# EnricoMiccoli/nodal

Measured on AMD Instinct MI355X. Metric: circuits_per_sec, higher is better.
Workload: dtype f64; 1 GPU; cfg3: grid(1000) 1e6 nodes, sparse CSR path; n=999999, nnz=4995995, parallelism=one GPU

## Files before the change

### nodal_amd/csrc/knobs.h

```cpp
#pragma once
#include <stdint.h>
#include <stdlib.h>

#include <optional>

namespace knob {

struct Present {
    const char *name;
    bool now() const { return getenv(name) != nullptr; }
};
struct OnUnless0 {
    const char *name;
    bool now() const { const char *e = getenv(name); return !(e && atoi(e) == 0); }
};
struct OffUnlessNon0 {
    const char *name;
    bool now() const { const char *e = getenv(name); return e && atoi(e) != 0; }
};
struct OnIfSet0 {
    const char *name;
    bool now() const { const char *e = getenv(name); return e != nullptr && atoi(e) == 0; }
};
struct Level {
    const char *name;
    int now() const {
        const char *e = getenv(name);
        if (!e) return 0;
        const int v = atoi(e);
        return v > 1 ? v : 1;
    }
};
struct Int {
    const char *name;
    int dflt;
    int now() const { const char *e = getenv(name); return e ? atoi(e) : dflt; }
};
struct Int64 {
    const char *name;
    int64_t dflt;
    int64_t now() const { const char *e = getenv(name); return e ? atoll(e) : dflt; }
};
struct Double {
    const char *name;
    double dflt;
    double now() const { const char *e = getenv(name); return e ? atof(e) : dflt; }
};
struct IntIfSet {
    const char *name;
    std::optional<int> now() const { const char *e = getenv(name); return e ? std::optional<int>(atoi(e)) : std::nullopt; }
};
struct Int64IfSet {
    const char *name;
    std::optional<int64_t> now() const { const char *e = getenv(name); return e ? std::optional<int64_t>(atoll(e)) : std::nullopt; }
};
struct DoubleIfSet {
    const char *name;
    std::optional<double> now() const { const char *e = getenv(name); return e ? std::optional<double>(atof(e)) : std::nullopt; }
};
struct Text {
    const char *name;
    const char *now() const { return getenv(name); }
};

inline constexpr Present TRACE{"NODAL_TRACE"};
inline constexpr Level POISON{"NODAL_POISON"};
inline constexpr Present NOFILL{"NODAL_NOFILL"};
inline constexpr Present NANCHECK{"NODAL_NANCHECK"};
inline constexpr Double WAIT_TIMEOUT_S{"NODAL_WAIT_TIMEOUT_S", 60.0};
inline constexpr Text STREAM_PRIORITY{"NODAL_STREAM_PRIORITY"};
inline constexpr IntIfSet EXTRA_STREAMS{"NODAL_EXTRA_STREAMS"};
inline constexpr IntIfSet HOST_THREADS{"NODAL_HOST_THREADS"};
inline constexpr IntIfSet CSV_CHUNKS{"NODAL_CSV_CHUNKS"};
inline constexpr OnUnless0 FOLD_STREAM{"NODAL_FOLD_STREAM"};
inline constexpr OffUnlessNon0 COUNT_LDS{"NODAL_COUNT_LDS"};
inline constexpr IntIfSet DENSE_BLOCKINV{"NODAL_DENSE_BLOCKINV"};
inline constexpr IntIfSet GJ_SCALAR{"NODAL_GJ_SCALAR"};
inline constexpr OnUnless0 GJ_DPP{"NODAL_GJ_DPP"};
inline constexpr OnUnless0 BI_SYM{"NODAL_BI_SYM"};
inline constexpr OnIfSet0 BI_MASKED{"NODAL_BI_MASKED"};
inline constexpr Int PANEL_CUS{"NODAL_PANEL_CUS", 32};
inline constexpr Int64 BI_UNMASK_ROWS{"NODAL_BI_UNMASK_ROWS", 0};
inline constexpr OnUnless0 BI_EARLY_COPY{"NODAL_BI_EARLY_COPY"};
inline constexpr Int BI_FIRST_BLOCKS{"NODAL_BI_FIRST_BLOCKS", 2};
inline constexpr Text BI_SWITCH{"NODAL_BI_SWITCH"};
inline constexpr Text BI_SWITCH2{"NODAL_BI_SWITCH2"};
inline constexpr Text BI_WIDTH{"NODAL_BI_WIDTH"};
inline constexpr IntIfSet GEPP_PANEL{"NODAL_GEPP_PANEL"};
inline constexpr Int GEPP_MAX{"NODAL_GEPP_MAX", 1280};
inline constexpr Present GEPP_PROBE{"NODAL_GEPP_PROBE"};
inline constexpr Int64IfSet FCG_MAXIT{"NODAL_FCG_MAXIT"};
inline constexpr OnUnless0 FCG_HOST_SUM{"NODAL_FCG_HOST_SUM"};
inline constexpr Double FCG_LOOK{"NODAL_FCG_LOOK", 0.75};
inline constexpr OnUnless0 LOWDEG{"NODAL_LOWDEG"};
inline constexpr IntIfSet LOWDEG_SHARE{"NODAL_LOWDEG_SHARE"};
inline constexpr Int64 LOWDEG_MIN{"NODAL_LOWDEG_MIN", 32};
inline constexpr Present SPARSE_FORCE_DIRECT{"NODAL_SPARSE_FORCE_DIRECT"};
inline constexpr Present SPARSE_CHILD_DIRECT{"NODAL_SPARSE_CHILD_DIRECT"};
inline constexpr OnUnless0 SAGG{"NODAL_SAGG"};
inline constexpr OnUnless0 SA_REUSE{"NODAL_SA_REUSE"};
inline constexpr OnUnless0 SA_FORK{"NODAL_SA_FORK"};
inline constexpr Double SA_SPREAD{"NODAL_SA_SPREAD", 16.0};
inline constexpr Double SA_SHARE{"NODAL_SA_SHARE", 0.9};
inline constexpr IntIfSet SA_MIS{"NODAL_SA_MIS"};
inline constexpr Text SA_OMEGA_P{"NODAL_SA_OMEGA_P"};
inline constexpr Double SA_PADSLACK{"NODAL_SA_PADSLACK", 1.3};
inline constexpr OnUnless0 SA_D16{"NODAL_SA_D16"};
inline constexpr Int SA_GG{"NODAL_SA_GG", 40};
inline constexpr Int64 SA_GCAP{"NODAL_SA_GCAP", 16384};
inline constexpr Int SA_GSEG{"NODAL_SA_GSEG", 4};
inline constexpr Text SA_NU{"NODAL_SA_NU"};
inline constexpr Int SA_KCYCLE{"NODAL_SA_KCYCLE", 1};
inline constexpr Int SA_KLEVELS{"NODAL_SA_KLEVELS", 1};
inline constexpr OnUnless0 SA_KFREEZE{"NODAL_SA_KFREEZE"};
inline constexpr OnUnless0 SA_FUSE_DIR{"NODAL_SA_FUSE_DIR"};
inline constexpr OffUnlessNon0 SA_GRAPH{"NODAL_SA_GRAPH"};
inline constexpr Text SA_FOLD_POST{"NODAL_SA_FOLD_POST"};
inline constexpr OffUnlessNon0 SA_FOLD_CHECK{"NODAL_SA_FOLD_CHECK"};
inline constexpr OnUnless0 SA_TAIL_DENSE{"NODAL_SA_TAIL_DENSE"};
inline constexpr OffUnlessNon0 SA_TAIL_CHECK{"NODAL_SA_TAIL_CHECK"};
inline constexpr Int SA_TAIL_NU{"NODAL_SA_TAIL_NU", 3};
inline constexpr Present TAIL_PROBE{"NODAL_TAIL_PROBE"};
inline constexpr IntIfSet AMG_PASSES0{"NODAL_AMG_PASSES0"};
inline constexpr IntIfSet AMG_PASSES1{"NODAL_AMG_PASSES1"};
inline constexpr IntIfSet AMG_SWEEPS0{"NODAL_AMG_SWEEPS0"};
inline constexpr IntIfSet AMG_BLOCK{"NODAL_AMG_BLOCK"};
inline constexpr DoubleIfSet AMG_THETA{"NODAL_AMG_THETA"};
inline constexpr Present AMG_KEEP_DENSE{"NODAL_AMG_KEEP_DENSE"};
inline constexpr Present AMG_NOTAIL{"NODAL_AMG_NOTAIL"};
inline constexpr IntIfSet AMG_KMAX{"NODAL_AMG_KMAX"};
inline constexpr OnUnless0 PAIRS_BLOCK{"NODAL_PAIRS_BLOCK"};
inline constexpr OnUnless0 PAIRS_FUNCTIONAL{"NODAL_PAIRS_FUNCTIONAL"};
inline constexpr Int PAIRS_DIRECT{"NODAL_PAIRS_DIRECT", -1};
inline constexpr Int64 PAIRS_DIRECT_MIN{"NODAL_PAIRS_DIRECT_MIN", 256};
inline constexpr Double MULTI_BAR{"NODAL_MULTI_BAR", 1e-14};
inline constexpr IntIfSet PRESOLVE{"NODAL_PRESOLVE"};
inline constexpr OnUnless0 PRESOLVE_KEEP{"NODAL_PRESOLVE_KEEP"};
inline constexpr IntIfSet FGMRES_WINDOW{"NODAL_FGMRES_WINDOW"};
inline constexpr Text DIRECT_NB{"NODAL_DIRECT_NB"};
inline constexpr Int DIRECT_LANES{"NODAL_DIRECT_LANES", 4};
inline constexpr DoubleIfSet DIRECT_MAX_GB{"NODAL_DIRECT_MAX_GB"};
inline constexpr IntIfSet DIRECT_BIG_DIM{"NODAL_DIRECT_BIG_DIM"};
inline constexpr OnUnless0 DIRECT_FRONT_LDS{"NODAL_DIRECT_FRONT_LDS"};
inline constexpr Int DIRECT_LDS_BS{"NODAL_DIRECT_LDS_BS", 64};
inline constexpr OnUnless0 DIRECT_PANEL_REGS{"NODAL_DIRECT_PANEL_REGS"};
inline constexpr OnUnless0 DIRECT_BATCHED{"NODAL_DIRECT_BATCHED"};
inline constexpr OnUnless0 DIRECT_WAVE{"NODAL_DIRECT_WAVE"};
inline constexpr Present DIRECT_LEVELS{"NODAL_DIRECT_LEVELS"};
inline constexpr OnUnless0 DIRECT_SUPER{"NODAL_DIRECT_SUPER"};
inline constexpr OnUnless0 DIRECT_APPLY_STEPPED{"NODAL_DIRECT_APPLY_STEPPED"};
inline constexpr OnUnless0 DIRECT_PEEL{"NODAL_DIRECT_PEEL"};
inline constexpr Int ND_DEPTH{"NODAL_ND_DEPTH", 4};
inline constexpr Int64 ND_PAR{"NODAL_ND_PAR", 20000};
inline constexpr Present SLU_DEBUG{"SLU_DEBUG"};

}
```

### nodal_amd/csrc/sagg.hip

```cpp
#include <hip/hip_ext.h>

#include <atomic>
#include <type_traits>

#include "group.h"

int grounded_flags(nodal_ctx *h, uint8_t *flags_dev);

namespace {

using grp::TB;
constexpr int PW = 4;
constexpr int ACAP = 64;
constexpr int RCAP = 96;
constexpr int RCAP_SMALL = 512;
constexpr int RCAP_SMALL_ROWS = 16384;
inline int rcap_for(int64_t nc) { return nc <= RCAP_SMALL_ROWS ? RCAP_SMALL : RCAP; }
constexpr int W0_MAX = 32;
constexpr int COARSEST = 64;
constexpr int MAX_LEVELS = 12;
constexpr int MIS_ROUNDS = 6;
constexpr int TAIL_MAX_N = 1024;
constexpr int TAIL_LEVELS = 6;
constexpr int TAIL_LDS_BUDGET = 150 * 1024;
constexpr int APAD = 32;
constexpr int DOT_BLOCKS = 1024;
#ifndef NODAL_SA_OMEGA
#define NODAL_SA_OMEGA 0.85
#endif
constexpr double OMEGA = NODAL_SA_OMEGA;
constexpr double OMEGA_P = 0.70;
constexpr double OMEGA_P_COARSE = 0.85;
using cyc_t = nodal_cyc_t;

inline unsigned grid_for(int64_t n, unsigned cap = 8192) {
    int64_t g = (n + TB - 1) / TB;
    if (g < 1) g = 1;
    if (g >= 64) g = (g + 7) & ~(int64_t)7;
    return (unsigned)(g > cap ? cap : g);
}
inline int64_t pad64(int64_t n) { return (n + 63) & ~(int64_t)63; }
inline size_t align256(size_t x) { return (x + 255) & ~(size_t)255; }

__device__ __forceinline__ unsigned xcd_block() {
    const unsigned g = gridDim.x, b = blockIdx.x;
    return (g & 7u) ? b : (b & 7u) * (g >> 3) + (b >> 3);
}


struct Ell {
    int64_t n = 0, ld = 0;
    int32_t width = 0;
    const int32_t *col = nullptr;
    const int16_t *dcol = nullptr;
    const double *val = nullptr;
    const float *valf = nullptr;
    const int32_t *len = nullptr;
};

enum { ST_MAXLEN = 0, ST_GRADED = 1, ST_BADDIAG = 2, ST_OVERFLOW = 3, ST_NNZ = 4, ST_UNASSIGNED = 5,
       ST_MAXR = 6, ST_NC = 7 ,
       ST_FARCOL = 8 ,
       ST_FOLDMISS = 9 ,
       ST_COUNT = 10 };

struct SLevel {
    int64_t n = 0, ld = 0, nc = 0;
    int32_t width = 0;
    int32_t maxlen = 0;
    int32_t wfix = 0;
    int64_t nnz = 0;
    DevBuf acol, aval, alen, dinv;
    DevBuf adcol;
    bool d16 = false;
    DevBuf agg, pcol, pval;
    DevBuf rcol, rval, rlen;
    int64_t rld = 0;
    DevBuf vec, part, gflag;
    DevBuf avalf, pvalf, rvalf;
    DevBuf wcol, wval, wlen;
    int32_t wslots = 0;
    bool fold_want = false, fold = false;
    Ell A() const {
        Ell e;
        e.n = n; e.ld = ld; e.width = width;
        e.col = acol.as<int32_t>(); e.val = aval.as<double>(); e.len = alen.as<int32_t>();
        e.valf = avalf.as<float>();
        e.dcol = d16 ? adcol.as<int16_t>() : nullptr;
        return e;
    }
    template <typename T = double> T *v(int which) const { return reinterpret_cast<T *>(vec.as<double>() + (int64_t)which * ld); }
};
enum { V_X = 0, V_R = 1, V_XP = 2, V_RC = 3, V_C1 = 4, V_C2 = 5, V_V1 = 6, V_V2 = 7, V_R2 = 8, V_X1 = 9, V_T = 10,
       V_COUNT = 11 };

struct TailLevelDesc {
    int n, nc, ld, rld, width, nq, lpr;
    const int32_t *acol, *pcol, *rcol, *rlen, *alen;
    const double *aval, *dinv, *pval, *rval;
    int o_aval, o_acol, o_dinv, o_pval, o_pcol, o_rval, o_rcol, o_B, o_X, o_Y, o_R;
};
struct TailDesc {
    int nlev;
    TailLevelDesc lv[TAIL_LEVELS];
    const double *inv;
    int nu;
    int image_bytes;
    int lds_bytes;
    int skip;
    int slots;
    long long *stamps;
};

struct SHierarchy {
    std::vector<SLevel *> pool;
    int nlev = 0;
    int tail = -1;
    bool ready = false;
    bool kcycle = true;
    bool kfrozen = false;
    int kslot = -1, kcount = 0, ksamples = 0;
    int klevels = 1;
    int nu[3] = {2, 1, 2};
    bool dense_coarsest = true;
    DevBuf tail_stamps, tail_image, apcol, apval, aplen, bstat;
    DevBuf tail_op;
    bool tail_dense = false;
    DevBuf mvec;
    hipEvent_t ev_copy = nullptr;
    hipStream_t aux = nullptr;
    hipEvent_t ev_fork = nullptr, ev_join = nullptr, ev_flags = nullptr;
    bool aux_pending = false;
    bool aux_tried = false;
    bool want_flags = false;
    int flags_levels = 0;
    DevBuf stats, coarse_inv, mis_t, mis_m, mis_flag, mis_id, agg1, keys, rstart, cursor, lists;
    TailDesc td;
    uint64_t *host_stats = nullptr;
    bool sym_valid = false;
    uint64_t sym_epoch = 0;
    int64_t sym_n = 0, sym_nnz = 0;
    bool sym_general = false, sym_check = false;
    int32_t sym_floating = 0;
    hipGraph_t it_graph = nullptr;
    hipGraphExec_t it_exec = nullptr;
    uint64_t it_key = 0;
    bool refreshed = false;
    int last_iters = 0;
    int hint_iters = 0;
    int64_t hint_n = 0, hint_nnz = 0;
    int mblock_iters = 0;
    int64_t mblock_n = 0;
    unsigned long long sym_stats[MAX_LEVELS * ST_COUNT] = {0};
    SLevel *level(int l) {
        while ((int)pool.size() <= l) pool.push_back(new SLevel());
        return pool[l];
    }
    void drop_graph() {
        if (it_exec) (void)hipGraphExecDestroy(it_exec);
        if (it_graph) (void)hipGraphDestroy(it_graph);
        it_exec = nullptr;
        it_graph = nullptr;
        it_key = 0;
    }
    ~SHierarchy() {
        drop_graph();
        if (ev_copy) (void)hipEventDestroy(ev_copy);
        if (ev_fork) (void)hipEventDestroy(ev_fork);
        if (ev_join) (void)hipEventDestroy(ev_join);
        if (ev_flags) (void)hipEventDestroy(ev_flags);
        if (aux) (void)hipStreamDestroy(aux);
        for (SLevel *l : pool) {
            DevBuf *b[] = {&l->acol, &l->aval, &l->alen, &l->dinv, &l->agg, &l->pcol, &l->pval, &l->rcol,
                           &l->rval, &l->rlen, &l->vec, &l->part, &l->gflag, &l->avalf, &l->pvalf, &l->rvalf, &l->adcol,
                           &l->wcol, &l->wval, &l->wlen};
            for (DevBuf *x : b) x->release();
            delete l;
        }
        tail_image.release();
        tail_op.release();
        mvec.release();
        tail_stamps.release();
        bstat.release();
        apcol.release();
        apval.release();
        aplen.release();
        DevBuf *b[] = {&stats, &coarse_inv, &mis_t, &mis_m, &mis_flag, &mis_id, &agg1, &keys, &rstart, &cursor, &lists};
        for (DevBuf *x : b) x->release();
        if (host_stats) (void)hipHostFree(host_stats);
    }
};


constexpr int BSTAT_MAX = 65536;
__global__ __launch_bounds__(1024) void reduce_bstat(int nblocks, const uint32_t *__restrict__ bstat,
                                                     unsigned long long *__restrict__ stats, int slot_max,
                                                     int slot_sum) {
    __shared__ unsigned int s_max;
    __shared__ unsigned long long s_sum;
    if (threadIdx.x == 0) { s_max = 0; s_sum = 0; }
    __syncthreads();
    unsigned int m = 0;
    unsigned long long t = 0;
    for (int i = threadIdx.x; i < nblocks; i += 1024) {
        m = max(m, bstat[i]);
        t += bstat[BSTAT_MAX + i];
    }
    atomicMax(&s_max, m);
    atomicAdd(&s_sum, t);
    __syncthreads();
    if (threadIdx.x == 0) {
        if (slot_max >= 0) stats[slot_max] = s_max;
        if (slot_sum >= 0) stats[slot_sum] = s_sum;
    }
}

__global__ __launch_bounds__(TB) void row_stats(int64_t n, const int32_t *__restrict__ indptr,
                                                const int32_t *__restrict__ indices,
                                                const double *__restrict__ data, double share, double spread,
                                                bool general, unsigned long long *__restrict__ stats,
                                                uint32_t *__restrict__ bstat) {
    int32_t mlen = 0;
    uint32_t graded = 0, bad = 0, far = 0;
    for (int64_t i = (int64_t)xcd_block() * TB + threadIdx.x; i < n; i += (int64_t)gridDim.x * TB) {
        const int32_t e0 = indptr[i], e1 = indptr[i + 1];
        mlen = max(mlen, e1 - e0);
        double d = 0.0, mx = 0.0, mn = 1e300;
        for (int32_t e = e0; e < e1; ++e) {
            const double v = data[e];
            const int64_t dc = (int64_t)indices[e] - i;
            if (dc > 32767 || dc < -32767) far = 1;
            if (indices[e] == (int32_t)i) d = v;
            else if (v != 0.0) {
                mx = fmax(mx, fabs(v));
                mn = fmin(mn, fabs(v));
                if (v > 0.0 && !general) bad = 1;
            }
        }
        if (!(d > 0.0)) bad = 1;
        graded += (d > 0.0 && (mx > share * d || mx > spread * mn)) ? 1u : 0u;
    }
    __shared__ unsigned int s_len, s_graded, s_bad;
    if (threadIdx.x == 0) s_len = s_graded = s_bad = 0;
    __syncthreads();
    atomicMax(&s_len, (unsigned)mlen);
    if (graded) atomicAdd(&s_graded, graded);
    if (bad) atomicOr(&s_bad, 1u);
    if (far) atomicOr(&s_bad, 2u);
    __syncthreads();
    if (threadIdx.x == 0) {
        bstat[blockIdx.x] = s_len;
        bstat[BSTAT_MAX + blockIdx.x] = s_graded;
        if (s_bad & 1u) atomicOr(&stats[ST_BADDIAG], 1ull);
        if (s_bad & 2u) stats[ST_FARCOL] = 1ull;
    }
}

__global__ __launch_bounds__(TB) void csr_to_ell(int64_t n, int64_t ld, const int32_t *__restrict__ indptr,
                                                 const int32_t *__restrict__ indices,
                                                 const double *__restrict__ data, int32_t *__restrict__ col,
                                                 double *__restrict__ val, float *__restrict__ valf,
                                                 int32_t *__restrict__ len, double *__restrict__ dinv, int32_t wpad,
                                                 int16_t *__restrict__ dcol) {
    for (int64_t i = (int64_t)xcd_block() * TB + threadIdx.x; i < n; i += (int64_t)gridDim.x * TB) {
        const int32_t e0 = indptr[i], e1 = indptr[i + 1];
        double d = 1.0;
        for (int32_t e = e0; e < e1; ++e) {
            const int32_t c = indices[e];
            const double v = data[e];
            col[(int64_t)(e - e0) * ld + i] = c;
            if (dcol) dcol[(int64_t)(e - e0) * ld + i] = (int16_t)(c - (int32_t)i);
            val[(int64_t)(e - e0) * ld + i] = v;
            valf[(int64_t)(e - e0) * ld + i] = (float)v;
            if (c == (int32_t)i) d = v;
        }
        for (int32_t s = e1 - e0; s < wpad; ++s) {
            col[(int64_t)s * ld + i] = (int32_t)i;
            if (dcol) dcol[(int64_t)s * ld + i] = 0;
            val[(int64_t)s * ld + i] = 0.0;
            valf[(int64_t)s * ld + i] = 0.0f;
        }
        len[i] = e1 - e0;
        dinv[i] = 1.0 / d;
    }
}


__device__ __forceinline__ uint32_t hash30(uint32_t x) {
    x ^= x >> 16;
    x *= 0x7feb352du;
    x ^= x >> 15;
    x *= 0x846ca68bu;
    x ^= x >> 16;
    return x & 0x3fffffffu;
}

__global__ __launch_bounds__(TB) void mis_init(int64_t n, uint32_t *__restrict__ T) {
    for (int64_t i = (int64_t)xcd_block() * TB + threadIdx.x; i < n; i += (int64_t)gridDim.x * TB)
        T[i] = (1u << 30) | hash30((uint32_t)i);
}

template <int NB>
__device__ __forceinline__ uint32_t nbr_max_batch(const Ell &A, const uint32_t *__restrict__ v, int64_t i, int32_t l, int32_t s0,
                                                  uint32_t best) {
    int32_t c[NB];
#pragma unroll
    for (int u = 0; u < NB; ++u) c[u] = A.col[(int64_t)(s0 + u < l ? s0 + u : 0) * A.ld + i];
    uint32_t t[NB];
#pragma unroll
    for (int u = 0; u < NB; ++u) t[u] = v[c[u]];
#pragma unroll
    for (int u = 0; u < NB; ++u) best = t[u] > best ? t[u] : best;
    return best;
}
__device__ __forceinline__ uint32_t nbr_max(const Ell &A, const uint32_t *__restrict__ v, int64_t i, int32_t l, uint32_t best) {
    if (l <= 5) return nbr_max_batch<5>(A, v, i, l, 0, best);
    for (int32_t s0 = 0; s0 < l; s0 += 8) best = nbr_max_batch<8>(A, v, i, l, s0, best);
    return best;
}

__global__ __launch_bounds__(TB) void mis_max(Ell A, const uint32_t *__restrict__ v, uint32_t *__restrict__ m) {
    for (int64_t i = (int64_t)xcd_block() * TB + threadIdx.x; i < A.n; i += (int64_t)gridDim.x * TB)
        m[i] = nbr_max(A, v, i, A.len[i], v[i]);
}

__global__ __launch_bounds__(TB) void mis_update(Ell A, uint32_t *__restrict__ T, const uint32_t *__restrict__ m1) {
    for (int64_t i = (int64_t)xcd_block() * TB + threadIdx.x; i < A.n; i += (int64_t)gridDim.x * TB) {
        const uint32_t own = T[i];
        if ((own >> 30) != 1) continue;
        const uint32_t best = nbr_max(A, m1, i, A.len[i], m1[i]);
        if (best == own) T[i] = own | (2u << 30);
        else if ((best >> 30) == 3) T[i] = 0;
    }
}

__global__ __launch_bounds__(TB) void mis_count(int64_t n, const uint32_t *__restrict__ T,
                                                unsigned long long *__restrict__ out) {
    uint32_t left = 0;
    for (int64_t i = (int64_t)xcd_block() * TB + threadIdx.x; i < n; i += (int64_t)gridDim.x * TB)
        left += (T[i] >> 30) == 1 ? 1u : 0u;
#pragma unroll
    for (int off = 32; off > 0; off >>= 1) left += __shfl_down(left, off, 64);
    if ((threadIdx.x & 63) == 0 && left) atomicAdd(out, (unsigned long long)left);
}

__global__ __launch_bounds__(TB) void mis_flag_roots(Ell A, const uint32_t *__restrict__ T,
                                                     uint32_t *__restrict__ flag) {
    for (int64_t i = (int64_t)xcd_block() * TB + threadIdx.x; i <= A.n; i += (int64_t)gridDim.x * TB) {
        uint32_t f = 0;
        if (i < A.n) {
            const uint32_t own = T[i];
            if ((own >> 30) == 3) f = 1;
            else if ((own >> 30) == 1) {
                bool near = false;
                const int32_t l = A.len[i];
                for (int32_t s = 0; s < l; ++s) near = near || (T[A.col[(int64_t)s * A.ld + i]] >> 30) == 3;
                f = near ? 0u : 1u;
            }
        }
        flag[i] = f;
    }
}

constexpr int64_t MIS_SMALL_MAX = 1024;
__global__ __launch_bounds__(1024) void mis_small(Ell A, uint32_t *__restrict__ T, uint32_t *__restrict__ M,
                                                  uint32_t *__restrict__ flag, int rounds) {
    const int64_t n = A.n;
    for (int64_t i = threadIdx.x; i < n; i += 1024) T[i] = (1u << 30) | hash30((uint32_t)i);
    __syncthreads();
    for (int r = 0; r < rounds; ++r) {
        for (int64_t i = threadIdx.x; i < n; i += 1024) {
            uint32_t best = T[i];
            const int32_t l = A.len[i];
            for (int32_t s = 0; s < l; ++s) {
                const uint32_t t = T[A.col[(int64_t)s * A.ld + i]];
                best = t > best ? t : best;
            }
            M[i] = best;
        }
        __syncthreads();
        for (int64_t i = threadIdx.x; i < n; i += 1024) {
            const uint32_t own = T[i];
            if ((own >> 30) != 1) continue;
            uint32_t best = M[i];
            const int32_t l = A.len[i];
            for (int32_t s = 0; s < l; ++s) {
                const uint32_t t = M[A.col[(int64_t)s * A.ld + i]];
                best = t > best ? t : best;
            }
            if (best == own) T[i] = own | (2u << 30);
            else if ((best >> 30) == 3) T[i] = 0;
        }
        __syncthreads();
    }
    for (int64_t i = threadIdx.x; i <= n; i += 1024) {
        uint32_t f = 0;
        if (i < n) {
            const uint32_t own = T[i];
            if ((own >> 30) == 3) f = 1;
            else if ((own >> 30) == 1) {
                bool near = false;
                const int32_t l = A.len[i];
                for (int32_t s = 0; s < l; ++s) near = near || (T[A.col[(int64_t)s * A.ld + i]] >> 30) == 3;
                f = near ? 0u : 1u;
            }
        }
        flag[i] = f;
    }
}

__global__ __launch_bounds__(TB) void assign_near(Ell A, const uint32_t *__restrict__ T,
                                                  const uint32_t *__restrict__ flag,
                                                  const uint32_t *__restrict__ id, int32_t *__restrict__ agg1) {
    for (int64_t i = (int64_t)xcd_block() * TB + threadIdx.x; i < A.n; i += (int64_t)gridDim.x * TB) {
        int32_t a = -1;
        if (flag[i]) a = (int32_t)id[i];
        else {
            uint32_t best = 0;
            const int32_t l = A.len[i];
            auto batch = [&](auto NBc, int32_t s0) {
                constexpr int NB = decltype(NBc)::value;
                int32_t c[NB];
#pragma unroll
                for (int u = 0; u < NB; ++u) c[u] = A.col[(int64_t)(s0 + u < l ? s0 + u : 0) * A.ld + i];
                uint32_t fl[NB], tt[NB], idd[NB];
#pragma unroll
                for (int u = 0; u < NB; ++u) {
                    fl[u] = flag[c[u]];
                    tt[u] = T[c[u]];
                    idd[u] = id[c[u]];
                }
#pragma unroll
                for (int u = 0; u < NB; ++u) {
                    if (s0 + u >= l || c[u] == (int32_t)i || !fl[u]) continue;
                    const uint32_t t = tt[u] | (3u << 30);
                    if (t > best) { best = t; a = (int32_t)idd[u]; }
                }
            };
            if (l <= 5) batch(std::integral_constant<int, 5>{}, 0);
            else for (int32_t s0 = 0; s0 < l; s0 += 8) batch(std::integral_constant<int, 8>{}, s0);
        }
        agg1[i] = a;
    }
}

__global__ __launch_bounds__(TB) void assign_far(Ell A, const int32_t *__restrict__ agg1, int32_t *__restrict__ agg,
                                                 unsigned long long *__restrict__ stats) {
    for (int64_t i = (int64_t)xcd_block() * TB + threadIdx.x; i < A.n; i += (int64_t)gridDim.x * TB) {
        int32_t a = agg1[i];
        if (a < 0) {
            double bw = -1.0;
            const int32_t l = A.len[i];
            auto batch = [&](auto NBc, int32_t s0) {
                constexpr int NB = decltype(NBc)::value;
                int32_t c[NB];
                double w[NB];
#pragma unroll
                for (int u = 0; u < NB; ++u) {
                    const int64_t at = (int64_t)(s0 + u < l ? s0 + u : 0) * A.ld + i;
                    c[u] = A.col[at];
                    w[u] = fabs(A.val[at]);
                }
                int32_t aj[NB];
#pragma unroll
                for (int u = 0; u < NB; ++u) aj[u] = agg1[c[u]];
#pragma unroll
                for (int u = 0; u < NB; ++u) {
                    if (s0 + u >= l || c[u] == (int32_t)i || aj[u] < 0) continue;
                    if (w[u] > bw) { bw = w[u]; a = aj[u]; }
                }
            };
            if (l <= 5) batch(std::integral_constant<int, 5>{}, 0);
            else for (int32_t s0 = 0; s0 < l; s0 += 8) batch(std::integral_constant<int, 8>{}, s0);
            if (a < 0) stats[ST_UNASSIGNED] = 1;
        }
        agg[i] = a;
    }
}

__global__ __launch_bounds__(TB) void build_P(Ell A, const double *__restrict__ dinv,
                                              const int32_t *__restrict__ agg, int32_t *__restrict__ pcol,
                                              double *__restrict__ pval, float *__restrict__ pvalf, double omega_p) {
    for (int64_t i = (int64_t)xcd_block() * TB + threadIdx.x; i < A.n; i += (int64_t)gridDim.x * TB) {
        int32_t c[PW];
        double v[PW];
#pragma unroll
        for (int k = 0; k < PW; ++k) { c[k] = -1; v[k] = 0.0; }
        const int32_t own = agg[i];
        c[0] = own;
        v[0] = 1.0;
        const double wd = omega_p * dinv[i];
        const int32_t l = A.len[i];
        for (int32_t s = 0; s < l; ++s) {
            const int32_t J = agg[A.col[(int64_t)s * A.ld + i]];
            const double t = -wd * A.val[(int64_t)s * A.ld + i];
            bool placed = false;
#pragma unroll
            for (int k = 0; k < PW; ++k) {
                if (!placed && c[k] == J) { v[k] += t; placed = true; }
            }
#pragma unroll
            for (int k = 1; k < PW; ++k) {
                if (!placed && c[k] < 0) { c[k] = J; v[k] = t; placed = true; }
            }
            if (!placed) v[0] += t;
        }
#pragma unroll
        for (int k = 0; k < PW; ++k) {
            pcol[(int64_t)k * A.ld + i] = c[k];
            pval[(int64_t)k * A.ld + i] = v[k];
            pvalf[(int64_t)k * A.ld + i] = (float)v[k];
        }
    }
}

__global__ __launch_bounds__(TB) void r_count(int64_t n, int64_t ld, const int32_t *__restrict__ pcol,
                                              uint32_t *__restrict__ cnt, uint32_t *__restrict__ place) {
    for (int64_t i = (int64_t)xcd_block() * TB + threadIdx.x; i < n; i += (int64_t)gridDim.x * TB) {
#pragma unroll
        for (int k = 0; k < PW; ++k) {
            const int32_t J = pcol[(int64_t)k * ld + i];
            if (J >= 0) place[(int64_t)k * ld + i] = atomicAdd(&cnt[J], 1u);
        }
    }
}
__global__ __launch_bounds__(TB) void r_fill(int64_t n, int64_t ld, const int32_t *__restrict__ pcol,
                                             const uint32_t *__restrict__ rstart, const uint32_t *__restrict__ place,
                                             uint64_t *__restrict__ keys) {
    for (int64_t i = (int64_t)xcd_block() * TB + threadIdx.x; i < n; i += (int64_t)gridDim.x * TB) {
#pragma unroll
        for (int k = 0; k < PW; ++k) {
            const int32_t J = pcol[(int64_t)k * ld + i];
            if (J >= 0) keys[rstart[J] + place[(int64_t)k * ld + i]] = ((uint64_t)i << 2) | (uint64_t)k;
        }
    }
}
__global__ __launch_bounds__(TB) void r_to_ell(int64_t nc, int64_t rld, const uint32_t *__restrict__ rstart,
                                               const uint64_t *__restrict__ keys, int64_t ld,
                                               const double *__restrict__ pval, int32_t *__restrict__ rcol,
                                               double *__restrict__ rval, float *__restrict__ rvalf,
                                               int32_t *__restrict__ rlen,
                                               unsigned long long *__restrict__ stats, uint32_t *__restrict__ bstat,
                                               uint32_t rcap) {
    uint32_t mlen = 0;
    const int sub = threadIdx.x & 7;
    const int64_t rows_per_pass = (int64_t)gridDim.x * (TB / 8);
    for (int64_t I = (int64_t)xcd_block() * (TB / 8) + threadIdx.x / 8; I < nc; I += rows_per_pass) {
        const uint32_t s0 = rstart[I];
        uint32_t l = rstart[I + 1] - s0;
        mlen = l > mlen ? l : mlen;
        if (l > rcap) l = rcap;
        const uint32_t upto = nc <= 4096 ? rcap : ((l + 7u) & ~7u);
        for (uint32_t t = sub; t < upto; t += 8) {
            const int64_t at = ((int64_t)(t >> 3) * rld + I) * 8 + (t & 7);
            if (t < l) {
                const uint64_t key = keys[s0 + t];
                const int64_t i = (int64_t)(key >> 2);
                const double v = pval[(int64_t)(key & 3) * ld + i];
                rcol[at] = (int32_t)i;
                rval[at] = v;
                rvalf[at] = (float)v;
            } else {
                rcol[at] = 0;
                rval[at] = 0.0;
                rvalf[at] = 0.0f;
            }
        }
        if (sub == 0) rlen[I] = (int32_t)l;
    }
    if (mlen > rcap) atomicOr(&stats[ST_OVERFLOW], 2ull);
    __shared__ unsigned int s_max;
    if (threadIdx.x == 0) s_max = 0;
    __syncthreads();
#pragma unroll
    for (int off = 32; off > 0; off >>= 1) {
        const uint32_t o = __shfl_down(mlen, off, 64);
        mlen = o > mlen ? o : mlen;
    }
    if ((threadIdx.x & 63) == 0) atomicMax(&s_max, mlen);
    __syncthreads();
    if (threadIdx.x == 0) {
        bstat[blockIdx.x] = s_max;
        bstat[BSTAT_MAX + blockIdx.x] = 0;
    }
}

__global__ __launch_bounds__(TB) void r_refresh(int64_t nc, int64_t rld, const int32_t *__restrict__ rlen,
                                                const int32_t *__restrict__ rcol, int64_t ld,
                                                const int32_t *__restrict__ pcol, const double *__restrict__ pval,
                                                double *__restrict__ rval, float *__restrict__ rvalf) {
    const int sub = threadIdx.x & 7;
    const int64_t rows_per_pass = (int64_t)gridDim.x * (TB / 8);
    for (int64_t I = (int64_t)xcd_block() * (TB / 8) + threadIdx.x / 8; I < nc; I += rows_per_pass) {
        const int32_t l = rlen[I];
        for (int32_t t = sub; t < l; t += 8) {
            const int64_t at = ((int64_t)(t >> 3) * rld + I) * 8 + (t & 7);
            const int64_t i = rcol[at];
            double v = 0.0;
#pragma unroll
            for (int k = 0; k < PW; ++k) {
                const double pv = pval[(int64_t)k * ld + i];
                v = pcol[(int64_t)k * ld + i] == (int32_t)I ? pv : v;
            }
            rval[at] = v;
            rvalf[at] = (float)v;
        }
    }
}

__global__ __launch_bounds__(TB) void r_sort_short(const uint32_t *__restrict__ rstart, uint64_t *__restrict__ keys,
                                                   int64_t nc) {
    for (int64_t I = (int64_t)xcd_block() * TB + threadIdx.x; I < nc; I += (int64_t)gridDim.x * TB) {
        const uint32_t s0 = rstart[I];
        const int len = (int)(rstart[I + 1] - s0);
        if (len < 2) continue;
        if (len <= 4) grp::sort_short_row<4>(keys + s0, len);
        else if (len <= 8) grp::sort_short_row<8>(keys + s0, len);
        else if (len <= 16) grp::sort_short_row<16>(keys + s0, len);
        else if (len <= 32) grp::sort_short_row<32>(keys + s0, len);
    }
}
__global__ __launch_bounds__(64) void r_sort_medium(const uint32_t *__restrict__ rstart, uint64_t *__restrict__ keys,
                                                    int64_t nc) {
    __shared__ uint64_t buf[RCAP_SMALL];
    const int lane = threadIdx.x;
    for (int64_t I = blockIdx.x; I < nc; I += gridDim.x) {
        const uint32_t s0 = rstart[I];
        const int len = (int)(rstart[I + 1] - s0);
        if (len <= 32 || len > RCAP_SMALL) continue;
        const int P = len <= 64 ? 64 : (len <= 128 ? 128 : (len <= 256 ? 256 : 512));
        for (int e = lane; e < P; e += 64) buf[e] = e < len ? keys[s0 + e] : ~0ull;
        __syncthreads();
        for (int size = 2; size <= P; size <<= 1)
            for (int stride = size >> 1; stride > 0; stride >>= 1) {
                for (int p = lane; p < P / 2; p += 64) {
                    const int i = ((p & ~(stride - 1)) << 1) | (p & (stride - 1));
                    const int j = i | stride;
                    const bool up = (i & size) == 0;
                    const uint64_t a = buf[i], b = buf[j];
                    if ((a > b) == up) { buf[i] = b; buf[j] = a; }
                }
                __syncthreads();
            }
        for (int e = lane; e < len; e += 64) keys[s0 + e] = buf[e];
        __syncthreads();
    }
}

__device__ __forceinline__ int wave_excl_scan(int v, int *total) {
    const int lane = threadIdx.x & 63;
    int incl = v;
#pragma unroll
    for (int off = 1; off < 64; off <<= 1) {
        const int t = __shfl_up(incl, off, 64);
        if (lane >= off) incl += t;
    }
    *total = __shfl(incl, 63, 64);
    return incl - v;
}

template <int APW, bool EMIT>
__global__ __launch_bounds__(TB) void ap_rows(Ell A, const int32_t *__restrict__ pcol, const double *__restrict__ pval,
                                              int32_t *__restrict__ apcol, double *__restrict__ apval,
                                              int32_t *__restrict__ aplen, unsigned long long *__restrict__ stats,
                                              const double *__restrict__ dinv, int32_t *__restrict__ wcol,
                                              float *__restrict__ wval, int32_t *__restrict__ wlen) {
    bool overflow = false, miss = false;
    for (int64_t i = (int64_t)xcd_block() * TB + threadIdx.x; i < A.n; i += (int64_t)gridDim.x * TB) {
        int32_t c[APW];
        double v[APW];
        [[maybe_unused]] int32_t Jo[PW];
        [[maybe_unused]] double po[PW], wd = 0.0;
        if constexpr (EMIT) {
#pragma unroll
            for (int sp = 0; sp < PW; ++sp) {
                Jo[sp] = pcol[(int64_t)sp * A.ld + i];
                po[sp] = pval[(int64_t)sp * A.ld + i];
            }
            wd = OMEGA * dinv[i];
        }
#pragma unroll
        for (int q = 0; q < APW; ++q) { c[q] = -1; v[q] = 0.0; }
        int cnt = 0;
        const int32_t l = A.len[i];
        for (int32_t s = 0; s < l; ++s) {
            const int32_t k = A.col[(int64_t)s * A.ld + i];
            const double a = A.val[(int64_t)s * A.ld + i];
            int32_t J[PW];
            double pp[PW];
#pragma unroll
            for (int sp = 0; sp < PW; ++sp) {
                J[sp] = pcol[(int64_t)sp * A.ld + k];
                pp[sp] = pval[(int64_t)sp * A.ld + k];
            }
#pragma unroll
            for (int sp = 0; sp < PW; ++sp) {
                if (J[sp] < 0) continue;
                const double t = a * pp[sp];
                bool placed = false;
#pragma unroll
                for (int q = 0; q < APW; ++q)
                    if (!placed && c[q] == J[sp]) { v[q] += t; placed = true; }
#pragma unroll
                for (int q = 0; q < APW; ++q)
                    if (!placed && c[q] < 0) { c[q] = J[sp]; v[q] = t; placed = true; cnt = q + 1; }
                if (!placed) overflow = true;
            }
        }
#pragma unroll
        for (int q = 0; q < APW; ++q)
            if (q < cnt) {
                apcol[(int64_t)q * A.ld + i] = c[q];
                apval[(int64_t)q * A.ld + i] = v[q];
            }
        aplen[i] = cnt;
        if constexpr (EMIT) {
            int have = 0, found = 0;
#pragma unroll
            for (int sp = 0; sp < PW; ++sp) have += Jo[sp] >= 0 ? 1 : 0;
#pragma unroll
            for (int q = 0; q < APW; ++q)
                if (q < cnt) {
                    double pv = 0.0;
#pragma unroll
                    for (int sp = 0; sp < PW; ++sp)
                        if (Jo[sp] == c[q]) { pv += po[sp]; ++found; }
                    wcol[(int64_t)q * A.ld + i] = c[q];
                    wval[(int64_t)q * A.ld + i] = (float)(pv - wd * v[q]);
                }
            wlen[i] = cnt;
            if (found != have) miss = true;
        }
    }
    if (overflow) atomicOr(&stats[ST_OVERFLOW], 4ull);
    if (miss) stats[ST_FOLDMISS] = 1ull;
}

template <int APW, bool EMIT>
__global__ __launch_bounds__(64) void ap_rows_lds(Ell A, const int32_t *__restrict__ pcol,
                                                  const double *__restrict__ pval, int32_t *__restrict__ apcol,
                                                  double *__restrict__ apval, int32_t *__restrict__ aplen,
                                                  unsigned long long *__restrict__ stats,
                                                  const double *__restrict__ dinv, int32_t *__restrict__ wcol,
                                                  float *__restrict__ wval, int32_t *__restrict__ wlen) {
    __shared__ int32_t tc[APW * 64];
    __shared__ double tv[APW * 64];
    const int lane = threadIdx.x;
    bool overflow = false, miss = false;
    for (int64_t i0 = (int64_t)xcd_block() * 64; i0 < A.n; i0 += (int64_t)gridDim.x * 64) {
        const int64_t i = i0 + lane;
#pragma unroll 8
        for (int q = 0; q < APW; ++q) tc[q * 64 + lane] = -1;
        int cnt = 0;
        if (i < A.n) {
            const int32_t l = A.len[i];
            [[maybe_unused]] int32_t Jo[PW];
            [[maybe_unused]] double po[PW], wd = 0.0;
            if constexpr (EMIT) {
#pragma unroll
                for (int sp = 0; sp < PW; ++sp) {
                    Jo[sp] = pcol[(int64_t)sp * A.ld + i];
                    po[sp] = pval[(int64_t)sp * A.ld + i];
                }
                wd = OMEGA * dinv[i];
            }
            constexpr int AB = 4;
            for (int32_t s0 = 0; s0 < l; s0 += AB) {
                int32_t kk[AB];
                double aa[AB];
#pragma unroll
                for (int u = 0; u < AB; ++u) {
                    const int32_t su = s0 + u < l ? s0 + u : 0;
                    kk[u] = A.col[(int64_t)su * A.ld + i];
                    aa[u] = A.val[(int64_t)su * A.ld + i];
                }
                int32_t J[AB][PW];
                double pp[AB][PW];
#pragma unroll
                for (int u = 0; u < AB; ++u)
#pragma unroll
                    for (int sp = 0; sp < PW; ++sp) {
                        J[u][sp] = pcol[(int64_t)sp * A.ld + kk[u]];
                        pp[u][sp] = pval[(int64_t)sp * A.ld + kk[u]];
                    }
#pragma unroll
                for (int u = 0; u < AB; ++u) {
                    if (s0 + u >= l) continue;
#pragma unroll
                    for (int sp = 0; sp < PW; ++sp) {
                        if (J[u][sp] < 0) continue;
                        const double t = aa[u] * pp[u][sp];
                        uint32_t slot = ((uint32_t)J[u][sp] * 2654435761u) >> 16 & (APW - 1);
                        bool placed = false;
                        for (int probe = 0; probe < APW && !placed; ++probe) {
                            const int32_t c = tc[slot * 64 + lane];
                            if (c == J[u][sp]) {
                                tv[slot * 64 + lane] += t;
                                placed = true;
                            } else if (c < 0) {
                                tc[slot * 64 + lane] = J[u][sp];
                                tv[slot * 64 + lane] = t;
                                ++cnt;
                                placed = true;
                            }
                            slot = (slot + 1) & (APW - 1);
                        }
                        if (!placed) overflow = true;
                    }
                }
            }
            int o = 0, found = 0;
            for (int q = 0; q < APW; ++q) {
                const int32_t c = tc[q * 64 + lane];
                if (c >= 0) {
                    const double t = tv[q * 64 + lane];
                    apcol[(int64_t)o * A.ld + i] = c;
                    apval[(int64_t)o * A.ld + i] = t;
                    if constexpr (EMIT) {
                        double pv = 0.0;
#pragma unroll
                        for (int sp = 0; sp < PW; ++sp)
                            if (Jo[sp] == c) { pv += po[sp]; ++found; }
                        wcol[(int64_t)o * A.ld + i] = c;
                        wval[(int64_t)o * A.ld + i] = (float)(pv - wd * t);
                    }
                    ++o;
                }
            }
            aplen[i] = cnt;
            if constexpr (EMIT) {
                int have = 0;
#pragma unroll
                for (int sp = 0; sp < PW; ++sp) have += Jo[sp] >= 0 ? 1 : 0;
                wlen[i] = cnt;
                if (found != have) miss = true;
            }
        }
    }
    if (overflow) atomicOr(&stats[ST_OVERFLOW], 4ull);
    if (miss) stats[ST_FOLDMISS] = 1ull;
}

__device__ __forceinline__ int galerkin_products(int64_t ld, const int32_t *__restrict__ apcol,
                                                 const double *__restrict__ apval, const int32_t *__restrict__ aplen,
                                                 int64_t rld, const int32_t *__restrict__ rcol,
                                                 const double *__restrict__ rval, int64_t I, int t0, int tn,
                                                 int32_t *lJ, double *lV) {
    const int lane = threadIdx.x;
    int32_t i = 0, len = 0;
    double w = 0.0;
    if (lane < tn) {
        const int t = t0 + lane;
        const int64_t rat = ((int64_t)(t >> 3) * rld + I) * 8 + (t & 7);
        i = rcol[rat];
        w = rval[rat];
        len = aplen[i];
    }
    int np = 0;
    int o = wave_excl_scan(len, &np);
    constexpr int INFL = 8;
    for (int32_t s0 = 0; s0 < len; s0 += INFL) {
        int32_t cj[INFL];
        double cv[INFL];
#pragma unroll
        for (int q = 0; q < INFL; ++q) {
            const int32_t s = s0 + q < len ? s0 + q : s0;
            cj[q] = apcol[(int64_t)s * ld + i];
            cv[q] = apval[(int64_t)s * ld + i];
        }
#pragma unroll
        for (int q = 0; q < INFL; ++q)
            if (s0 + q < len) {
                lJ[o] = cj[q];
                lV[o] = w * cv[q];
                ++o;
            }
    }
    for (int p = lane + np; p < np + 72; p += 64) lJ[p] = -1;
    __syncthreads();
    return np;
}

template <bool NUMERIC>
__global__ __launch_bounds__(64) void galerkin(int64_t ld, const int32_t *__restrict__ apcol,
                                               const double *__restrict__ apval, const int32_t *__restrict__ aplen,
                                               int64_t nc, int64_t rld, const int32_t *__restrict__ rcol,
                                               const double *__restrict__ rval, const int32_t *__restrict__ rlen,
                                               int64_t cld, int32_t *__restrict__ ccol, double *__restrict__ cval,
                                               float *__restrict__ cvalf,
                                               int32_t *__restrict__ clen, double *__restrict__ cdinv,
                                               unsigned long long *__restrict__ stats, uint32_t *__restrict__ bstat,
                                               int G, int pcap, int maxseg) {
    extern __shared__ __attribute__((aligned(16))) char gsm[];
    int32_t *set = reinterpret_cast<int32_t *>(gsm);
    double *lV = reinterpret_cast<double *>(gsm + 1024);
    int32_t *lJ = reinterpret_cast<int32_t *>(lV + pcap);
    const int lane = threadIdx.x;
    uint32_t my_max = 0, my_nnz = 0, my_flags = 0;
    for (int64_t I = blockIdx.x; I < nc; I += gridDim.x) {
        const int rl = rlen[I];
        const int ngroups = (rl + G - 1) / G;
        int np = 0;
        int total = 0;
        int32_t myJ = 0x7fffffff;
        if constexpr (NUMERIC) {
            total = clen[I];
            if (lane < total) myJ = ccol[(int64_t)lane * cld + I];
        } else {
        for (int k = lane; k < 256; k += 64) set[k] = -1;
        __syncthreads();
        for (int g = 0; g < ngroups; ++g) {
            np = galerkin_products(ld, apcol, apval, aplen, rld, rcol, rval, I, g * G, min(G, rl - g * G), lJ, lV);
            for (int p = lane; p < np; p += 64) {
                const int32_t J = lJ[p];
                uint32_t hsh = ((uint32_t)J * 2654435761u) >> 24;
                for (int probe = 0; probe < 256; ++probe) {
                    const int32_t old = atomicCAS(&set[hsh], -1, J);
                    if (old == -1 || old == J) break;
                    hsh = (hsh + 1) & 255u;
                    if (probe == 255) my_flags |= 1u;
                }
            }
            __syncthreads();
        }
        int32_t mine[4];
        int cnt = 0;
#pragma unroll
        for (int q = 0; q < 4; ++q) {
            mine[q] = set[lane * 4 + q];
            cnt += mine[q] >= 0 ? 1 : 0;
        }
        int off = wave_excl_scan(cnt, &total);
        __syncthreads();
#pragma unroll
        for (int q = 0; q < 4; ++q)
            if (mine[q] >= 0) set[off++] = mine[q];
        __syncthreads();
        if (total > ACAP) {
            my_flags |= 1u;
            total = ACAP;
        }
        myJ = lane < total ? set[lane] : 0x7fffffff;
        __syncthreads();
#pragma unroll
        for (int k = 2; k <= 64; k <<= 1) {
#pragma unroll
            for (int j = k >> 1; j > 0; j >>= 1) {
                const int32_t other = __shfl_xor(myJ, j, 64);
                const bool up = (lane & k) == 0, lower = (lane & j) == 0;
                const int32_t lo = myJ < other ? myJ : other, hi = myJ < other ? other : myJ;
                myJ = (lower == up) ? lo : hi;
            }
        }
        }
        const int nseg = min(maxseg, total <= 16 ? 4 : (total <= 32 ? 2 : 1)), segw = 64 / nseg;
        const int seg = lane / segw;
        const int32_t segJ = __shfl(myJ, lane % segw, 64);
        double acc = 0.0;
        for (int g = 0; g < ngroups; ++g) {
            if (ngroups > 1 || NUMERIC)
                np = galerkin_products(ld, apcol, apval, aplen, rld, rcol, rval, I, g * G, min(G, rl - g * G), lJ, lV);
            int chunk = (((np + nseg - 1) / nseg) + 7) & ~7;
            if (nseg > 1 && ((chunk >> 3) & 1) == 0) chunk += 8;
            for (int p = seg * chunk; p < (seg + 1) * chunk; p += 8) {
                int32_t j8[8];
                double v8[8];
#pragma unroll
                for (int u = 0; u < 8; ++u) {
                    j8[u] = lJ[p + u];
                    v8[u] = lV[p + u];
                }
#pragma unroll
                for (int u = 0; u < 8; ++u) acc += j8[u] == segJ ? v8[u] : 0.0;
            }
            __syncthreads();
        }
        if (nseg == 4) {
            const double a1 = __shfl(acc, lane + 16, 64), a2 = __shfl(acc, lane + 32, 64), a3 = __shfl(acc, lane + 48, 64);
            acc = (acc + a1) + (a2 + a3);
        } else if (nseg == 2) {
            acc += __shfl(acc, lane + 32, 64);
        }
        if (lane >= total && lane < APAD) {
            ccol[(int64_t)lane * cld + I] = (int32_t)I;
            cval[(int64_t)lane * cld + I] = 0.0;
            cvalf[(int64_t)lane * cld + I] = 0.0f;
        }
        if (lane < total) {
            ccol[(int64_t)lane * cld + I] = myJ;
            cval[(int64_t)lane * cld + I] = acc;
            cvalf[(int64_t)lane * cld + I] = (float)acc;
            if (myJ == (int32_t)I) {
                if (!(acc > 0.0)) my_flags |= 4u;
                cdinv[I] = acc > 0.0 ? 1.0 / acc : 1.0;
            }
        }
        if (lane == 0) {
            clen[I] = total;
            my_max = (uint32_t)total > my_max ? (uint32_t)total : my_max;
            my_nnz += (uint32_t)total;
        }
        __syncthreads();
    }
    if (lane == 0) {
        bstat[blockIdx.x] = my_max;
        bstat[BSTAT_MAX + blockIdx.x] = my_nnz;
    }
    if (my_flags & 1u) atomicOr(&stats[ST_OVERFLOW], 1ull);
    if (my_flags & 4u) atomicOr(&stats[ST_BADDIAG], 1ull);
}

__global__ __launch_bounds__(256) void coarsest_inverse(Ell A, double *__restrict__ inv,
                                                        unsigned long long *__restrict__ stats) {
    __shared__ double M[COARSEST][2 * COARSEST + 1];
    const int n = (int)A.n;
    for (int t = threadIdx.x; t < n * 2 * n; t += 256) {
        const int r = t / (2 * n), c = t % (2 * n);
        M[r][c] = (c >= n && c - n == r) ? 1.0 : 0.0;
    }
    __syncthreads();
    for (int r = threadIdx.x; r < n; r += 256)
        for (int s = 0; s < A.len[r]; ++s) M[r][A.col[(int64_t)s * A.ld + r]] = A.val[(int64_t)s * A.ld + r];
    __syncthreads();
    for (int k = 0; k < n; ++k) {
        const double pv = M[k][k];
        if (!(pv > 0.0)) {
            if (threadIdx.x == 0) atomicOr(&stats[ST_BADDIAG], 2ull);
            return;
        }
        const double rp = 1.0 / pv;
        __syncthreads();
        for (int c = threadIdx.x; c < 2 * n; c += 256) M[k][c] *= rp;
        __syncthreads();
        for (int t = threadIdx.x; t < n * 2 * n; t += 256) {
            const int r = t / (2 * n), c = t % (2 * n);
            if (r != k && c != k) M[r][c] = fma(-M[r][k], M[k][c], M[r][c]);
        }
        __syncthreads();
        for (int r = threadIdx.x; r < n; r += 256)
            if (r != k) M[r][k] = 0.0;
        __syncthreads();
    }
    for (int t = threadIdx.x; t < n * n; t += 256) inv[t] = M[t / n][n + t % n];
}

__global__ __launch_bounds__(TB) void flags_up(int64_t n, const int32_t *__restrict__ agg,
                                               const uint8_t *__restrict__ fine, uint8_t *__restrict__ coarse) {
    for (int64_t i = (int64_t)xcd_block() * TB + threadIdx.x; i < n; i += (int64_t)gridDim.x * TB)
        if (fine[i]) coarse[agg[i]] = 1;
}
__global__ __launch_bounds__(64) void last_level_floating(Ell A, const uint8_t *__restrict__ grounded,
                                                          uint32_t *__restrict__ floating) {
    __shared__ int label[COARSEST];
    __shared__ int changed;
    const int n = (int)A.n, i = threadIdx.x;
    if (i < n) label[i] = i;
    __syncthreads();
    for (int it = 0; it < COARSEST; ++it) {
        if (i == 0) changed = 0;
        __syncthreads();
        int best = i < n ? label[i] : 0;
        if (i < n)
            for (int s = 0; s < A.len[i]; ++s) {
                const int l = label[A.col[(int64_t)s * A.ld + i]];
                best = l < best ? l : best;
            }
        __syncthreads();
        if (i < n && best < label[i]) {
            label[i] = best;
            changed = 1;
        }
        __syncthreads();
        if (!changed) break;
        __syncthreads();
    }
    __shared__ int ok[COARSEST];
    if (i < n) ok[i] = 0;
    __syncthreads();
    if (i < n && grounded[i]) ok[label[i]] = 1;
    __syncthreads();
    if (i < n && label[i] == i && !ok[i]) *floating = 1;
}

__global__ __launch_bounds__(TB) void any_unflagged(int64_t n, const uint8_t *__restrict__ grounded,
                                                    uint32_t *__restrict__ floating) {
    for (int64_t i = (int64_t)xcd_block() * TB + threadIdx.x; i < n; i += (int64_t)gridDim.x * TB)
        if (!grounded[i]) *floating = 1;
}

}

#include "sagg_cycle.h"

namespace {

constexpr int SAGG_DECLINED = -3;

int width_class(int maxlen) {
    static const int classes[] = {4, 5, 6, 8, 12, 16, 20, 24, 32};
    for (int c : classes)
        if (maxlen <= c) return c;
    return 0;
}
int choose_wfix(int maxlen, int64_t n, int64_t nnz, int pad_limit) {
    const int c = width_class(maxlen);
    if (c == 0 || c > pad_limit) return 0;
    static const double slack = knob::SA_PADSLACK.now();
    if ((double)c * (double)n <= slack * (double)nnz || n <= 32768) return c;
    return 0;
}

SHierarchy *hierarchy_of(nodal_ctx *h) {
    if (!h->sagg) h->sagg = new SHierarchy();
    return static_cast<SHierarchy *>(h->sagg);
}

struct SolveBufs {
    double *r, *p, *p2, *Ap, *part_rz, *part_zap, *part_rr, *part_pap, *sc;
    cyc_t *z, *x0;
    int g0;
};

template <bool NUMERIC>
int galerkin_product(nodal_ctx *h, SHierarchy *H, int l, hipEvent_t r_ready = nullptr, int phase = 0) {
    hipStream_t st = h->stream;
    SLevel *L = H->level(l), *C = H->level(l + 1);
    const int64_t n = L->n, ld = L->ld, nc = C->n;
    Ell A = L->A();
    A.width = L->maxlen;
    unsigned long long *dstats = H->stats.as<unsigned long long>();
    const int apw = A.width <= 6 ? 16 : 64;
    NODAL_HIP_TRY(h, H->apcol.reserve((size_t)apw * ld * 4 + 64));
    NODAL_HIP_TRY(h, H->apval.reserve((size_t)apw * ld * 8 + 64));
    NODAL_HIP_TRY(h, H->aplen.reserve((size_t)ld * 4 + 64));
    int32_t *apcol = H->apcol.as<int32_t>(), *aplen = H->aplen.as<int32_t>();
    double *apval = H->apval.as<double>();
    unsigned long long *lst = dstats + (size_t)l * ST_COUNT;
    const unsigned g = grid_for(n);
    if (phase != 2) {
        const bool w = L->fold_want && L->wslots == apw;
        int32_t *wcol = w ? L->wcol.as<int32_t>() : nullptr, *wlen = w ? L->wlen.as<int32_t>() : nullptr;
        float *wval = w ? L->wval.as<float>() : nullptr;
        const double *dinv = L->dinv.as<double>();
        const int32_t *pc = L->pcol.as<int32_t>();
        const double *pv = L->pval.as<double>();
        const unsigned gl = (unsigned)((n + 63) / 64 < 4096 ? (n + 63) / 64 : 4096);
        if (apw == 16 && w) ap_rows<16, true><<<g, TB, 0, st>>>(A, pc, pv, apcol, apval, aplen, lst, dinv, wcol, wval, wlen);
        else if (apw == 16) ap_rows<16, false><<<g, TB, 0, st>>>(A, pc, pv, apcol, apval, aplen, lst, dinv, wcol, wval, wlen);
        else if (w) ap_rows_lds<64, true><<<gl, 64, 0, st>>>(A, pc, pv, apcol, apval, aplen, lst, dinv, wcol, wval, wlen);
        else ap_rows_lds<64, false><<<gl, 64, 0, st>>>(A, pc, pv, apcol, apval, aplen, lst, dinv, wcol, wval, wlen);
        NODAL_HIP_TRY(h, hipGetLastError());
    }
    if (phase == 1) return NODAL_OK;
    int G = 1024 / apw;
    G = (G < 8 ? 8 : (G > 64 ? 64 : G));
    static const int g_env = knob::SA_GG.now();
    if (g_env >= 8 && g_env <= 64 && apw == 16) G = g_env & ~7;
    const int pcap = G * apw + 72;
    const size_t lds = 1024 + (size_t)pcap * 12;
    static const int64_t gcap = knob::SA_GCAP.now();
    static const int maxseg = knob::SA_GSEG.now();
    const unsigned gg = (unsigned)(nc < gcap ? nc : (gcap < BSTAT_MAX ? gcap : BSTAT_MAX));
    if (r_ready) NODAL_HIP_TRY(h, hipStreamWaitEvent(st, r_ready, 0));
    galerkin<NUMERIC><<<gg, 64, lds, st>>>(
        ld, apcol, apval, aplen, nc, L->rld, L->rcol.as<int32_t>(), L->rval.as<double>(), L->rlen.as<int32_t>(),
        C->ld, C->acol.as<int32_t>(), C->aval.as<double>(), C->avalf.as<float>(), C->alen.as<int32_t>(),
        C->dinv.as<double>(), dstats + (size_t)(l + 1) * ST_COUNT, H->bstat.as<uint32_t>(), G, pcap, maxseg);
    if (!NUMERIC)
        reduce_bstat<<<1, 1024, 0, st>>>((int)gg, H->bstat.as<uint32_t>(), dstats + (size_t)(l + 1) * ST_COUNT,
                                         ST_MAXLEN, ST_NNZ);
    NODAL_HIP_TRY(h, hipGetLastError());
    return NODAL_OK;
}

double omega_p(int level) {
    static double w[2] = {-1.0, -1.0};
    if (w[0] < 0.0) {
        double a = OMEGA_P, b = OMEGA_P_COARSE;
        if (const char *e = knob::SA_OMEGA_P.now()) {
            a = atof(e);
            const char *c = strchr(e, ',');
            b = c ? atof(c + 1) : a;
        }
        w[1] = b > 0.0 && b < 1.2 ? b : OMEGA_P_COARSE;
        w[0] = a > 0.0 && a < 1.0 ? a : OMEGA_P;
    }
    return w[level > 0 ? 1 : 0];
}

constexpr int64_t FOLD_MAX_ROWS = 1 << 19;
struct FoldSetting { int mode = 0; unsigned mask = 0; };
const FoldSetting &fold_setting() {
    static const FoldSetting s = [] {
        FoldSetting f;
        const char *e = knob::SA_FOLD_POST.now();
        if (!e || !*e) return f;
        if (strchr(e, 'l')) {
            f.mode = 3;
            for (const char *q = e; (q = strchr(q, 'l')) != nullptr; ++q) {
                const int k = atoi(q + 1);
                if (q[1] >= '0' && q[1] <= '9' && k < MAX_LEVELS) f.mask |= 1u << k;
            }
        } else {
            f.mode = atoi(e) == 0 ? 1 : 2;
        }
        return f;
    }();
    return s;
}
bool fold_wanted(int level, int64_t n) {
    if (level > 0 && n <= TAIL_MAX_N) return false;
    const FoldSetting &f = fold_setting();
    switch (f.mode) {
    case 1: return false;
    case 2: return true;
    case 3: return (f.mask >> level & 1u) != 0;
    default: return n <= FOLD_MAX_ROWS;
    }
}
void decide_folds(SHierarchy *H, const unsigned long long *hs, bool trace) {
    for (int k = 0; k < H->nlev; ++k) {
        SLevel *L = H->pool[k];
        const bool runs_cycle = k + 1 < H->nlev && (H->tail < 0 || k < H->tail);
        const bool miss = hs[(size_t)k * ST_COUNT + ST_FOLDMISS] != 0;
        L->fold = L->fold_want && runs_cycle && !miss;
        if (trace && L->fold_want && runs_cycle)
            fprintf(stderr, "[sagg] level %d (%lld rows): first post-smoothing sweep %s\n", k, (long long)L->n,
                    miss ? "NOT folded: a row of A P lacks a column of its P row (no stored diagonal)"
                         : "folded into the prolongation");
    }
}

int build_level(nodal_ctx *h, SHierarchy *H, int l, unsigned long long *hs, bool *declined, bool *stop) {
    hipStream_t st = h->stream;
    SLevel *L = H->level(l);
    const int64_t n = L->n, ld = L->ld;
    Ell A = L->A();
    A.width = L->maxlen;
    unsigned long long *dstats = H->stats.as<unsigned long long>();

    NODAL_HIP_TRY(h, H->mis_t.reserve((size_t)n * 8 + 64));
    NODAL_HIP_TRY(h, H->mis_m.reserve((size_t)n * 8 + 64));
    NODAL_HIP_TRY(h, H->mis_flag.reserve((size_t)(n + 1) * 4 + 64));
    NODAL_HIP_TRY(h, H->mis_id.reserve((size_t)(n + 1) * 4 + 64 + scan_tmp_bytes(n + 1)));
    NODAL_HIP_TRY(h, H->agg1.reserve((size_t)n * 4 + 64));
    NODAL_HIP_TRY(h, L->agg.reserve((size_t)n * 4 + 64));
    NODAL_HIP_TRY(h, H->cursor.reserve((MIS_ROUNDS + 2) * 8 + 64));
    uint32_t *T = H->mis_t.as<uint32_t>(), *M = H->mis_m.as<uint32_t>();
    uint32_t *flag = H->mis_flag.as<uint32_t>(), *id = H->mis_id.as<uint32_t>();
    unsigned long long *cnt = H->cursor.as<unsigned long long>();
    void *scan_tmp = H->mis_id.as<char>() + (((size_t)(n + 1) * 4 + 63) & ~(size_t)63);

    const unsigned g = grid_for(n);
    static const bool trace_mis = knob::TRACE.now();
    if (trace_mis) NODAL_HIP_TRY(h, hipMemsetAsync(cnt, 0, (MIS_ROUNDS + 2) * 8, st));
    static const int mis_rounds = std::min(MIS_ROUNDS, std::max(1, knob::SA_MIS.now().value_or(MIS_ROUNDS)));
    if (n <= MIS_SMALL_MAX && !trace_mis) {
        mis_small<<<1, 1024, 0, st>>>(A, T, M, flag, mis_rounds);
    } else {
        mis_init<<<g, TB, 0, st>>>(n, T);
        for (int r = 0; r < mis_rounds; ++r) {
            mis_max<<<g, TB, 0, st>>>(A, T, M);
            mis_update<<<g, TB, 0, st>>>(A, T, M);
            if (trace_mis) mis_count<<<g, TB, 0, st>>>(n, T, cnt + r + 1);
        }
        mis_flag_roots<<<grid_for(n + 1), TB, 0, st>>>(A, T, flag);
    }
    NODAL_HIP_TRY(h, hipGetLastError());
    NODAL_TRY(scan_exclusive_u32(h, flag, id, n + 1, reinterpret_cast<uint32_t *>(dstats + (size_t)l * ST_COUNT + ST_NC),
                                 scan_tmp));
    NODAL_HIP_TRY(h, hipMemcpyAsync(hs, dstats, (size_t)MAX_LEVELS * ST_COUNT * 8, hipMemcpyDeviceToHost, st));
    unsigned long long hcnt[MIS_ROUNDS + 1] = {0};
    if (trace_mis) NODAL_HIP_TRY(h, hipMemcpyAsync(hcnt, cnt, sizeof hcnt, hipMemcpyDeviceToHost, st));
    if (!H->ev_copy) NODAL_HIP_TRY(h, hipEventCreateWithFlags(&H->ev_copy, hipEventDisableTiming));
    NODAL_HIP_TRY(h, hipEventRecord(H->ev_copy, st));
    NODAL_HIP_TRY(h, L->pcol.reserve((size_t)PW * ld * 4 + 64));
    NODAL_HIP_TRY(h, L->pval.reserve((size_t)PW * ld * 8 + 64));
    NODAL_HIP_TRY(h, L->pvalf.reserve((size_t)PW * ld * 4 + 64));
    assign_near<<<g, TB, 0, st>>>(A, T, flag, id, H->agg1.as<int32_t>());
    assign_far<<<g, TB, 0, st>>>(A, H->agg1.as<int32_t>(), L->agg.as<int32_t>(), dstats + (size_t)l * ST_COUNT);
    build_P<<<g, TB, 0, st>>>(A, L->dinv.as<double>(), L->agg.as<int32_t>(), L->pcol.as<int32_t>(),
                             L->pval.as<double>(), L->pvalf.as<float>(), omega_p(l));
    NODAL_HIP_TRY(h, hipGetLastError());
    NODAL_WAIT_EVENT(h, H->ev_copy, st);
    if (trace_mis) {
        fprintf(stderr, "[sagg] level %d: undecided after each MIS round:", l);
        for (int r = 1; r <= MIS_ROUNDS; ++r) fprintf(stderr, " %llu", hcnt[r]);
        fprintf(stderr, "\n");
    }
    const int64_t nc = (int64_t)(hs[(size_t)l * ST_COUNT + ST_NC] & 0xffffffffull);
    if (l > 0) {
        const unsigned long long *s = hs + (size_t)l * ST_COUNT;
        L->maxlen = (int32_t)s[ST_MAXLEN];
        L->nnz = (int64_t)s[ST_NNZ];
        A.width = L->maxlen;
        if (s[ST_OVERFLOW] || s[ST_BADDIAG] || hs[(size_t)(l - 1) * ST_COUNT + ST_OVERFLOW] ||
            hs[(size_t)(l - 1) * ST_COUNT + ST_UNASSIGNED]) {
            *declined = true;
            return NODAL_OK;
        }
    }
    if (nc >= n || L->maxlen <= 1) {
        *stop = true;
        return NODAL_OK;
    }
    if ((nc * 2 > n && n > 4096) || nc < 1) {
        *declined = true;
        return NODAL_OK;
    }
    L->nc = nc;

    static const bool fork_allowed = knob::SA_FORK.now();
    if (H->aux && !nodal_extra_streams_ok(h) && nodal_calls_in_flight() <= 1) {
        NODAL_WAIT_STREAM(h, H->aux);
        (void)hipStreamDestroy(H->aux);
        H->aux = nullptr;
        H->aux_tried = false;
    }
    if (fork_allowed && !H->aux_tried && nodal_extra_streams_ok(h)) {
        H->aux_tried = true;
        if (hipStreamCreateWithFlags(&H->aux, hipStreamNonBlocking) != hipSuccess) H->aux = nullptr;
        if (H->aux && ((!H->ev_fork && hipEventCreateWithFlags(&H->ev_fork, hipEventDisableTiming) != hipSuccess) ||
                       (!H->ev_join && hipEventCreateWithFlags(&H->ev_join, hipEventDisableTiming) != hipSuccess) ||
                       (!H->ev_flags && hipEventCreateWithFlags(&H->ev_flags, hipEventDisableTiming) != hipSuccess))) {
            (void)hipStreamDestroy(H->aux);
            H->aux = nullptr;
        }
        (void)hipGetLastError();
    }
    const bool forked = fork_allowed && H->aux != nullptr && nodal_extra_streams_ok(h);
    const size_t a4 = (((size_t)(nc + 1) * 4) + 255) & ~(size_t)255;
    const size_t scan2 = (scan_tmp_bytes(nc + 1) + 255) & ~(size_t)255;
    NODAL_HIP_TRY(h, H->rstart.reserve(a4 + 256 + scan2 + (size_t)PW * ld * 4 + 64));
    NODAL_HIP_TRY(h, H->keys.reserve((size_t)PW * n * 8 + 64));
    SLevel *C = H->level(l + 1);
    C->n = nc;
    C->ld = pad64(nc);
    C->width = ACAP;
    C->nc = 0;
    L->rld = C->ld;
    const int rcap = rcap_for(nc);
    NODAL_HIP_TRY(h, L->rcol.reserve((size_t)rcap * C->ld * 4 + 64));
    NODAL_HIP_TRY(h, L->rval.reserve((size_t)rcap * C->ld * 8 + 64));
    NODAL_HIP_TRY(h, L->rvalf.reserve((size_t)rcap * C->ld * 4 + 64));
    NODAL_HIP_TRY(h, L->rlen.reserve((size_t)C->ld * 4 + 64));
    NODAL_HIP_TRY(h, C->acol.reserve((size_t)ACAP * C->ld * 4 + 64));
    NODAL_HIP_TRY(h, C->aval.reserve((size_t)ACAP * C->ld * 8 + 64));
    NODAL_HIP_TRY(h, C->avalf.reserve((size_t)ACAP * C->ld * 4 + 64));
    NODAL_HIP_TRY(h, C->alen.reserve((size_t)C->ld * 4 + 64));
    NODAL_HIP_TRY(h, C->dinv.reserve((size_t)C->ld * 8 + 64));
    if (forked && H->want_flags) {
        if (l == 0) NODAL_HIP_TRY(h, L->gflag.reserve((size_t)n + 64));
        NODAL_HIP_TRY(h, C->gflag.reserve((size_t)C->n + 64));
    }
    {
        const int apw = L->maxlen <= 6 ? 16 : 64;
        NODAL_HIP_TRY(h, H->apcol.reserve((size_t)apw * ld * 4 + 64));
        NODAL_HIP_TRY(h, H->apval.reserve((size_t)apw * ld * 8 + 64));
        NODAL_HIP_TRY(h, H->aplen.reserve((size_t)ld * 4 + 64));
        L->fold = false;
        L->fold_want = fold_wanted(l, n);
        L->wslots = apw;
        if (L->fold_want) {
            NODAL_HIP_TRY(h, L->wcol.reserve((size_t)apw * ld * 4 + 64));
            NODAL_HIP_TRY(h, L->wval.reserve((size_t)apw * ld * 4 + 64));
            NODAL_HIP_TRY(h, L->wlen.reserve((size_t)ld * 4 + 64));
        }
    }
    hipStream_t main_st = h->stream;
    struct StreamGuard {
        nodal_ctx *h;
        hipStream_t keep;
        ~StreamGuard() { h->stream = keep; }
    } guard{h, main_st};
    if (forked) {
        NODAL_HIP_TRY(h, hipEventRecord(H->ev_fork, main_st));
        NODAL_HIP_TRY(h, hipStreamWaitEvent(H->aux, H->ev_fork, 0));
        H->aux_pending = true;
        NODAL_TRY(galerkin_product<false>(h, H, l, nullptr, 1));
        h->stream = H->aux;
        st = H->aux;
    }
    char *rs = H->rstart.as<char>();
    uint32_t *rstart = reinterpret_cast<uint32_t *>(rs);
    void *scan_tmp2 = rs + a4 + 256;
    uint32_t *place = reinterpret_cast<uint32_t *>(rs + a4 + 256 + scan2);
    NODAL_HIP_TRY(h, hipMemsetAsync(rs, 0, a4 + 256, st));
    r_count<<<g, TB, 0, st>>>(n, ld, L->pcol.as<int32_t>(), rstart, place);
    NODAL_HIP_TRY(h, hipGetLastError());
    NODAL_TRY(scan_exclusive_u32(h, rstart, rstart, nc + 1, nullptr, scan_tmp2));
    uint64_t *keys = H->keys.as<uint64_t>();
    r_fill<<<g, TB, 0, st>>>(n, ld, L->pcol.as<int32_t>(), rstart, place, keys);
    r_sort_short<<<grid_for(nc), TB, 0, st>>>(rstart, keys, nc);
    r_sort_medium<<<(unsigned)(nc < 8192 ? nc : 8192), 64, 0, st>>>(rstart, keys, nc);
    NODAL_HIP_TRY(h, hipGetLastError());

    {
        const unsigned gr = grid_for(nc * 8);
        r_to_ell<<<gr, TB, 0, st>>>(nc, L->rld, rstart, keys, ld, L->pval.as<double>(), L->rcol.as<int32_t>(),
                                   L->rval.as<double>(), L->rvalf.as<float>(), L->rlen.as<int32_t>(),
                                   dstats + (size_t)l * ST_COUNT, H->bstat.as<uint32_t>(), (uint32_t)rcap);
        reduce_bstat<<<1, 1024, 0, st>>>((int)gr, H->bstat.as<uint32_t>(), dstats + (size_t)l * ST_COUNT, ST_MAXR, -1);
    }
    if (forked) {
        NODAL_HIP_TRY(h, hipGetLastError());
        NODAL_HIP_TRY(h, hipEventRecord(H->ev_join, H->aux));
        if (H->want_flags && H->flags_levels == l) {
            if (l == 0) NODAL_TRY(grounded_flags(h, L->gflag.as<uint8_t>()));
            NODAL_HIP_TRY(h, hipMemsetAsync(C->gflag.p, 0, ((size_t)C->n + 63) & ~(size_t)63, st));
            flags_up<<<grid_for(n), TB, 0, st>>>(n, L->agg.as<int32_t>(), L->gflag.as<uint8_t>(), C->gflag.as<uint8_t>());
            NODAL_HIP_TRY(h, hipGetLastError());
            NODAL_HIP_TRY(h, hipEventRecord(H->ev_flags, H->aux));
            H->flags_levels = l + 1;
        }
        h->stream = main_st;
        st = main_st;
    }
    NODAL_TRY(galerkin_product<false>(h, H, l, forked ? H->ev_join : nullptr, forked ? 2 : 0));
    if (forked && H->flags_levels != l + 1) H->aux_pending = false;
    return NODAL_OK;
}

const void *tail_kernel(int slots) {
    return slots <= 8 ? reinterpret_cast<const void *>(k_tail<8>)
                      : slots <= 16 ? reinterpret_cast<const void *>(k_tail<16>)
                                    : reinterpret_cast<const void *>(k_tail<32>);
}

const void *tail_op_kernel(int slots) {
    return slots <= 8 ? reinterpret_cast<const void *>(k_tail_pack_op<8>)
                      : slots <= 16 ? reinterpret_cast<const void *>(k_tail_pack_op<16>)
                                    : reinterpret_cast<const void *>(k_tail_pack_op<32>);
}

int tail_walk(nodal_ctx *h, SHierarchy *H, const double *b, double *out, int nv) {
    const TailDesc &d = H->td;
    const char *img = H->tail_image.as<char>();
    if (d.slots <= 8) k_tail<8><<<nv, 1024, (size_t)d.lds_bytes, h->stream>>>(d, img, b, out, nv);
    else if (d.slots <= 16) k_tail<16><<<nv, 1024, (size_t)d.lds_bytes, h->stream>>>(d, img, b, out, nv);
    else k_tail<32><<<nv, 1024, (size_t)d.lds_bytes, h->stream>>>(d, img, b, out, nv);
    NODAL_HIP_TRY(h, hipGetLastError());
    return NODAL_OK;
}

template <int NV>
int tail_apply(nodal_ctx *h, SHierarchy *H, const double *b, double *out) {
    const int n = H->td.lv[0].n;
    const double *T = H->tail_op.as<double>();
    const unsigned gr = (unsigned)((n + 3) / 4);
    if (n <= 256) k_tail_apply<4, NV><<<gr, 256, 0, h->stream>>>(n, T, b, out);
    else if (n <= 512) k_tail_apply<8, NV><<<gr, 256, 0, h->stream>>>(n, T, b, out);
    else k_tail_apply<16, NV><<<gr, 256, 0, h->stream>>>(n, T, b, out);
    NODAL_HIP_TRY(h, hipGetLastError());
    return NODAL_OK;
}

int tail_self_check(nodal_ctx *h, SHierarchy *H) {
    const int n = H->td.lv[0].n;
    std::vector<double> b((size_t)n), yc((size_t)n), yd((size_t)n), T((size_t)n * n);
    uint64_t seed = 0x9e3779b97f4a7c15ull;
    for (int i = 0; i < n; ++i) {
        uint64_t z = (seed += 0x9e3779b97f4a7c15ull);
        z = (z ^ (z >> 30)) * 0xbf58476d1ce4e5b9ull;
        z = (z ^ (z >> 27)) * 0x94d049bb133111ebull;
        z ^= z >> 31;
        b[i] = (double)(z >> 11) * (1.0 / 4503599627370496.0) - 1.0;
    }
    DevBuf v;
    hipError_t e = v.reserve((size_t)3 * n * 8);
    double *db = v.as<double>(), *dc = db + n, *dd = dc + n;
    int rc = NODAL_OK;
    if (e == hipSuccess) e = hipMemcpyAsync(db, b.data(), (size_t)n * 8, hipMemcpyHostToDevice, h->stream);
    if (e == hipSuccess) rc = tail_walk(h, H, db, dc, 1);
    if (e == hipSuccess && rc == NODAL_OK) rc = tail_apply<1>(h, H, db, dd);
    if (e == hipSuccess && rc == NODAL_OK) e = hipStreamSynchronize(h->stream);
    if (e == hipSuccess) e = hipMemcpy(yc.data(), dc, (size_t)n * 8, hipMemcpyDeviceToHost);
    if (e == hipSuccess) e = hipMemcpy(yd.data(), dd, (size_t)n * 8, hipMemcpyDeviceToHost);
    if (e == hipSuccess) e = hipMemcpy(T.data(), H->tail_op.p, (size_t)n * n * 8, hipMemcpyDeviceToHost);
    v.release();
    if (rc != NODAL_OK) return rc;
    NODAL_HIP_TRY(h, e);
    double d = 0.0, dp = 0.0;
    for (int i = 0; i < n; ++i) {
        long double y = 0.0L, a = 0.0L;
        for (int j = 0; j < n; ++j) {
            y += (long double)T[(size_t)i * n + j] * b[j];
            a += fabsl((long double)T[(size_t)i * n + j] * b[j]);
        }
        const double den = (double)a;
        const double q = fabs(yd[i] - yc[i]) / den, qp = (double)(fabsl((long double)yd[i] - y) / a);
        d = !(q <= d) ? q : d;
        dp = !(qp <= dp) ? qp : dp;
    }
    fprintf(stderr, "[sagg] tail check: n_t %d, dense operator against the cycle d = %.3e (product alone %.3e)\n", n, d, dp);
    return NODAL_OK;
}

int form_tail_op(nodal_ctx *h, SHierarchy *H) {
    static const bool on = knob::SA_TAIL_DENSE.now();
    H->tail_dense = false;
    if (!on || H->tail < 0) return NODAL_OK;
    const TailDesc &d = H->td;
    const int n = d.lv[0].n;
    static std::atomic<int> cus[64];
    const int dev = h->device >= 0 && h->device < 64 ? h->device : 0;
    int ncu = cus[dev].load(std::memory_order_acquire);
    if (ncu == 0) {
        NODAL_HIP_TRY(h, hipDeviceGetAttribute(&ncu, hipDeviceAttributeMultiprocessorCount, h->device >= 0 ? h->device : 0));
        if (ncu < 1) ncu = 1;
        cus[dev].store(ncu, std::memory_order_release);
    }
    NODAL_HIP_TRY(h, H->tail_op.reserve((size_t)n * n * 8 + 64));
    const unsigned gr = (unsigned)(n < ncu ? n : ncu);
    double *T = H->tail_op.as<double>();
    const char *img = H->tail_image.as<char>();
    if (d.slots <= 8) k_tail_pack_op<8><<<gr, 1024, (size_t)d.lds_bytes, h->stream>>>(d, img, T);
    else if (d.slots <= 16) k_tail_pack_op<16><<<gr, 1024, (size_t)d.lds_bytes, h->stream>>>(d, img, T);
    else k_tail_pack_op<32><<<gr, 1024, (size_t)d.lds_bytes, h->stream>>>(d, img, T);
    NODAL_HIP_TRY(h, hipGetLastError());
    H->tail_dense = true;
    static const bool check = knob::TRACE.now() && knob::SA_TAIL_CHECK.now();
    if (check) NODAL_TRY(tail_self_check(h, H));
    return NODAL_OK;
}

template <typename TC>
int fold_check_level(nodal_ctx *h, SHierarchy *H, int l, bool two) {
    hipStream_t st = h->stream;
    const SLevel *L = H->pool[l];
    const int64_t n = L->n, nc = H->pool[l + 1]->n;
    const Ell A = L->A();
    uint64_t seed = 0x9e3779b97f4a7c15ull + (uint64_t)l;
    auto unit = [&]() {
        uint64_t z = (seed += 0x9e3779b97f4a7c15ull);
        z = (z ^ (z >> 30)) * 0xbf58476d1ce4e5b9ull;
        z = (z ^ (z >> 27)) * 0x94d049bb133111ebull;
        z ^= z >> 31;
        return (double)(z >> 11) * (1.0 / 4503599627370496.0) - 1.0;
    };
    std::vector<cyc_t> hx((size_t)n), hb((size_t)n);
    std::vector<TC> he((size_t)2 * nc);
    for (auto &v : hx) v = (cyc_t)unit();
    for (auto &v : hb) v = (cyc_t)unit();
    for (auto &v : he) v = (TC)unit();
    const double hcoef[2] = {0.9, 0.4};
    const size_t vb = align256((size_t)n * sizeof(cyc_t)), eb = align256((size_t)nc * sizeof(TC)), db = align256((size_t)n * 8);
    DevBuf buf;
    hipError_t e = buf.reserve(6 * vb + 2 * eb + 2 * db + 256);
    char *p = buf.as<char>();
    cyc_t *x = reinterpret_cast<cyc_t *>(p), *b = reinterpret_cast<cyc_t *>(p + vb), *r = reinterpret_cast<cyc_t *>(p + 2 * vb),
          *xp = reinterpret_cast<cyc_t *>(p + 3 * vb), *mt = reinterpret_cast<cyc_t *>(p + 4 * vb),
          *mf = reinterpret_cast<cyc_t *>(p + 5 * vb);
    TC *c1 = reinterpret_cast<TC *>(p + 6 * vb), *c2 = reinterpret_cast<TC *>(p + 6 * vb + eb);
    double *d = reinterpret_cast<double *>(p + 6 * vb + 2 * eb), *q = reinterpret_cast<double *>(p + 6 * vb + 2 * eb + db);
    double *coef = reinterpret_cast<double *>(p + 6 * vb + 2 * eb + 2 * db);
    std::vector<double> hd((size_t)n), hq((size_t)n);
    if (e == hipSuccess) e = hipMemcpyAsync(x, hx.data(), (size_t)n * sizeof(cyc_t), hipMemcpyHostToDevice, st);
    if (e == hipSuccess) e = hipMemcpyAsync(b, hb.data(), (size_t)n * sizeof(cyc_t), hipMemcpyHostToDevice, st);
    if (e == hipSuccess) e = hipMemcpyAsync(c1, he.data(), (size_t)nc * sizeof(TC), hipMemcpyHostToDevice, st);
    if (e == hipSuccess) e = hipMemcpyAsync(c2, he.data() + nc, (size_t)nc * sizeof(TC), hipMemcpyHostToDevice, st);
    if (e == hipSuccess) e = hipMemcpyAsync(coef, hcoef, sizeof hcoef, hipMemcpyHostToDevice, st);
    if (e == hipSuccess) {
        const unsigned g = grid_for(n), tb = L->wfix ? TB : TB * LPR_RAGGED;
        const double *dinv = L->dinv.as<double>(), *cf = two ? coef : nullptr;
        const int32_t *wcol = L->wcol.as<int32_t>(), *wlen = L->wlen.as<int32_t>();
        const float *wval = L->wval.as<float>();
        SAGG_DISPATCH_W(L->wfix, (k_smooth_residual<W, cyc_t><<<g, tb, 0, st>>>(A, b, x, r)));
        k_prolong<TC><<<g, TB, 0, st>>>(n, L->ld, L->pcol.as<int32_t>(), L->pvalf.as<float>(), x, c1, two ? c2 : nullptr, cf, xp);
        SAGG_DISPATCH_W(L->wfix, (k_post<W, false, cyc_t, cyc_t><<<g, tb, 0, st>>>(A, dinv, b, xp, mt, nullptr, nullptr, nullptr)));
        k_prolong_post<TC, cyc_t><<<g, TB, 0, st>>>(n, L->ld, wcol, wval, wlen, x, r, dinv, c1, two ? c2 : nullptr, cf, mf);
        k_fold_check<TC><<<g, TB, 0, st>>>(A, dinv, b, x, xp, wcol, wval, wlen, c1, two ? c2 : nullptr, cf, mt, mf, d, q);
        e = hipGetLastError();
    }
    if (e == hipSuccess) e = hipStreamSynchronize(st);
    if (e == hipSuccess) e = hipMemcpy(hd.data(), d, (size_t)n * 8, hipMemcpyDeviceToHost);
    if (e == hipSuccess) e = hipMemcpy(hq.data(), q, (size_t)n * 8, hipMemcpyDeviceToHost);
    buf.release();
    NODAL_HIP_TRY(h, e);
    double dm = 0.0, qm = 0.0;
    for (int64_t i = 0; i < n; ++i) {
        dm = !(hd[i] <= dm) ? hd[i] : dm;
        qm = !(hq[i] <= qm) ? hq[i] : qm;
    }
    fprintf(stderr, "[sagg] fold check: level %d, rows %lld, slots %d, width %d, fused launch against the two d = %.3e "
                    "(worst row against its own bound: %.3e)\n", l, (long long)n, (int)L->wslots, (int)L->maxlen, dm, qm);
    return NODAL_OK;
}
int fold_self_check(nodal_ctx *h, SHierarchy *H) {
    static const bool check = knob::TRACE.now() && knob::SA_FOLD_CHECK.now();
    if (!check) return NODAL_OK;
    for (int l = 0; l + 1 < H->nlev; ++l) {
        if (!H->pool[l]->fold) continue;
        const bool last = l + 1 == H->tail || l + 1 == H->nlev - 1;
        if (last) NODAL_TRY(fold_check_level<double>(h, H, l, false));
        else NODAL_TRY(fold_check_level<cyc_t>(h, H, l, true));
    }
    return NODAL_OK;
}

int build_tail(nodal_ctx *h, SHierarchy *H, const unsigned long long *hs) {
    H->tail = -1;
    H->tail_dense = false;
    const int last = H->nlev - 1;
    auto up16 = [](int x) { return (x + 15) & ~15; };
    for (int t = 1; t <= last; ++t) {
        if (H->pool[t]->n > TAIL_MAX_N || last - t + 1 > TAIL_LEVELS) continue;
        TailDesc d;
        memset(&d, 0, sizeof d);
        d.nlev = last - t + 1;
        d.nu = knob::SA_TAIL_NU.now();
        if (d.nu < 1) d.nu = 1;
        int off = 0;
        for (int k = 0; k < d.nlev; ++k) {
            const SLevel *L = H->pool[t + k];
            TailLevelDesc &q = d.lv[k];
            q.n = (int)L->n; q.nc = (int)L->nc; q.ld = (int)L->ld; q.rld = (int)L->rld; q.width = L->maxlen;
            q.acol = L->acol.as<int32_t>(); q.aval = L->aval.as<double>();
            q.dinv = L->dinv.as<double>(); q.alen = L->alen.as<int32_t>();
            q.pcol = L->pcol.as<int32_t>(); q.pval = L->pval.as<double>();
            q.rcol = L->rcol.as<int32_t>(); q.rval = L->rval.as<double>(); q.rlen = L->rlen.as<int32_t>();
            if (k == d.nlev - 1) {
                q.o_aval = off; off = up16(off + (H->dense_coarsest ? q.n * q.n : q.n) * 8);
                continue;
            }
            const int maxr = (int)hs[(size_t)(t + k) * ST_COUNT + ST_MAXR];
            q.nq = (maxr + 7) / 8;
            q.lpr = 1;
            while (q.lpr < 8 && q.n * q.lpr * 2 <= 1024) q.lpr *= 2;
            q.o_aval = off; off = up16(off + q.n * q.width * 8);
            q.o_acol = off; off = up16(off + q.n * q.width * 2);
            q.o_dinv = off; off = up16(off + q.n * 8);
            q.o_pval = off; off = up16(off + q.n * PW * 8);
            q.o_pcol = off; off = up16(off + q.n * PW * 2);
            q.o_rval = off; off = up16(off + q.nq * q.nc * 8 * 8);
            q.o_rcol = off; off = up16(off + q.nq * q.nc * 8 * 2);
        }
        d.image_bytes = off;
        for (int k = 0; k < d.nlev; ++k) {
            TailLevelDesc &q = d.lv[k];
            q.o_B = off; off = up16(off + q.n * 8);
            q.o_X = off; off = up16(off + q.n * 8);
            if (k == d.nlev - 1) continue;
            q.o_Y = off; off = up16(off + q.n * 8);
            q.o_R = off; off = up16(off + q.n * 8);
        }
        d.inv = H->dense_coarsest ? H->coarse_inv.as<double>() : nullptr;
        d.skip = d.nlev > 1 ? d.lv[0].o_dinv : 0;
        d.lds_bytes = off - d.skip;
        if (knob::TAIL_PROBE.now()) {
            NODAL_HIP_TRY(h, H->tail_stamps.reserve(64 * sizeof(long long)));
            d.stamps = H->tail_stamps.as<long long>();
        }
        if (d.lds_bytes > TAIL_LDS_BUDGET) continue;
        d.slots = d.nlev > 1 ? (d.lv[0].width + d.lv[0].lpr - 1) / d.lv[0].lpr : 1;
        if (d.slots > 32) continue;
        {
            static std::atomic<bool> lds_allowed[64][3];
            const int dev = h->device >= 0 && h->device < 64 ? h->device : 0;
            const int which = d.slots <= 8 ? 0 : (d.slots <= 16 ? 1 : 2);
            if (!lds_allowed[dev][which].load(std::memory_order_acquire)) {
                NODAL_HIP_TRY(h, hipFuncSetAttribute(tail_kernel(d.slots), hipFuncAttributeMaxDynamicSharedMemorySize,
                                                     TAIL_LDS_BUDGET));
                NODAL_HIP_TRY(h, hipFuncSetAttribute(tail_op_kernel(d.slots), hipFuncAttributeMaxDynamicSharedMemorySize,
                                                     TAIL_LDS_BUDGET));
                lds_allowed[dev][which].store(true, std::memory_order_release);
            }
        }
        NODAL_HIP_TRY(h, H->tail_image.reserve((size_t)d.image_bytes + 256));
        k_tail_pack<<<1, 1024, 0, h->stream>>>(d, H->tail_image.as<char>());
        NODAL_HIP_TRY(h, hipGetLastError());
        H->td = d;
        H->tail = t;
        NODAL_TRY(form_tail_op(h, H));
        break;
    }
    return NODAL_OK;
}

int sagg_refresh(nodal_ctx *h, SHierarchy *H, const int32_t *indptr0, const int32_t *indices0, const double *data0,
                 bool general, bool *ok) {
    *ok = false;
    hipStream_t st = h->stream;
    unsigned long long *dstats = H->stats.as<unsigned long long>();
    unsigned long long *hs = reinterpret_cast<unsigned long long *>(H->host_stats);
    NODAL_HIP_TRY(h, hipMemsetAsync(dstats, 0, (size_t)MAX_LEVELS * ST_COUNT * 8, st));
    SLevel *L0 = H->pool[0];
    const int64_t n0 = L0->n;
    {
        const unsigned gr = grid_for(n0);
        static const double spread = knob::SA_SPREAD.now();
        static const double share = knob::SA_SHARE.now();
        row_stats<<<gr, TB, 0, st>>>(n0, indptr0, indices0, data0, share, spread, general, dstats, H->bstat.as<uint32_t>());
        reduce_bstat<<<1, 1024, 0, st>>>((int)gr, H->bstat.as<uint32_t>(), dstats, ST_MAXLEN, ST_GRADED);
    }
    csr_to_ell<<<grid_for(n0), TB, 0, st>>>(n0, L0->ld, indptr0, indices0, data0, L0->acol.as<int32_t>(),
                                           L0->aval.as<double>(), L0->avalf.as<float>(),
                                           L0->alen.as<int32_t>(), L0->dinv.as<double>(), L0->wfix,
                                           L0->d16 ? L0->adcol.as<int16_t>() : nullptr);
    NODAL_HIP_TRY(h, hipGetLastError());
    for (int l = 0; l + 1 < H->nlev; ++l) {
        SLevel *L = H->pool[l], *C = H->pool[l + 1];
        Ell A = L->A();
        A.width = L->maxlen;
        build_P<<<grid_for(L->n), TB, 0, st>>>(A, L->dinv.as<double>(), L->agg.as<int32_t>(), L->pcol.as<int32_t>(),
                                              L->pval.as<double>(), L->pvalf.as<float>(), omega_p(l));
        const bool forked = H->aux != nullptr && nodal_extra_streams_ok(h) &&
                            knob::SA_FORK.now();
        hipStream_t rst = st;
        if (forked) {
            NODAL_HIP_TRY(h, hipEventRecord(H->ev_fork, st));
            NODAL_HIP_TRY(h, hipStreamWaitEvent(H->aux, H->ev_fork, 0));
            H->aux_pending = true;
            NODAL_TRY(galerkin_product<true>(h, H, l, nullptr, 1));
            rst = H->aux;
        }
        r_refresh<<<grid_for(C->n * 8), TB, 0, rst>>>(C->n, L->rld, L->rlen.as<int32_t>(), L->rcol.as<int32_t>(), L->ld,
                                                     L->pcol.as<int32_t>(), L->pval.as<double>(), L->rval.as<double>(),
                                                     L->rvalf.as<float>());
        NODAL_HIP_TRY(h, hipGetLastError());
        if (forked) NODAL_HIP_TRY(h, hipEventRecord(H->ev_join, H->aux));
        NODAL_TRY(galerkin_product<true>(h, H, l, forked ? H->ev_join : nullptr, forked ? 2 : 0));
        if (forked) H->aux_pending = false;
    }
    const int last = H->nlev - 1;
    if (H->dense_coarsest)
        coarsest_inverse<<<1, 256, 0, st>>>(H->pool[last]->A(), H->coarse_inv.as<double>(), dstats + (size_t)last * ST_COUNT);
    if (H->tail >= 0) k_tail_pack<<<1, 1024, 0, st>>>(H->td, H->tail_image.as<char>());
    NODAL_HIP_TRY(h, hipGetLastError());
    NODAL_TRY(form_tail_op(h, H));
    NODAL_HIP_TRY(h, hipMemcpyAsync(hs, dstats, (size_t)MAX_LEVELS * ST_COUNT * 8, hipMemcpyDeviceToHost, st));
    NODAL_WAIT_STREAM(h, st);
    const int64_t bar = n0 / 100 < 32 ? (n0 / 100 > 0 ? n0 / 100 : 1) : 32;
    if (hs[ST_BADDIAG] || (int64_t)hs[ST_GRADED] >= bar) return NODAL_OK;
    for (int k = 1; k < H->nlev; ++k)
        if (hs[(size_t)k * ST_COUNT + ST_BADDIAG] || hs[(size_t)k * ST_COUNT + ST_OVERFLOW]) return NODAL_OK;
    decide_folds(H, hs, false);
    NODAL_TRY(fold_self_check(h, H));
    *ok = true;
    return NODAL_OK;
}

}

void sagg_destroy(nodal_ctx *h) {
    delete static_cast<SHierarchy *>(h->sagg);
    h->sagg = nullptr;
}

static int sagg_setup_csr_body(nodal_ctx *h, int64_t n0, int64_t nnz0, const int32_t *indptr0, const int32_t *indices0,
                               const double *data0, bool general, bool check_floating, bool *accepted, int32_t *floating);

int sagg_setup_csr(nodal_ctx *h, int64_t n0, int64_t nnz0, const int32_t *indptr0, const int32_t *indices0,
                   const double *data0, bool general, bool check_floating, bool *accepted, int32_t *floating) {
    const int s = sagg_setup_csr_body(h, n0, nnz0, indptr0, indices0, data0, general, check_floating, accepted, floating);
    SHierarchy *H = static_cast<SHierarchy *>(h->sagg);
    if (H && H->aux && H->aux_pending && H->ev_flags) {
        if (hipEventRecord(H->ev_flags, H->aux) == hipSuccess) (void)hipStreamWaitEvent(h->stream, H->ev_flags, 0);
        H->aux_pending = false;
        (void)hipGetLastError();
    }
    return s;
}

static int sagg_setup_csr_body(nodal_ctx *h, int64_t n0, int64_t nnz0, const int32_t *indptr0, const int32_t *indices0,
                               const double *data0, bool general, bool check_floating, bool *accepted, int32_t *floating) {
    *accepted = false;
    *floating = 0;
    static const bool enabled = knob::SAGG.now();
    static const bool trace = knob::TRACE.now();
    if (!enabled) return NODAL_OK;
    SHierarchy *H = hierarchy_of(h);
    H->ready = false;
    hipStream_t st = h->stream;
    if (n0 >= (1ll << 30)) return NODAL_OK;
    static const bool reuse = knob::SA_REUSE.now();
    if (reuse && H->sym_valid && H->sym_epoch == h->struct_epoch && H->sym_n == n0 && H->sym_nnz == nnz0 &&
        H->sym_general == general && H->sym_check == check_floating) {
        bool ok = false;
        NODAL_TRY(sagg_refresh(h, H, indptr0, indices0, data0, general, &ok));
        if (ok) {
            *floating = H->sym_floating;
            H->refreshed = true;
            H->ready = true;
            *accepted = true;
            if (trace) fprintf(stderr, "[sagg] symbolic setup kept (struct epoch %llu): values refreshed\n",
                               (unsigned long long)h->struct_epoch);
            return NODAL_OK;
        }
        if (trace) fprintf(stderr, "[sagg] the kept hierarchy does not take the new values: full setup\n");
    }
    H->sym_valid = false;
    H->refreshed = false;
    H->want_flags = check_floating;
    H->flags_levels = 0;
    H->last_iters = 0;
    H->drop_graph();
    NODAL_HIP_TRY(h, H->stats.reserve((size_t)MAX_LEVELS * ST_COUNT * 8 + 64));
    if (!H->host_stats)
        NODAL_HIP_TRY(h, hipHostMalloc(reinterpret_cast<void **>(&H->host_stats), (size_t)MAX_LEVELS * ST_COUNT * 8 + 64));
    unsigned long long *dstats = H->stats.as<unsigned long long>();
    unsigned long long *hs = reinterpret_cast<unsigned long long *>(H->host_stats);
    NODAL_HIP_TRY(h, hipMemsetAsync(dstats, 0, (size_t)MAX_LEVELS * ST_COUNT * 8, st));
    NODAL_HIP_TRY(h, H->bstat.reserve((size_t)2 * BSTAT_MAX * 4 + 64));
    {
        const unsigned gr = grid_for(n0);
        static const double spread = knob::SA_SPREAD.now();
        static const double share = knob::SA_SHARE.now();
        row_stats<<<gr, TB, 0, st>>>(n0, indptr0, indices0, data0, share, spread, general, dstats, H->bstat.as<uint32_t>());
        reduce_bstat<<<1, 1024, 0, st>>>((int)gr, H->bstat.as<uint32_t>(), dstats, ST_MAXLEN, ST_GRADED);
    }
    NODAL_HIP_TRY(h, hipGetLastError());
    NODAL_HIP_TRY(h, hipMemcpyAsync(hs, dstats, ST_COUNT * 8, hipMemcpyDeviceToHost, st));
    NODAL_WAIT_STREAM(h, st);
    const int64_t bar = n0 / 100 < 32 ? (n0 / 100 > 0 ? n0 / 100 : 1) : 32;
    if (hs[ST_MAXLEN] > (unsigned long long)W0_MAX || hs[ST_MAXLEN] == 0 || hs[ST_BADDIAG] ||
        (int64_t)hs[ST_GRADED] >= bar) {
        if (trace)
            fprintf(stderr, "[sagg] declined: longest row %llu, graded nodes %llu (bar %lld), M-matrix %s\n",
                    hs[ST_MAXLEN], hs[ST_GRADED], (long long)bar, hs[ST_BADDIAG] ? "no" : "yes");
        return NODAL_OK;
    }
    SLevel *L0 = H->level(0);
    L0->n = n0;
    L0->ld = pad64(n0);
    L0->maxlen = (int32_t)hs[ST_MAXLEN];
    L0->nnz = nnz0;
    L0->wfix = choose_wfix(L0->maxlen, n0, nnz0, 8);
    L0->width = L0->wfix ? L0->wfix : L0->maxlen;
    NODAL_HIP_TRY(h, L0->acol.reserve((size_t)L0->width * L0->ld * 4 + 64));
    NODAL_HIP_TRY(h, L0->aval.reserve((size_t)L0->width * L0->ld * 8 + 64));
    NODAL_HIP_TRY(h, L0->avalf.reserve((size_t)L0->width * L0->ld * 4 + 64));
    NODAL_HIP_TRY(h, L0->alen.reserve((size_t)L0->ld * 4 + 64));
    NODAL_HIP_TRY(h, L0->dinv.reserve((size_t)L0->ld * 8 + 64));
    static const bool d16_env = knob::SA_D16.now();
    L0->d16 = d16_env && hs[ST_FARCOL] == 0;
    if (L0->d16) NODAL_HIP_TRY(h, L0->adcol.reserve((size_t)L0->width * L0->ld * 2 + 64));
    csr_to_ell<<<grid_for(n0), TB, 0, st>>>(n0, L0->ld, indptr0, indices0, data0, L0->acol.as<int32_t>(),
                                           L0->aval.as<double>(), L0->avalf.as<float>(),
                                           L0->alen.as<int32_t>(), L0->dinv.as<double>(), L0->wfix,
                                           L0->d16 ? L0->adcol.as<int16_t>() : nullptr);
    NODAL_HIP_TRY(h, hipGetLastError());

    int l = 0;
    bool diag_last = false;
    for (;; ++l) {
        SLevel *L = H->level(l);
        if (L->n <= COARSEST && l > 0) break;
        if (l + 1 >= MAX_LEVELS) {
            if (trace) fprintf(stderr, "[sagg] declined: more than %d levels\n", MAX_LEVELS);
            return NODAL_OK;
        }
        bool declined = false, stop = false;
        NODAL_TRY(build_level(h, H, l, hs, &declined, &stop));
        if (declined) {
            if (trace)
                fprintf(stderr, "[sagg] declined at level %d (%lld rows): does not coarsen / over a cap / not positive "
                                "(this level: overflow %llx baddiag %llx; level above: overflow %llx unassigned %llu maxr %llu)\n",
                        l, (long long)L->n, hs[(size_t)l * ST_COUNT + ST_OVERFLOW], hs[(size_t)l * ST_COUNT + ST_BADDIAG],
                        l > 0 ? hs[(size_t)(l - 1) * ST_COUNT + ST_OVERFLOW] : 0ull,
                        l > 0 ? hs[(size_t)(l - 1) * ST_COUNT + ST_UNASSIGNED] : 0ull,
                        l > 0 ? hs[(size_t)(l - 1) * ST_COUNT + ST_MAXR] : 0ull);
            return NODAL_OK;
        }
        if (stop) {
            diag_last = true;
            break;
        }
    }
    H->nlev = l + 1;
    SLevel *last = H->level(l);
    last->fold_want = last->fold = false;
    if (H->nlev < 2) return NODAL_OK;
    NODAL_HIP_TRY(h, hipMemcpyAsync(hs, dstats, (size_t)MAX_LEVELS * ST_COUNT * 8, hipMemcpyDeviceToHost, st));
    if (!H->ev_copy) NODAL_HIP_TRY(h, hipEventCreateWithFlags(&H->ev_copy, hipEventDisableTiming));
    NODAL_HIP_TRY(h, hipEventRecord(H->ev_copy, st));
    if (check_floating) {
        if (H->flags_levels == 0) {
            NODAL_HIP_TRY(h, H->level(0)->gflag.reserve((size_t)n0 + 64));
            NODAL_TRY(grounded_flags(h, H->level(0)->gflag.as<uint8_t>()));
        } else {
            NODAL_HIP_TRY(h, hipStreamWaitEvent(st, H->ev_flags, 0));
            H->aux_pending = false;
        }
        for (int k = H->flags_levels; k + 1 < H->nlev; ++k) {
            SLevel *L = H->pool[k], *C = H->pool[k + 1];
            NODAL_HIP_TRY(h, C->gflag.reserve((size_t)C->n + 64));
            NODAL_HIP_TRY(h, hipMemsetAsync(C->gflag.p, 0, ((size_t)C->n + 63) & ~(size_t)63, st));
            flags_up<<<grid_for(L->n), TB, 0, st>>>(L->n, L->agg.as<int32_t>(), L->gflag.as<uint8_t>(),
                                                   C->gflag.as<uint8_t>());
        }
        NODAL_HIP_TRY(h, hipGetLastError());
    }
    NODAL_WAIT_EVENT(h, H->ev_copy, st);
    for (int k = 0; k < H->nlev; ++k) {
        const unsigned long long *s = hs + (size_t)k * ST_COUNT;
        if (k > 0) {
            H->pool[k]->maxlen = (int32_t)s[ST_MAXLEN];
            H->pool[k]->nnz = (int64_t)s[ST_NNZ];
            H->pool[k]->wfix = choose_wfix(H->pool[k]->maxlen, H->pool[k]->n, H->pool[k]->nnz, APAD);
        }
        if (s[ST_OVERFLOW] || (k > 0 && s[ST_BADDIAG]) || s[ST_UNASSIGNED]) {
            if (trace) fprintf(stderr, "[sagg] declined: level %d over a cap / not positive\n", k);
            return NODAL_OK;
        }
    }
    diag_last = last->maxlen <= 1;
    H->dense_coarsest = !diag_last;
    if (H->dense_coarsest) {
        if (last->n > COARSEST) return NODAL_OK;
        NODAL_HIP_TRY(h, H->coarse_inv.reserve((size_t)last->n * last->n * 8 + 64));
        coarsest_inverse<<<1, 256, 0, st>>>(last->A(), H->coarse_inv.as<double>(),
                                            dstats + (size_t)l * ST_COUNT);
        NODAL_HIP_TRY(h, hipGetLastError());
    }
    for (int k = 0; k < H->nlev; ++k) {
        SLevel *L = H->pool[k];
        NODAL_HIP_TRY(h, L->vec.reserve((size_t)V_COUNT * L->ld * 8 + 256));
        NODAL_HIP_TRY(h, L->part.reserve(5 * DOT_BLOCKS * 8 + 512));
    }
    NODAL_TRY(build_tail(h, H, hs));

    if (!check_floating) {
        NODAL_HIP_TRY(h, hipMemcpyAsync(hs, dstats, (size_t)MAX_LEVELS * ST_COUNT * 8, hipMemcpyDeviceToHost, st));
        NODAL_WAIT_STREAM(h, st);
        if (hs[(size_t)l * ST_COUNT + ST_BADDIAG] & 2ull) return NODAL_OK;
    } else {
        uint32_t *fl = reinterpret_cast<uint32_t *>(dstats + (size_t)(MAX_LEVELS - 1) * ST_COUNT + ST_COUNT - 1);
        if (H->dense_coarsest) last_level_floating<<<1, 64, 0, st>>>(last->A(), last->gflag.as<uint8_t>(), fl);
        else any_unflagged<<<grid_for(last->n), TB, 0, st>>>(last->n, last->gflag.as<uint8_t>(), fl);
        NODAL_HIP_TRY(h, hipGetLastError());
        NODAL_HIP_TRY(h, hipMemcpyAsync(hs, dstats, (size_t)MAX_LEVELS * ST_COUNT * 8, hipMemcpyDeviceToHost, st));
        NODAL_WAIT_STREAM(h, st);
        if (hs[(size_t)l * ST_COUNT + ST_BADDIAG] & 2ull) {
            if (trace) fprintf(stderr, "[sagg] declined: coarsest matrix not positive definite\n");
            return NODAL_OK;
        }
        *floating = hs[(size_t)(MAX_LEVELS - 1) * ST_COUNT + ST_COUNT - 1] != 0 ? 1 : 0;
    }
    if (trace) {
        fprintf(stderr, "[sagg] levels (rows/entries/longest row/padded width):");
        for (int k = 0; k < H->nlev; ++k)
            fprintf(stderr, " %lld/%lld/%d/%d", (long long)H->pool[k]->n, (long long)H->pool[k]->nnz,
                    H->pool[k]->maxlen, H->pool[k]->wfix);
        fprintf(stderr, "  tail %d (%d register slots)  coarsest %s\n", H->tail, H->tail >= 0 ? H->td.slots : 0,
                H->dense_coarsest ? "dense" : "diagonal");
    }
    decide_folds(H, hs, trace);
    NODAL_TRY(fold_self_check(h, H));
    H->ready = true;
    *accepted = true;
    H->sym_valid = true;
    H->sym_epoch = h->struct_epoch;
    H->sym_n = n0;
    H->sym_nnz = nnz0;
    H->sym_general = general;
    H->sym_check = check_floating;
    H->sym_floating = *floating;
    memcpy(H->sym_stats, hs, sizeof H->sym_stats);
    return NODAL_OK;
}

int sagg_setup(nodal_ctx *h, bool *accepted, int32_t *floating) {
    return sagg_setup_csr(h, h->n, h->nnz, h->indptr.as<int32_t>(), h->indices.as<int32_t>(), h->data.as<double>(),
                          false, true, accepted, floating);
}

namespace {

int last_level(nodal_ctx *h, SHierarchy *H, int l, const double *b, double *out) {
    hipStream_t st = h->stream;
    SLevel *L = H->pool[l];
    const int64_t n = L->n;
    if (l == H->tail) return H->tail_dense ? tail_apply<1>(h, H, b, out) : tail_walk(h, H, b, out, 1);
    k_coarsest<<<grid_for(n), TB, 0, st>>>(n, H->dense_coarsest ? H->coarse_inv.as<double>() : nullptr,
                                           L->dinv.as<double>(), b, out);
    NODAL_HIP_TRY(h, hipGetLastError());
    return NODAL_OK;
}

void kcycle_schedule(SHierarchy *H, int it) {
    static const bool on = knob::SA_KFREEZE.now();
    H->kfrozen = false;
    H->kslot = -1;
    if (!on || it < 0) return;
    if (it == 0) H->ksamples = 0;
    const bool adaptive = it < 4 || (it & 3) == 0;
    if (!adaptive && H->ksamples > 0) {
        H->kfrozen = true;
    } else if (it >= 2) {
        H->kslot = H->ksamples % 3;
        ++H->ksamples;
        H->kcount = H->ksamples < 3 ? H->ksamples : 3;
    }
}

template <typename TBV, typename TOUT>
int cycle(nodal_ctx *h, SHierarchy *H, int l, const TBV *b, const cyc_t *x0, TOUT *out, const SolveBufs *sb) {
    hipStream_t st = h->stream;
    SLevel *L = H->pool[l];
    const int64_t n = L->n;
    SLevel *C = H->pool[l + 1];
    const int64_t nc = C->n;
    const Ell A = L->A();
    const double *dinv = L->dinv.as<double>();
    const cyc_t *x = x0;
    cyc_t *r = L->v<cyc_t>(V_R), *xp = L->v<cyc_t>(V_XP);
    const unsigned g = sb ? (unsigned)sb->g0 : grid_for(n);
    const unsigned tb = L->wfix ? TB : TB * LPR_RAGGED;
    const int nu = H->nu[l < 2 ? l : 2];
    const bool fold = L->fold && !(sb && nu == 1);
    auto hand_up = [&](const auto *c1, const auto *c2, const double *cf) {
        using TC = std::remove_cv_t<std::remove_pointer_t<decltype(c1)>>;
        if (!fold)
            k_prolong<TC><<<grid_for(n), TB, 0, st>>>(n, L->ld, L->pcol.as<int32_t>(), L->pvalf.as<float>(), x, c1, c2, cf, xp);
        else if (nu == 1)
            k_prolong_post<TC, TOUT><<<grid_for(n), TB, 0, st>>>(n, L->ld, L->wcol.as<int32_t>(), L->wval.as<float>(),
                                                               L->wlen.as<int32_t>(), x, r, dinv, c1, c2, cf, out);
        else
            k_prolong_post<TC, cyc_t><<<grid_for(n), TB, 0, st>>>(n, L->ld, L->wcol.as<int32_t>(), L->wval.as<float>(),
                                                                L->wlen.as<int32_t>(), x, r, dinv, c1, c2, cf, xp);
    };
    if (nu >= 2) {
        cyc_t *x1 = L->v<cyc_t>(V_X1);
        SAGG_DISPATCH_W(L->wfix, (k_post<W, false, TBV, cyc_t><<<g, tb, 0, st>>>(A, dinv, b, x0, x1, nullptr, nullptr, nullptr)));
        x = x1;
    }
    if (nu >= 3) {
        cyc_t *x2 = L->v<cyc_t>(V_T);
        SAGG_DISPATCH_W(L->wfix, (k_post<W, false, TBV, cyc_t><<<g, tb, 0, st>>>(A, dinv, b, x, x2, nullptr, nullptr, nullptr)));
        x = x2;
    }
    SAGG_DISPATCH_W(L->wfix, (k_smooth_residual<W, TBV><<<g, tb, 0, st>>>(A, b, x, r)));
    const bool last = l + 1 == H->tail || l + 1 == H->nlev - 1;
    const double *coef = nullptr;
    if (last) {
        double *rc = C->v<double>(V_RC), *c1 = C->v<double>(V_C1);
        k_restrict<double><<<grid_for(nc * RL), TB, 0, st>>>(nc, L->rld, L->rcol.as<int32_t>(), L->rvalf.as<float>(),
                                                            L->rlen.as<int32_t>(), r, rc, C->dinv.as<double>(), nullptr);
        NODAL_HIP_TRY(h, hipGetLastError());
        NODAL_TRY(last_level(h, H, l + 1, rc, c1));
        hand_up((const double *)c1, (const double *)nullptr, nullptr);
    } else {
        cyc_t *rc = C->v<cyc_t>(V_RC), *c1 = C->v<cyc_t>(V_C1), *c2 = C->v<cyc_t>(V_C2), *x0c = C->v<cyc_t>(V_X);
        k_restrict<cyc_t><<<grid_for(nc * RL), TB, 0, st>>>(nc, L->rld, L->rcol.as<int32_t>(), L->rvalf.as<float>(),
                                                           L->rlen.as<int32_t>(), r, rc, C->dinv.as<double>(), x0c);
        NODAL_HIP_TRY(h, hipGetLastError());
        int nparts = 0;
        const bool kcycle = l < H->klevels && H->kcycle;
        if (kcycle) {
            cyc_t *v1 = C->v<cyc_t>(V_V1), *v2 = C->v<cyc_t>(V_V2), *r2 = C->v<cyc_t>(V_R2);
            double *part = C->part.as<double>();
            const Ell Ac = C->A();
            const unsigned gd = grid_for(nc, DOT_BLOCKS);
            const unsigned tbc = C->wfix ? TB : TB * LPR_RAGGED;
            nparts = (int)gd;
            double *cf = part + 5 * DOT_BLOCKS;
            if (H->kfrozen && l == 0) {
                NODAL_TRY((cycle<cyc_t, cyc_t>(h, H, l + 1, rc, x0c, c1, nullptr)));
                SAGG_DISPATCH_W(C->wfix, (k_spmv_resid<W><<<gd, tbc, 0, st>>>(Ac, c1, rc, cf + 3, r2, C->dinv.as<double>(), x0c)));
                NODAL_HIP_TRY(h, hipGetLastError());
                NODAL_TRY((cycle<cyc_t, cyc_t>(h, H, l + 1, r2, x0c, c2, nullptr)));
                coef = cf + 3;
                nparts = 0;
            } else {
                NODAL_TRY((cycle<cyc_t, cyc_t>(h, H, l + 1, rc, x0c, c1, nullptr)));
                SAGG_DISPATCH_W(C->wfix, (k_spmv_dots<W><<<gd, tbc, 0, st>>>(Ac, c1, v1, rc, nullptr, part + 0 * DOT_BLOCKS,
                                                                            part + 1 * DOT_BLOCKS, nullptr)));
                k_second_residual<<<grid_for(nc), TB, 0, st>>>(nc, rc, v1, part, nparts, r2, C->dinv.as<double>(), x0c);
                NODAL_HIP_TRY(h, hipGetLastError());
                NODAL_TRY((cycle<cyc_t, cyc_t>(h, H, l + 1, r2, x0c, c2, nullptr)));
                SAGG_DISPATCH_W(C->wfix, (k_spmv_dots<W><<<gd, tbc, 0, st>>>(Ac, c2, v2, v1, r2, part + 3 * DOT_BLOCKS,
                                                                            part + 2 * DOT_BLOCKS, part + 4 * DOT_BLOCKS)));
                NODAL_HIP_TRY(h, hipGetLastError());
            }
        } else {
            NODAL_TRY((cycle<cyc_t, cyc_t>(h, H, l + 1, rc, x0c, c1, nullptr)));
        }
        if (nparts) {
            double *cf = C->part.as<double>() + 5 * DOT_BLOCKS;
            const bool sample = l == 0 && H->kslot >= 0;
            k_kcoef<<<1, 320, 0, st>>>(C->part.as<double>(), nparts, cf, sample ? H->kslot : -1, sample ? H->kcount : 0);
            coef = cf;
        }
        hand_up((const cyc_t *)c1, (const cyc_t *)c2, coef);
    }
    const cyc_t *cur = xp;
    const int left = fold ? nu - 1 : nu;
    if (left == 0) {
        NODAL_HIP_TRY(h, hipGetLastError());
        return NODAL_OK;
    }
    if (left >= 2) {
        cyc_t *mid = L->v<cyc_t>(V_T);
        SAGG_DISPATCH_W(L->wfix, (k_post<W, false, TBV, cyc_t><<<g, tb, 0, st>>>(A, dinv, b, cur, mid, nullptr, nullptr, nullptr)));
        cur = mid;
    }
    if (left >= 3) {
        cyc_t *mid2 = L->v<cyc_t>(V_X1);
        SAGG_DISPATCH_W(L->wfix, (k_post<W, false, TBV, cyc_t><<<g, tb, 0, st>>>(A, dinv, b, cur, mid2, nullptr, nullptr, nullptr)));
        cur = mid2;
    }
    if (sb) {
        SAGG_DISPATCH_W(L->wfix, (k_post<W, true, TBV, TOUT><<<g, tb, 0, st>>>(A, dinv, b, cur, out, sb->Ap, sb->part_rz,
                                                                              sb->part_zap)));
    } else {
        SAGG_DISPATCH_W(L->wfix, (k_post<W, false, TBV, TOUT><<<g, tb, 0, st>>>(A, dinv, b, cur, out, nullptr, nullptr, nullptr)));
    }
    NODAL_HIP_TRY(h, hipGetLastError());
    return NODAL_OK;
}

__global__ void f_set_scalars(double *__restrict__ sc, double tol2) {
    for (int k = 0; k < F_COUNT; ++k) sc[k] = 0.0;
    sc[F_TOL2] = tol2;
}

size_t align_up(size_t x) { return (x + 255) & ~(size_t)255; }

}

__global__ __launch_bounds__(TB) void k_x0(int64_t n, const double *__restrict__ dinv, const double *__restrict__ r,
                                           cyc_t *__restrict__ x0) {
    for (int64_t i = (int64_t)xcd_block() * TB + threadIdx.x; i < n; i += (int64_t)gridDim.x * TB)
        x0[i] = (cyc_t)(OMEGA * dinv[i] * r[i]);
}
bool sagg_ready(nodal_ctx *h, int64_t n) {
    SHierarchy *H = static_cast<SHierarchy *>(h->sagg);
    return H && H->ready && H->pool[0]->n == n;
}
void sagg_invalidate(nodal_ctx *h) {
    if (h->sagg) static_cast<SHierarchy *>(h->sagg)->ready = false;
}
int sagg_levels(nodal_ctx *h) { return h->sagg ? static_cast<SHierarchy *>(h->sagg)->nlev : 0; }
bool sagg_x0_slot(nodal_ctx *h, const double **dinv, nodal_cyc_t **x0, int64_t *n0, double *omega) {
    SHierarchy *H = static_cast<SHierarchy *>(h->sagg);
    if (!H || !H->ready) return false;
    SLevel *L0 = H->pool[0];
    *dinv = L0->dinv.as<double>();
    *x0 = L0->v<cyc_t>(V_X);
    *n0 = L0->n;
    *omega = OMEGA;
    return true;
}
int sagg_apply(nodal_ctx *h, const double *r, double *z, bool x0_ready, int it) {
    SHierarchy *H = static_cast<SHierarchy *>(h->sagg);
    if (!H || !H->ready) return nodal_fail(h, NODAL_E_INVALID, "sagg_setup_csr not called");
    SLevel *L0 = H->pool[0];
    cyc_t *x0 = L0->v<cyc_t>(V_X);
    if (!x0_ready) k_x0<<<grid_for(L0->n), TB, 0, h->stream>>>(L0->n, L0->dinv.as<double>(), r, x0);
    NODAL_HIP_TRY(h, hipGetLastError());
    kcycle_schedule(H, it);
    const int rc = cycle<double, double>(h, H, 0, r, x0, z, nullptr);
    H->kfrozen = false;
    H->kslot = -1;
    return rc;
}

int sagg_spmv(nodal_ctx *h, const double *x, double *y, hipEvent_t start, hipEvent_t stop) {
    SHierarchy *H = static_cast<SHierarchy *>(h->sagg);
    if (!H || !H->ready) return nodal_fail(h, NODAL_E_INVALID, "sagg_setup_csr not called");
    const SLevel *L0 = H->pool[0];
    const Ell A0 = L0->A();
    const unsigned tb0 = L0->wfix ? TB : TB * LPR_RAGGED;
    if (start && stop) {
        SAGG_DISPATCH_W(L0->wfix, (hipExtLaunchKernelGGL((k_ell_spmv<W>), dim3(grid_for(L0->n)), dim3(tb0), 0, h->stream,
                                                         start, stop, 0, A0, x, y)));
    } else {
        SAGG_DISPATCH_W(L0->wfix, (k_ell_spmv<W><<<grid_for(L0->n), tb0, 0, h->stream>>>(A0, x, y)));
    }
    NODAL_HIP_TRY(h, hipGetLastError());
    return NODAL_OK;
}

int sagg_fcg_solve(nodal_ctx *h, const double *b, bool do_setup, int32_t *info, int32_t *iters, double *resid) {
    static const bool trace = knob::TRACE.now();
    const int64_t n = h->n;
    hipStream_t st = h->stream;
    SHierarchy *H = hierarchy_of(h);
    if (do_setup) {
        bool accepted = false;
        int32_t floating = 0;
        NODAL_TRY(sagg_setup(h, &accepted, &floating));
        if (!accepted) return SAGG_DECLINED;
        if (floating) {
            *info = 1;
            *iters = 0;
            *resid = 0.0;
            return -2;
        }
    }
    if (!H->ready || H->pool[0]->n != n) return SAGG_DECLINED;
    h->amg_levels = H->nlev;
    static const int kc = knob::SA_KCYCLE.now();
    H->kcycle = kc != 0;
    H->klevels = knob::SA_KLEVELS.now();
    if (const char *e = knob::SA_NU.now()) {
        for (int k = 0; k < 3 && e[k] >= '1' && e[k] <= '3'; ++k) H->nu[k] = e[k] - '0';
    }

    const size_t vec = align_up((size_t)n * 8);
    NODAL_HIP_TRY(h, h->solver.reserve(6 * vec + 4 * MAX_PARTIALS * 8 + F_COUNT * 8 + 256));
    char *base = h->solver.as<char>();
    SolveBufs sb;
    sb.r = reinterpret_cast<double *>(base);
    sb.z = reinterpret_cast<cyc_t *>(base + vec);
    sb.p = reinterpret_cast<double *>(base + 2 * vec);
    sb.Ap = reinterpret_cast<double *>(base + 3 * vec);
    sb.x0 = reinterpret_cast<cyc_t *>(base + 4 * vec);
    sb.p2 = reinterpret_cast<double *>(base + 5 * vec);
    sb.part_rz = reinterpret_cast<double *>(base + 6 * vec);
    sb.part_zap = sb.part_rz + MAX_PARTIALS;
    sb.part_rr = sb.part_zap + MAX_PARTIALS;
    sb.part_pap = sb.part_rr + MAX_PARTIALS;
    sb.sc = sb.part_pap + MAX_PARTIALS;
    sb.g0 = (int)grid_for(n, MAX_PARTIALS);
    double *x = h->x.as<double>();
    const Ell A0 = H->pool[0]->A();

    const double tol = 1e-13;
    f_set_scalars<<<1, 1, 0, st>>>(sb.sc, tol * tol);
    const double *dinv0 = H->pool[0]->dinv.as<double>();
    f_init<<<sb.g0, TB, 0, st>>>(b, x, sb.r, sb.Ap, dinv0, sb.x0, sb.part_rr, n);
    NODAL_HIP_TRY(h, hipGetLastError());

    const int64_t maxit = knob::FCG_MAXIT.now().value_or(2000);
    hipEvent_t e0 = h->ev[2], e1 = h->ev[3];
    h->kern_ms = 0;
    h->kern_launches = 0;
    double hs[F_COUNT];
    int64_t enqueued = 0;
    int batch = 6;
    if (H->last_iters > 6 && (H->refreshed || !do_setup)) batch = H->last_iters + 1 > 32 ? 32 : H->last_iters + 1;
    else if (H->hint_iters > 8 && H->hint_n == n && H->hint_nnz == H->pool[0]->nnz) {
        batch = (3 * H->hint_iters) / 4;
        if (batch > 32) batch = 32;
    }
    int status = 0;
    const bool poll_partials = knob::FCG_HOST_SUM.now();
    double rr_prev = -1.0;
    int64_t it_prev = 0;
    int polls = 0;
    static const bool fuse_dir_env = knob::SA_FUSE_DIR.now();
    const bool fuse_dir = fuse_dir_env && LPR_RAGGED == 1;
    static const bool graphs_env = knob::SA_GRAPH.now();
    auto iteration = [&](int it, bool timed) -> int {
        kcycle_schedule(H, graphs_env ? -1 : it);
        struct KReset {
            SHierarchy *H;
            ~KReset() { H->kfrozen = false; H->kslot = -1; }
        } kreset{H};
        NODAL_TRY((cycle<double, cyc_t>(h, H, 0, sb.r, sb.x0, sb.z, &sb)));
        if (fuse_dir) {
            double *p_new = (it & 1) ? sb.p2 : sb.p;
            const double *p_old = (it & 1) ? sb.p : sb.p2;
            const unsigned tbf = TB;
            if (timed) {
                SAGG_DISPATCH_W(H->pool[0]->wfix, (hipExtLaunchKernelGGL((f_dir_spmv<W>), dim3(sb.g0), dim3(tbf), 0, st, e0, e1, 0,
                                                                         A0, (const cyc_t *)sb.z, p_old, p_new, sb.Ap,
                                                                         (const double *)sb.part_rz, (const double *)sb.part_zap,
                                                                         (const double *)sb.part_rr, sb.g0, sb.part_pap, sb.sc,
                                                                         it & 1)));
            } else {
                SAGG_DISPATCH_W(H->pool[0]->wfix, (f_dir_spmv<W><<<sb.g0, tbf, 0, st>>>(A0, sb.z, p_old, p_new, sb.Ap, sb.part_rz,
                                                                                       sb.part_zap, sb.part_rr, sb.g0,
                                                                                       sb.part_pap, sb.sc, it & 1)));
            }
            f_update<<<sb.g0, TB, 0, st>>>(x, sb.r, p_new, sb.Ap, sb.part_pap, sb.g0, dinv0, sb.x0, sb.part_rr, sb.sc, it & 1, n);
            NODAL_HIP_TRY(h, hipGetLastError());
            return NODAL_OK;
        }
        f_direction<<<sb.g0, TB, 0, st>>>(sb.z, sb.p, sb.part_rz, sb.part_zap, sb.part_rr, sb.g0, sb.sc, it & 1, n);
        const unsigned tb0 = H->pool[0]->wfix ? TB : TB * LPR_RAGGED;
        if (timed) {
            SAGG_DISPATCH_W(H->pool[0]->wfix, (hipExtLaunchKernelGGL((f_spmv<W>), dim3(sb.g0), dim3(tb0), 0, st, e0, e1, 0,
                                                                     A0, (const double *)sb.p, sb.Ap, sb.part_pap,
                                                                     (const double *)sb.sc, it & 1)));
        } else {
            SAGG_DISPATCH_W(H->pool[0]->wfix, (f_spmv<W><<<sb.g0, tb0, 0, st>>>(A0, sb.p, sb.Ap, sb.part_pap, sb.sc, it & 1)));
        }
        f_update<<<sb.g0, TB, 0, st>>>(x, sb.r, sb.p, sb.Ap, sb.part_pap, sb.g0, dinv0, sb.x0, sb.part_rr, sb.sc, it & 1, n);
        NODAL_HIP_TRY(h, hipGetLastError());
        return NODAL_OK;
    };
    static const bool graphs = knob::SA_GRAPH.now();
    if (graphs && (H->refreshed || !do_setup)) {
        uint64_t key = 1469598103934665603ull;
        auto mix = [&](uint64_t v) { key = (key ^ v) * 1099511628211ull; };
        mix((uint64_t)(uintptr_t)base); mix((uint64_t)(uintptr_t)x); mix((uint64_t)n); mix((uint64_t)sb.g0);
        mix((uint64_t)H->nlev); mix((uint64_t)(H->tail + 1)); mix((uint64_t)H->kcycle); mix((uint64_t)H->klevels);
        mix((uint64_t)(H->nu[0] * 100 + H->nu[1] * 10 + H->nu[2])); mix((uint64_t)H->td.lds_bytes);
        mix((uint64_t)(uintptr_t)H->tail_image.p); mix((uint64_t)(uintptr_t)H->coarse_inv.p);
        mix((uint64_t)(uintptr_t)(H->tail_dense ? H->tail_op.p : nullptr));
        for (int k = 0; k < H->nlev; ++k) {
            const SLevel *L = H->pool[k];
            const void *ps[] = {L->acol.p, L->aval.p, L->avalf.p, L->alen.p, L->dinv.p, L->pcol.p, L->pvalf.p,
                                L->rcol.p, L->rvalf.p, L->rlen.p, L->vec.p, L->part.p};
            for (const void *q : ps) mix((uint64_t)(uintptr_t)q);
            mix((uint64_t)(L->fold ? 1 + L->wslots : 0));
            if (L->fold) { mix((uint64_t)(uintptr_t)L->wcol.p); mix((uint64_t)(uintptr_t)L->wval.p); mix((uint64_t)(uintptr_t)L->wlen.p); }
            mix((uint64_t)L->n); mix((uint64_t)L->ld); mix((uint64_t)L->wfix); mix((uint64_t)L->rld);
        }
        if (H->it_exec && H->it_key != key) H->drop_graph();
        if (!H->it_exec) {
            hipGraph_t g = nullptr;
            hipGraphExec_t ex = nullptr;
            if (hipStreamBeginCapture(st, hipStreamCaptureModeThreadLocal) == hipSuccess) {
                int cs = iteration(0, false);
                if (cs == NODAL_OK) cs = iteration(1, false);
                const hipError_t ce = hipStreamEndCapture(st, &g);
                if (cs == NODAL_OK && ce == hipSuccess && g && hipGraphInstantiate(&ex, g, nullptr, nullptr, 0) == hipSuccess) {
                    H->it_graph = g;
                    H->it_exec = ex;
                    H->it_key = key;
                } else {
                    if (g) (void)hipGraphDestroy(g);
                    (void)hipGetLastError();
                }
            } else {
                (void)hipGetLastError();
            }
        }
    } else if (H->it_exec && do_setup) {
        H->drop_graph();
    }
    while (status == 0) {
        for (int c = 0; c < batch;) {
            if (H->it_exec && c > 0 && c + 1 < batch && (enqueued & 1) == 0) {
                NODAL_HIP_TRY(h, hipGraphLaunch(H->it_exec, st));
                c += 2;
                enqueued += 2;
            } else {
                NODAL_TRY(iteration((int)enqueued, c == 0));
                ++c;
                ++enqueued;
            }
        }
        double rr_now = -1.0;
        {
            const size_t bytes = (size_t)(2 * MAX_PARTIALS + F_COUNT) * 8;
            double *stage = poll_partials ? static_cast<double *>(nodal_pinned_arena(h, bytes)) : nullptr;
            if (stage) {
                NODAL_HIP_TRY(h, hipMemcpyAsync(stage, sb.part_rr, bytes, hipMemcpyDeviceToHost, st));
                NODAL_WAIT_STREAM(h, st);
                memcpy(hs, stage + 2 * MAX_PARTIALS, F_COUNT * 8);
                double acc = 0.0;
                for (int k = 0; k < sb.g0; ++k) acc += stage[k];
                rr_now = acc;
            } else {
                NODAL_TRY(nodal_read_words(h, hs, sb.sc, F_COUNT * 8));
            }
        }
        ++polls;
        bool conv = hs[F_CONV + ((enqueued - 1) & 1)] != 0.0;
        bool host_conv = false;
        if (!conv && rr_now >= 0.0 && hs[F_FLAG] == 0.0 && hs[F_BB] > 0.0 && rr_now <= tol * tol * hs[F_BB]) {
            host_conv = true;
            hs[F_RR] = rr_now;
            hs[F_ITERS] = (double)enqueued;
        } else if (!conv && rr_now >= 0.0) {
            hs[F_RR] = rr_now;
        }
        float ms = 0;
        if (!(conv && !host_conv && hs[F_ITERS] <= (double)(enqueued - batch)) && hipEventElapsedTime(&ms, e0, e1) == hipSuccess) {
            h->kern_ms += ms;
            h->kern_launches += 1;
        }
        if (hs[F_FLAG] != 0.0 || !(hs[F_RR] == hs[F_RR])) status = 2;
        else if (conv || host_conv) status = 1;
        else if (enqueued >= maxit) status = 3;
        else {
            int next = 2;
            const double target = tol * tol * hs[F_BB];
            const double rr_ref = rr_prev > 0.0 ? rr_prev : hs[F_BB];
            const int64_t it_ref = rr_prev > 0.0 ? it_prev : 0;
            if (hs[F_RR] > 0.0 && hs[F_RR] < rr_ref && enqueued > it_ref) {
                const double rate = log(hs[F_RR] / rr_ref) / (double)(enqueued - it_ref);
                static const double look = knob::FCG_LOOK.now();
                next = (int)floor(look * log(target / hs[F_RR]) / rate);
            }
            if (next > enqueued) next = (int)enqueued;
            batch = next < 1 ? 1 : (next > 32 ? 32 : next);
            rr_prev = hs[F_RR];
            it_prev = enqueued;
        }
    }
    const int64_t its = status == 1 ? (int64_t)hs[F_ITERS] : enqueued;
    *iters = (int32_t)its;
    *resid = hs[F_BB] > 0 ? sqrt(hs[F_RR] / hs[F_BB]) : 0.0;
    const SLevel *L0 = H->pool[0];
    h->kern_alg = 12.0 * (double)L0->nnz + 4.0 * (double)n + 16.0 * (double)n;
    if (fuse_dir) h->kern_alg += 12.0 * (double)n;
    if (trace)
        fprintf(stderr, "[sagg] %d iterations (%lld enqueued, %d polls), relative residual %.2e, status %d\n", *iters,
                (long long)enqueued, polls, *resid, status);
    if (trace && H->tail >= 0 && H->td.stamps && !H->tail_dense) {
        long long ts[64];
        if (hipMemcpy(ts, H->td.stamps, sizeof ts, hipMemcpyDeviceToHost) == hipSuccess) {
            fprintf(stderr, "[sagg] tail phases (us):");
            for (int k = 1; k < (int)ts[63] && k < 63; ++k) fprintf(stderr, " %.2f", (double)(ts[k] - ts[k - 1]) * 0.01);
            fprintf(stderr, "  total %.2f, image %d B, lds %d B\n", (double)(ts[ts[63] - 1] - ts[0]) * 0.01,
                    H->td.image_bytes, H->td.lds_bytes);
            for (int k = 0; k < H->td.nlev; ++k)
                fprintf(stderr, "[sagg]   tail level %d: n %d width %d lpr %d nq %d\n", k, H->td.lv[k].n,
                        H->td.lv[k].width, H->td.lv[k].lpr, H->td.lv[k].nq);
        }
    }
    if (status != 1) {
        H->last_iters = 0;
        return -1;
    }
    H->last_iters = (int)its;
    H->hint_iters = (int)its;
    H->hint_n = n;
    H->hint_nnz = H->pool[0]->nnz;
    *info = 0;
    return NODAL_OK;
}

#include "sagg_multi.h"
```

### nodal_amd/csrc/sagg_cycle.h

```cpp
#pragma once

namespace {

constexpr int LPR_RAGGED = 1;
template <int W> struct RowLanes { static constexpr int value = W == 0 ? LPR_RAGGED : 1; };

template <class VT, class XF>
__device__ __forceinline__ double ell_row_lanes(const Ell &A, const VT *__restrict__ val, int64_t i, int sub, XF xf) {
    constexpr int Q = 8;
    const int32_t len = A.len[i];
    double acc = 0.0;
    for (int32_t s0 = sub; s0 < len; s0 += LPR_RAGGED * Q) {
        int32_t c[Q];
        double v[Q];
        if (A.dcol) {
#pragma unroll
            for (int q = 0; q < Q; ++q) {
                const bool ok = s0 + q * LPR_RAGGED < len;
                const int64_t at = (int64_t)(ok ? s0 + q * LPR_RAGGED : s0) * A.ld + i;
                c[q] = (int32_t)i + (int32_t)A.dcol[at];
                const VT loaded = val[at];
                v[q] = ok ? (double)loaded : 0.0;
            }
        } else {
#pragma unroll
            for (int q = 0; q < Q; ++q) {
                const bool ok = s0 + q * LPR_RAGGED < len;
                const int64_t at = (int64_t)(ok ? s0 + q * LPR_RAGGED : s0) * A.ld + i;
                c[q] = A.col[at];
                const VT loaded = val[at];
                v[q] = ok ? (double)loaded : 0.0;
            }
        }
#pragma unroll
        for (int q = 0; q < Q; ++q) acc = fma(v[q], xf(c[q]), acc);
    }
#pragma unroll
    for (int off = LPR_RAGGED >> 1; off > 0; off >>= 1) acc += __shfl_xor(acc, off, 64);
    return acc;
}

template <int W, class VT, class XF>
__device__ __forceinline__ double ell_row_w(const Ell &A, const VT *__restrict__ val, int64_t i, int sub, XF xf) {
    if constexpr (W == 0) {
        return ell_row_lanes(A, val, i, sub, xf);
    } else {
        int32_t c[W];
        double v[W];
        if (A.dcol) {
#pragma unroll
            for (int q = 0; q < W; ++q) {
                c[q] = (int32_t)i + (int32_t)A.dcol[(int64_t)q * A.ld + i];
                v[q] = (double)val[(int64_t)q * A.ld + i];
            }
        } else {
#pragma unroll
            for (int q = 0; q < W; ++q) {
                c[q] = A.col[(int64_t)q * A.ld + i];
                v[q] = (double)val[(int64_t)q * A.ld + i];
            }
        }
        double acc = 0.0;
#pragma unroll
        for (int q = 0; q < W; ++q) acc = fma(v[q], xf(c[q]), acc);
        return acc;
    }
}

template <int W, class VT>
__device__ __forceinline__ void ell_row_load(const Ell &A, const VT *__restrict__ val, int64_t i, int32_t (&c)[W > 0 ? W : 1],
                                             VT (&v)[W > 0 ? W : 1]) {
    if (A.dcol) {
#pragma unroll
        for (int q = 0; q < W; ++q) {
            c[q] = (int32_t)A.dcol[(int64_t)q * A.ld + i];
            v[q] = val[(int64_t)q * A.ld + i];
        }
    } else {
#pragma unroll
        for (int q = 0; q < W; ++q) {
            c[q] = A.col[(int64_t)q * A.ld + i] - (int32_t)i;
            v[q] = val[(int64_t)q * A.ld + i];
        }
    }
}
template <int W, class VT, class XF>
__device__ __forceinline__ double ell_row_sum(int64_t i, const int32_t (&c)[W > 0 ? W : 1], const VT (&v)[W > 0 ? W : 1], XF xf) {
    double acc = 0.0;
#pragma unroll
    for (int q = 0; q < W; ++q) acc = fma((double)v[q], xf((int32_t)i + c[q]), acc);
    return acc;
}

#define SAGG_DISPATCH_W(w, CALL)                         \
    switch (w) {                                         \
    case 4: { constexpr int W = 4; CALL; } break;        \
    case 5: { constexpr int W = 5; CALL; } break;        \
    case 6: { constexpr int W = 6; CALL; } break;        \
    case 8: { constexpr int W = 8; CALL; } break;        \
    case 12: { constexpr int W = 12; CALL; } break;      \
    case 16: { constexpr int W = 16; CALL; } break;      \
    case 20: { constexpr int W = 20; CALL; } break;      \
    case 24: { constexpr int W = 24; CALL; } break;      \
    case 32: { constexpr int W = 32; CALL; } break;      \
    default: { constexpr int W = 0; CALL; } break;       \
    }

__device__ __forceinline__ double wave_sum(double v) {
#pragma unroll
    for (int off = 32; off > 0; off >>= 1) v += __shfl_down(v, off, 64);
    return v;
}
template <int NT = TB>
__device__ __forceinline__ double block_sum(double v) {
    __shared__ double ws[NT / 64];
    __syncthreads();
    v = wave_sum(v);
    if ((threadIdx.x & 63) == 0) ws[threadIdx.x >> 6] = v;
    __syncthreads();
    double s = 0.0;
#pragma unroll
    for (int w = 0; w < NT / 64; ++w) s += ws[w];
    return s;
}
__device__ __forceinline__ double reduce_partials(const double *__restrict__ part, int count) {
    double s = 0.0;
    for (int i = threadIdx.x; i < count; i += TB) s += part[i];
    return block_sum(s);
}
__device__ __forceinline__ void reduce_partials3(const double *__restrict__ pa, const double *__restrict__ pb,
                                                 const double *__restrict__ pc, int count, double &ra, double &rb,
                                                 double &rc) {
    __shared__ double ws[3][TB / 64];
    double a = 0.0, b = 0.0, c = 0.0;
    for (int i = threadIdx.x; i < count; i += TB) {
        a += pa[i];
        b += pb[i];
        if (pc) c += pc[i];
    }
    __syncthreads();
    a = wave_sum(a);
    b = wave_sum(b);
    c = wave_sum(c);
    if ((threadIdx.x & 63) == 0) {
        ws[0][threadIdx.x >> 6] = a;
        ws[1][threadIdx.x >> 6] = b;
        ws[2][threadIdx.x >> 6] = c;
    }
    __syncthreads();
    ra = rb = rc = 0.0;
#pragma unroll
    for (int w = 0; w < TB / 64; ++w) {
        ra += ws[0][w];
        rb += ws[1][w];
        rc += ws[2][w];
    }
}

template <int W, typename TBV>
__global__ __launch_bounds__(TB * RowLanes<W>::value) void k_smooth_residual(Ell A, const TBV *__restrict__ b,
                                                        const cyc_t *__restrict__ x0, cyc_t *__restrict__ r) {
    constexpr int LPR = RowLanes<W>::value, NT = TB * LPR;
    const int sub = threadIdx.x & (LPR - 1);
    for (int64_t t = (int64_t)xcd_block() * NT + threadIdx.x; t / LPR < A.n; t += (int64_t)gridDim.x * NT) {
        const int64_t i = t / LPR;
        const double s = ell_row_w<W>(A, A.valf, i, sub, [&](int32_t j) { return (double)x0[j]; });
        if (sub == 0) r[i] = (cyc_t)((double)b[i] - s);
    }
}

constexpr int RL = 8;
template <typename TO>
__global__ __launch_bounds__(TB) void k_restrict(int64_t nc, int64_t rld, const int32_t *__restrict__ rcol,
                                                 const float *__restrict__ rval, const int32_t *__restrict__ rlen,
                                                 const cyc_t *__restrict__ r, TO *__restrict__ rc,
                                                 const double *__restrict__ cdinv, cyc_t *__restrict__ x0c) {
    const int sub = threadIdx.x & (RL - 1);
    const int64_t rows_per_pass = (int64_t)gridDim.x * (TB / RL);
    for (int64_t I0 = (int64_t)xcd_block() * (TB / RL); I0 < nc; I0 += rows_per_pass) {
        const int64_t I = I0 + threadIdx.x / RL;
        double s = 0.0;
        if (I < nc) {
            const int32_t len = rlen[I];
            constexpr int RU = 6;
            for (int32_t q0 = 0; q0 * RL < len; q0 += RU) {
                int32_t c[RU];
                double v[RU];
#pragma unroll
                for (int u = 0; u < RU; ++u) {
                    const bool ok = (q0 + u) * RL < len;
                    const int64_t at = ((int64_t)(ok ? q0 + u : q0) * rld + I) * RL + sub;
                    c[u] = rcol[at];
                    const float loaded = rval[at];
                    v[u] = ok ? (double)loaded : 0.0;
                }
#pragma unroll
                for (int u = 0; u < RU; ++u) s = fma(v[u], (double)r[c[u]], s);
            }
        }
#pragma unroll
        for (int off = RL >> 1; off > 0; off >>= 1) s += __shfl_down(s, off, RL);
        if (I < nc && sub == 0) {
            rc[I] = (TO)s;
            if (x0c) x0c[I] = (cyc_t)(OMEGA * cdinv[I] * s);
        }
    }
}

struct KCoef { double s1, s2; };
__device__ __forceinline__ KCoef kcycle_coefficients(const double *__restrict__ part, int nparts) {
    if (nparts == 0) return KCoef{1.0, 0.0};
    const double rho1 = reduce_partials(part + 0 * DOT_BLOCKS, nparts);
    const double alpha1 = reduce_partials(part + 1 * DOT_BLOCKS, nparts);
    const double gamma = reduce_partials(part + 2 * DOT_BLOCKS, nparts);
    const double beta = reduce_partials(part + 3 * DOT_BLOCKS, nparts);
    const double alpha2 = reduce_partials(part + 4 * DOT_BLOCKS, nparts);
    if (!(rho1 > 0.0)) return KCoef{0.0, 0.0};
    const double rho2 = beta - gamma * gamma / rho1;
    if (!(rho2 > 0.0)) return KCoef{alpha1 / rho1, 0.0};
    return KCoef{alpha1 / rho1 - gamma * alpha2 / (rho1 * rho2), alpha2 / rho2};
}

__global__ __launch_bounds__(320) void k_kcoef(const double *__restrict__ part, int nparts, double *__restrict__ coef,
                                               int slot, int count) {
    __shared__ double d[5];
    const int w = threadIdx.x >> 6, lane = threadIdx.x & 63;
    double s = 0.0;
    for (int i = lane; i < nparts; i += 64) s += part[w * DOT_BLOCKS + i];
    s = wave_sum(s);
    if (lane == 0) d[w] = s;
    __syncthreads();
    if (threadIdx.x == 0) {
        const double rho1 = d[0], alpha1 = d[1], gamma = d[2], beta = d[3], alpha2 = d[4];
        double s1 = 0.0, s2 = 0.0;
        if (rho1 > 0.0) {
            const double rho2 = beta - gamma * gamma / rho1;
            if (rho2 > 0.0) {
                s1 = alpha1 / rho1 - gamma * alpha2 / (rho1 * rho2);
                s2 = alpha2 / rho2;
            } else {
                s1 = alpha1 / rho1;
            }
        }
        coef[0] = s1;
        coef[1] = s2;
        if (slot >= 0) {
            double *ring = coef + 6;
            ring[3 * slot + 0] = s1;
            ring[3 * slot + 1] = s2;
            ring[3 * slot + 2] = rho1 > 0.0 ? alpha1 / rho1 : 0.0;
            double m0 = 0.0, m1 = 0.0, m2 = 0.0;
            for (int q = 0; q < count; ++q) {
                m0 += ring[3 * q + 0];
                m1 += ring[3 * q + 1];
                m2 += ring[3 * q + 2];
            }
            coef[3] = m0 / count;
            coef[4] = m1 / count;
            coef[5] = m2 / count;
        }
    }
}

template <int W>
__global__ __launch_bounds__(TB * RowLanes<W>::value) void k_spmv_resid(Ell A, const cyc_t *__restrict__ c,
                                                   const cyc_t *__restrict__ rc, const double *__restrict__ frz,
                                                   cyc_t *__restrict__ r2, const double *__restrict__ dinv,
                                                   cyc_t *__restrict__ x0) {
    constexpr int LPR = RowLanes<W>::value, NT = TB * LPR;
    const int sub = threadIdx.x & (LPR - 1);
    const double t = frz[2];
    for (int64_t tt = (int64_t)xcd_block() * NT + threadIdx.x; tt / LPR < A.n; tt += (int64_t)gridDim.x * NT) {
        const int64_t i = tt / LPR;
        const double sd = ell_row_w<W>(A, A.valf, i, sub, [&](int32_t j) { return (double)c[j]; });
        if (sub != 0) continue;
        const double v = fma(-t, (double)(cyc_t)sd, (double)rc[i]);
        r2[i] = (cyc_t)v;
        x0[i] = (cyc_t)(OMEGA * dinv[i] * v);
    }
}

template <typename TC>
__global__ __launch_bounds__(TB) void k_prolong(int64_t n, int64_t ld, const int32_t *__restrict__ pcol,
                                                const float *__restrict__ pval, const cyc_t *__restrict__ x,
                                                const TC *__restrict__ c1, const TC *__restrict__ c2,
                                                const double *__restrict__ coef, cyc_t *__restrict__ xp) {
    const bool two = coef != nullptr;
    const double s1 = two ? coef[0] : 1.0, s2 = two ? coef[1] : 0.0;
    for (int64_t i = (int64_t)xcd_block() * TB + threadIdx.x; i < n; i += (int64_t)gridDim.x * TB) {
        int32_t J[PW];
        double w[PW];
#pragma unroll
        for (int q = 0; q < PW; ++q) {
            J[q] = pcol[(int64_t)q * ld + i];
            w[q] = (double)pval[(int64_t)q * ld + i];
        }
        double s = (double)x[i];
#pragma unroll
        for (int q = 0; q < PW; ++q) {
            const int32_t j = J[q] < 0 ? 0 : J[q];
            const double e = two ? s1 * (double)c1[j] + s2 * (double)c2[j] : (double)c1[j];
            s = fma(J[q] < 0 ? 0.0 : w[q], e, s);
        }
        xp[i] = (cyc_t)s;
    }
}

template <int W, bool DOTS, typename TBV, typename TOUT>
__global__ __launch_bounds__(TB * RowLanes<W>::value) void k_post(Ell A, const double *__restrict__ dinv, const TBV *__restrict__ b,
                                             const cyc_t *__restrict__ xp, TOUT *__restrict__ out,
                                             const double *__restrict__ u, double *__restrict__ p_ob,
                                             double *__restrict__ p_ou) {
    double a0 = 0.0, a1 = 0.0;
    constexpr int LPR = RowLanes<W>::value, NT = TB * LPR;
    const int sub = threadIdx.x & (LPR - 1);
    for (int64_t t = (int64_t)xcd_block() * NT + threadIdx.x; t / LPR < A.n; t += (int64_t)gridDim.x * NT) {
        const int64_t i = t / LPR;
        const double s = ell_row_w<W>(A, A.valf, i, sub, [&](int32_t j) { return (double)xp[j]; });
        if (sub != 0) continue;
        const double bi = (double)b[i];
        const TOUT os = (TOUT)fma(OMEGA * dinv[i], bi - s, (double)xp[i]);
        const double o = (double)os;
        out[i] = os;
        if (DOTS) {
            a0 = fma(o, bi, a0);
            a1 = fma(o, u[i], a1);
        }
    }
    if (DOTS) {
        a0 = block_sum<NT>(a0);
        a1 = block_sum<NT>(a1);
        if (threadIdx.x == 0) {
            p_ob[blockIdx.x] = a0;
            p_ou[blockIdx.x] = a1;
        }
    }
}

template <typename TC, typename TOUT>
__global__ __launch_bounds__(TB) void k_prolong_post(int64_t n, int64_t ld, const int32_t *__restrict__ wcol,
                                                     const float *__restrict__ wval, const int32_t *__restrict__ wlen,
                                                     const cyc_t *__restrict__ x, const cyc_t *__restrict__ r,
                                                     const double *__restrict__ dinv, const TC *__restrict__ c1,
                                                     const TC *__restrict__ c2, const double *__restrict__ coef,
                                                     TOUT *__restrict__ out) {
    constexpr int Q = 8;
    const bool two = coef != nullptr;
    const double s1 = two ? coef[0] : 1.0, s2 = two ? coef[1] : 0.0;
    for (int64_t i = (int64_t)xcd_block() * TB + threadIdx.x; i < n; i += (int64_t)gridDim.x * TB) {
        const int32_t len = wlen[i];
        const cyc_t xi = x[i], ri = r[i];
        const double di = dinv[i];
        double acc = 0.0;
        for (int32_t s0 = 0; s0 < len; s0 += Q) {
            int32_t J[Q];
            double w[Q];
#pragma unroll
            for (int q = 0; q < Q; ++q) {
                const bool ok = s0 + q < len;
                const int64_t at = (int64_t)(ok ? s0 + q : s0) * ld + i;
                J[q] = wcol[at];
                const float loaded = wval[at];
                w[q] = ok ? (double)loaded : 0.0;
            }
#pragma unroll
            for (int q = 0; q < Q; ++q) {
                const double e = two ? s1 * (double)c1[J[q]] + s2 * (double)c2[J[q]] : (double)c1[J[q]];
                acc = fma(w[q], e, acc);
            }
        }
        out[i] = (TOUT)(fma(OMEGA * di, (double)ri, (double)xi) + acc);
    }
}

template <typename TC>
__global__ __launch_bounds__(TB) void k_fold_check(Ell A, const double *__restrict__ dinv, const cyc_t *__restrict__ b,
                                                   const cyc_t *__restrict__ x, const cyc_t *__restrict__ xp,
                                                   const int32_t *__restrict__ wcol, const float *__restrict__ wval,
                                                   const int32_t *__restrict__ wlen, const TC *__restrict__ c1,
                                                   const TC *__restrict__ c2, const double *__restrict__ coef,
                                                   const cyc_t *__restrict__ m_two, const cyc_t *__restrict__ m_fused,
                                                   double *__restrict__ d, double *__restrict__ q) {
    const bool two = coef != nullptr;
    const double s1 = two ? coef[0] : 1.0, s2 = two ? coef[1] : 0.0;
    for (int64_t i = (int64_t)xcd_block() * TB + threadIdx.x; i < A.n; i += (int64_t)gridDim.x * TB) {
        double ax = 0.0, we = 0.0;
        const int32_t la = A.len[i], lw = wlen[i];
        for (int32_t s = 0; s < la; ++s)
            ax += fabs((double)A.valf[(int64_t)s * A.ld + i]) * fabs((double)xp[A.col[(int64_t)s * A.ld + i]]);
        for (int32_t s = 0; s < lw; ++s) {
            const int32_t j = wcol[(int64_t)s * A.ld + i];
            const double e = two ? s1 * (double)c1[j] + s2 * (double)c2[j] : (double)c1[j];
            we += fabs((double)wval[(int64_t)s * A.ld + i]) * fabs(e);
        }
        const double den = fabs((double)x[i]) + OMEGA * dinv[i] * (fabs((double)b[i]) + ax) + we;
        const double diff = fabs((double)m_fused[i] - (double)m_two[i]);
        const double di = diff / den;
        d[i] = di;
        q[i] = di / ((double)(lw + la + 8) * 0x1p-23);
    }
}

template <int W>
__global__ __launch_bounds__(TB * RowLanes<W>::value) void k_spmv_dots(Ell A, const cyc_t *__restrict__ c, cyc_t *__restrict__ v,
                                                  const cyc_t *__restrict__ u1, const cyc_t *__restrict__ u2,
                                                  double *__restrict__ p_cv, double *__restrict__ p_cu1,
                                                  double *__restrict__ p_cu2) {
    double a0 = 0.0, a1 = 0.0, a2 = 0.0;
    constexpr int LPR = RowLanes<W>::value, NT = TB * LPR;
    const int sub = threadIdx.x & (LPR - 1);
    for (int64_t t = (int64_t)xcd_block() * NT + threadIdx.x; t / LPR < A.n; t += (int64_t)gridDim.x * NT) {
        const int64_t i = t / LPR;
        const double sd = ell_row_w<W>(A, A.valf, i, sub, [&](int32_t j) { return (double)c[j]; });
        if (sub != 0) continue;
        const cyc_t vs = (cyc_t)sd;
        v[i] = vs;
        const double s = (double)vs, ci = (double)c[i];
        a0 = fma(ci, s, a0);
        a1 = fma(ci, (double)u1[i], a1);
        if (u2) a2 = fma(ci, (double)u2[i], a2);
    }
    a0 = block_sum<NT>(a0);
    a1 = block_sum<NT>(a1);
    a2 = block_sum<NT>(a2);
    if (threadIdx.x == 0) {
        p_cv[blockIdx.x] = a0;
        p_cu1[blockIdx.x] = a1;
        if (p_cu2) p_cu2[blockIdx.x] = a2;
    }
}

__global__ __launch_bounds__(TB) void k_second_residual(int64_t n, const cyc_t *__restrict__ rc,
                                                        const cyc_t *__restrict__ v1,
                                                        const double *__restrict__ part, int nparts,
                                                        cyc_t *__restrict__ r2, const double *__restrict__ dinv,
                                                        cyc_t *__restrict__ x0) {
    double rho1, alpha1, unused;
    reduce_partials3(part + 0 * DOT_BLOCKS, part + 1 * DOT_BLOCKS, nullptr, nparts, rho1, alpha1, unused);
    const double t = rho1 > 0.0 ? alpha1 / rho1 : 0.0;
    for (int64_t i = (int64_t)xcd_block() * TB + threadIdx.x; i < n; i += (int64_t)gridDim.x * TB)
    {
        const double v = fma(-t, (double)v1[i], (double)rc[i]);
        r2[i] = (cyc_t)v;
        x0[i] = (cyc_t)(OMEGA * dinv[i] * v);
    }
}

__global__ __launch_bounds__(TB) void k_coarsest(int64_t n, const double *__restrict__ inv,
                                                 const double *__restrict__ dinv, const double *__restrict__ b,
                                                 double *__restrict__ out) {
    for (int64_t i = (int64_t)xcd_block() * TB + threadIdx.x; i < n; i += (int64_t)gridDim.x * TB) {
        double s = 0.0;
        if (inv)
            for (int64_t j = 0; j < n; ++j) s = fma(inv[i * n + j], b[j], s);
        else
            s = dinv[i] * b[i];
        out[i] = s;
    }
}



__device__ __forceinline__ double lds_row(const double *aval, const uint16_t *acol, int n, int width, int i,
                                          int sub, int lpr, const double *x) {
    double s0 = 0.0, s1 = 0.0;
    int t = sub;
    for (; t + 3 * lpr < width; t += 4 * lpr) {
        const double v0 = aval[t * n + i], v1 = aval[(t + lpr) * n + i], v2 = aval[(t + 2 * lpr) * n + i],
                     v3 = aval[(t + 3 * lpr) * n + i];
        const int c0 = acol[t * n + i], c1 = acol[(t + lpr) * n + i], c2 = acol[(t + 2 * lpr) * n + i],
                  c3 = acol[(t + 3 * lpr) * n + i];
        s0 = fma(v0, x[c0], s0);
        s1 = fma(v1, x[c1], s1);
        s0 = fma(v2, x[c2], s0);
        s1 = fma(v3, x[c3], s1);
    }
    for (; t < width; t += lpr) s0 = fma(aval[t * n + i], x[acol[t * n + i]], s0);
    double s = s0 + s1;
    for (int off = lpr >> 1; off > 0; off >>= 1) s += __shfl_xor(s, off, 64);
    return s;
}

__global__ __launch_bounds__(1024) void k_tail_pack(TailDesc d, char *__restrict__ image) {
    const int tid = threadIdx.x;
    const int last = d.nlev - 1;
    auto f64 = [&](int off) { return reinterpret_cast<double *>(image + off); };
    auto u16 = [&](int off) { return reinterpret_cast<uint16_t *>(image + off); };
    auto copy_f64 = [&](double *dst, const double *src, int rows, int64_t ld, int slots) {
        for (int e = tid; e < rows * slots; e += 1024) {
            const int t = e / rows, i = e - t * rows;
            dst[e] = src[(int64_t)t * ld + i];
        }
    };
    auto copy_u16 = [&](uint16_t *dst, const int32_t *src, int rows, int64_t ld, int slots) {
        for (int e = tid; e < rows * slots; e += 1024) {
            const int t = e / rows, i = e - t * rows;
            const int32_t v = src[(int64_t)t * ld + i];
            dst[e] = (uint16_t)(v < 0 ? 0 : v);
        }
    };
    for (int k = 0; k < last; ++k) {
        const TailLevelDesc &L = d.lv[k];
        for (int e = tid; e < L.n * L.width; e += 1024) {
            const int t = e / L.n, i = e - t * L.n;
            const bool in = t < L.alen[i];
            f64(L.o_aval)[e] = in ? L.aval[(int64_t)t * L.ld + i] : 0.0;
            const int32_t c = in ? L.acol[(int64_t)t * L.ld + i] : 0;
            u16(L.o_acol)[e] = (uint16_t)(c < 0 ? 0 : c);
        }
        copy_f64(f64(L.o_dinv), L.dinv, L.n, L.ld, 1);
        copy_f64(f64(L.o_pval), L.pval, L.n, L.ld, PW);
        copy_u16(u16(L.o_pcol), L.pcol, L.n, L.ld, PW);
        copy_f64(f64(L.o_rval), L.rval, L.nc * RL, (int64_t)L.rld * RL, L.nq);
        copy_u16(u16(L.o_rcol), L.rcol, L.nc * RL, (int64_t)L.rld * RL, L.nq);
    }
    const TailLevelDesc &L = d.lv[last];
    if (d.inv) copy_f64(f64(L.o_aval), d.inv, L.n * L.n, L.n * L.n, 1);
    else copy_f64(f64(L.o_aval), L.dinv, L.n, L.n, 1);
}

template <int SLOTS>
__device__ __forceinline__ double reg_row(const double (&v)[SLOTS], const uint32_t (&c)[SLOTS / 2], int lpr,
                                          const double *x) {
    double s0 = 0.0, s1 = 0.0;
#pragma unroll
    for (int j = 0; j < SLOTS; j += 2) {
        s0 = fma(v[j], x[c[j / 2] & 0xffffu], s0);
        s1 = fma(v[j + 1], x[c[j / 2] >> 16], s1);
    }
    double s = s0 + s1;
    for (int off = lpr >> 1; off > 0; off >>= 1) s += __shfl_xor(s, off, 64);
    return s;
}

template <int SLOTS, bool UNIT>
__device__ __forceinline__ void tail_cycle(const TailDesc &d, char *smem, const char *__restrict__ image,
                                           const double *__restrict__ rc, double *__restrict__ out, int vs, int voff) {
    const int tid = threadIdx.x;
    const int last = d.nlev - 1;
    const int TAIL_NU = d.nu;
    auto f64 = [&](int off) { return reinterpret_cast<double *>(smem + (off - d.skip)); };
    auto u16 = [&](int off) { return reinterpret_cast<uint16_t *>(smem + (off - d.skip)); };
    int stamp_no = 0;
    auto stamp = [&]() {
        if (!UNIT && d.stamps && tid == 0) d.stamps[stamp_no] = wall_clock64();
        ++stamp_no;
    };
    stamp();
    double v0[SLOTS];
    uint32_t c0[SLOTS / 2];
    {
        const TailLevelDesc &L = d.lv[0];
        const double *aval = reinterpret_cast<const double *>(image + L.o_aval);
        const uint16_t *acol = reinterpret_cast<const uint16_t *>(image + L.o_acol);
        const int lpr = L.lpr, sub = tid & (lpr - 1), i = tid / lpr, ii = i < L.n ? i : L.n - 1;
        const bool row = last > 0 && i < L.n;
#pragma unroll
        for (int j = 0; j < SLOTS; j += 2) {
            const int ta = sub + j * lpr, tb = ta + lpr;
            const bool ha = row && ta < L.width, hb = row && tb < L.width;
            const int ea = ha ? ta * L.n + ii : 0, eb = hb ? tb * L.n + ii : 0;
            const double va = aval[ea], vb = aval[eb];
            const uint32_t ca = acol[ea], cb = acol[eb];
            v0[j] = ha ? va : 0.0;
            v0[j + 1] = hb ? vb : 0.0;
            c0[j / 2] = (ha ? ca : 0u) | ((hb ? cb : 0u) << 16);
        }
    }
    {
        constexpr int FLY = (TAIL_LDS_BUDGET / 16 + 1023) / 1024;
        const int4 *src = reinterpret_cast<const int4 *>(image + d.skip);
        int4 *dst = reinterpret_cast<int4 *>(smem);
        const int pieces = (d.image_bytes - d.skip) / 16;
        int4 v[FLY];
#pragma unroll
        for (int u = 0; u < FLY; ++u) v[u] = src[tid + u * 1024 < pieces ? tid + u * 1024 : 0];
#pragma unroll
        for (int u = 0; u < FLY; ++u)
            if (tid + u * 1024 < pieces) dst[tid + u * 1024] = v[u];
    }
    for (;;) {
        for (int i = tid; i < d.lv[0].n; i += 1024)
            f64(d.lv[0].o_B)[i] = UNIT ? (i == voff ? 1.0 : 0.0) : rc[(int64_t)i * vs + voff];
        __syncthreads();
        stamp();
        for (int k = 0; k < last; ++k) {
            const TailLevelDesc &L = d.lv[k];
            const double *aval = f64(L.o_aval), *dinv = f64(L.o_dinv), *B = f64(L.o_B);
            const uint16_t *acol = u16(L.o_acol);
            double *X = f64(L.o_X), *Y = f64(L.o_Y), *R = f64(L.o_R);
            const int lpr = L.lpr, sub = tid & (lpr - 1), rows = 1024 / lpr;
            for (int i = tid; i < L.n; i += 1024) X[i] = OMEGA * dinv[i] * B[i];
            __syncthreads();
            for (int sweep = 1; sweep < TAIL_NU; ++sweep) {
                for (int i0 = 0; i0 < L.n; i0 += rows) {
                    const int i = i0 + tid / lpr, ii = i < L.n ? i : L.n - 1;
                    const double ax = k == 0 ? reg_row<SLOTS>(v0, c0, lpr, X)
                                             : lds_row(aval, acol, L.n, L.width, ii, sub, lpr, X);
                    if (i < L.n && sub == 0) Y[i] = fma(OMEGA * dinv[i], B[i] - ax, X[i]);
                }
                __syncthreads();
                double *t = X; X = Y; Y = t;
            }
            for (int i0 = 0; i0 < L.n; i0 += rows) {
                const int i = i0 + tid / lpr, ii = i < L.n ? i : L.n - 1;
                const double ax = k == 0 ? reg_row<SLOTS>(v0, c0, lpr, X)
                                         : lds_row(aval, acol, L.n, L.width, ii, sub, lpr, X);
                if (i < L.n && sub == 0) R[i] = B[i] - ax;
            }
            __syncthreads();
            stamp();
            const double *rval = f64(L.o_rval);
            const uint16_t *rcol = u16(L.o_rcol);
            double *Bc = f64(d.lv[k + 1].o_B);
            for (int I0 = 0; I0 < L.nc; I0 += 1024 / RL) {
                const int I = I0 + tid / RL, r8 = tid & (RL - 1);
                double s = 0.0;
                if (I < L.nc) {
                    double s1 = 0.0;
                    const int e0 = I * RL + r8, step = L.nc * RL;
                    int q = 0;
                    for (; q + 3 < L.nq; q += 4) {
                        const int ea = e0 + q * step, eb = ea + step, ec = eb + step, ed = ec + step;
                        const double va = rval[ea], vb = rval[eb], vc = rval[ec], vd = rval[ed];
                        const int ca = rcol[ea], cb = rcol[eb], cc = rcol[ec], cd = rcol[ed];
                        s = fma(va, R[ca], s);
                        s1 = fma(vb, R[cb], s1);
                        s = fma(vc, R[cc], s);
                        s1 = fma(vd, R[cd], s1);
                    }
                    for (; q < L.nq; ++q) s = fma(rval[e0 + q * step], R[rcol[e0 + q * step]], s);
                    s += s1;
                }
#pragma unroll
                for (int off = RL >> 1; off > 0; off >>= 1) s += __shfl_xor(s, off, 64);
                if (I < L.nc && r8 == 0) Bc[I] = s;
            }
            __syncthreads();
            stamp();
        }
        {
            const TailLevelDesc &L = d.lv[last];
            const double *inv = f64(L.o_aval), *B = f64(L.o_B);
            double *E = f64(L.o_X);
            for (int i = tid; i < L.n; i += 1024) {
                double s = 0.0;
                if (d.inv) {
                    double s1 = 0.0, s2 = 0.0, s3 = 0.0;
                    const double *row = inv + i * L.n;
                    int j = 0;
                    for (; j + 3 < L.n; j += 4) {
                        s = fma(row[j], B[j], s);
                        s1 = fma(row[j + 1], B[j + 1], s1);
                        s2 = fma(row[j + 2], B[j + 2], s2);
                        s3 = fma(row[j + 3], B[j + 3], s3);
                    }
                    for (; j < L.n; ++j) s = fma(row[j], B[j], s);
                    s = (s + s1) + (s2 + s3);
                } else {
                    s = inv[i] * B[i];
                }
                E[i] = s;
            }
            __syncthreads();
            stamp();
        }
        const double *Ec = f64(d.lv[last].o_X);
        for (int k = last - 1; k >= 0; --k) {
            const TailLevelDesc &L = d.lv[k];
            const double *aval = f64(L.o_aval), *dinv = f64(L.o_dinv), *B = f64(L.o_B), *pval = f64(L.o_pval);
            const uint16_t *acol = u16(L.o_acol), *pcol = u16(L.o_pcol);
            double *X = f64((TAIL_NU & 1) ? L.o_X : L.o_Y), *Y = f64((TAIL_NU & 1) ? L.o_Y : L.o_X);
            for (int i = tid; i < L.n; i += 1024) {
                double s = X[i];
#pragma unroll
                for (int q = 0; q < PW; ++q) s = fma(pval[q * L.n + i], Ec[pcol[q * L.n + i]], s);
                Y[i] = s;
            }
            __syncthreads();
            stamp();
            const int lpr = L.lpr, sub = tid & (lpr - 1), rows = 1024 / lpr;
            for (int sweep = 0; sweep < TAIL_NU; ++sweep) {
                for (int i0 = 0; i0 < L.n; i0 += rows) {
                    const int i = i0 + tid / lpr, ii = i < L.n ? i : L.n - 1;
                    const double ax = k == 0 ? reg_row<SLOTS>(v0, c0, lpr, Y)
                                             : lds_row(aval, acol, L.n, L.width, ii, sub, lpr, Y);
                    if (i < L.n && sub == 0) X[i] = fma(OMEGA * dinv[i], B[i] - ax, Y[i]);
                }
                __syncthreads();
                double *t = X; X = Y; Y = t;
            }
            Ec = Y;
            stamp();
        }
        for (int i = tid; i < d.lv[0].n; i += 1024) out[(int64_t)i * vs + voff] = Ec[i];
        stamp();
        voff += (int)gridDim.x;
        if (!UNIT || voff >= d.lv[0].n) break;
        __syncthreads();
    }
    if (!UNIT && d.stamps && tid == 0) d.stamps[63] = stamp_no;
}

template <int SLOTS>
__global__ __launch_bounds__(1024) void k_tail(TailDesc d, const char *__restrict__ image,
                                               const double *__restrict__ rc, double *__restrict__ out, int vs) {
    extern __shared__ __attribute__((aligned(16))) char smem[];
    tail_cycle<SLOTS, false>(d, smem, image, rc, out, vs, vs > 1 ? (int)blockIdx.x : 0);
}

template <int SLOTS>
__global__ __launch_bounds__(1024) void k_tail_pack_op(TailDesc d, const char *__restrict__ image,
                                                       double *__restrict__ T) {
    extern __shared__ __attribute__((aligned(16))) char smem[];
    tail_cycle<SLOTS, true>(d, smem, image, nullptr, T, d.lv[0].n, (int)blockIdx.x);
}

template <int CH, int NV>
__global__ __launch_bounds__(256) void k_tail_apply(int n, const double *__restrict__ T,
                                                    const double *__restrict__ rc, double *__restrict__ out) {
    const int lane = threadIdx.x & 63;
    const int i = (int)blockIdx.x * 4 + (threadIdx.x >> 6);
    if (i >= n) return;
    const double *row = T + (int64_t)i * n;
    double t[CH];
#pragma unroll
    for (int u = 0; u < CH; ++u) {
        const int j = lane + 64 * u;
        t[u] = row[j < n ? j : 0];
    }
    if constexpr (NV == 1) {
        double r[CH];
#pragma unroll
        for (int u = 0; u < CH; ++u) {
            const int j = lane + 64 * u;
            r[u] = rc[j < n ? j : 0];
        }
        double s0 = 0.0, s1 = 0.0;
#pragma unroll
        for (int u = 0; u < CH; u += 2) {
            if (lane + 64 * u < n && t[u] != 0.0) s0 = fma(t[u], r[u], s0);
            if (lane + 64 * (u + 1) < n && t[u + 1] != 0.0) s1 = fma(t[u + 1], r[u + 1], s1);
        }
        const double s = wave_sum(s0 + s1);
        if (lane == 0) out[i] = s;
    } else {
        double s[NV];
#pragma unroll
        for (int c = 0; c < NV; ++c) s[c] = 0.0;
#pragma unroll
        for (int u = 0; u < CH; ++u) {
            const int j = lane + 64 * u;
            const double *rj = rc + (int64_t)(j < n ? j : 0) * NV;
            const bool use = j < n && t[u] != 0.0;
#pragma unroll
            for (int c = 0; c < NV; ++c) {
                const double v = rj[c];
                if (use) s[c] = fma(t[u], v, s[c]);
            }
        }
#pragma unroll
        for (int c = 0; c < NV; ++c) {
            const double v = wave_sum(s[c]);
            if (lane == 0) out[(int64_t)i * NV + c] = v;
        }
    }
}

enum { F_RZ = 0, F_ALPHA = 2, F_CONV = 4, F_RR = 6, F_BB = 7, F_FLAG = 8, F_ITERS = 9, F_TOL2 = 10,
       F_ITNO = 12,
       F_COUNT = 16 };
constexpr int MAX_PARTIALS = 1024;

__global__ __launch_bounds__(TB) void f_init(const double *__restrict__ b, double *__restrict__ x,
                                             double *__restrict__ r, double *__restrict__ Ap,
                                             const double *__restrict__ dinv, cyc_t *__restrict__ x0,
                                             double *__restrict__ part_rr, int64_t n) {
    double srr = 0.0;
    for (int64_t i = (int64_t)xcd_block() * TB + threadIdx.x; i < n; i += (int64_t)gridDim.x * TB) {
        const double ri = b[i];
        x[i] = 0.0;
        r[i] = ri;
        x0[i] = (cyc_t)(OMEGA * dinv[i] * ri);
        Ap[i] = 0.0;
        srr = fma(ri, ri, srr);
    }
    srr = block_sum(srr);
    if (threadIdx.x == 0) part_rr[blockIdx.x] = srr;
}

__global__ __launch_bounds__(TB) void f_direction(const cyc_t *__restrict__ z, double *__restrict__ p,
                                                  const double *__restrict__ part_rz,
                                                  const double *__restrict__ part_zap,
                                                  const double *__restrict__ part_rr, int nparts,
                                                  double *__restrict__ sc, int parity, int64_t n) {
    const int cur = parity & 1, prev = cur ^ 1;
    constexpr int FD_PRE = 4;
    const int64_t i0 = (int64_t)xcd_block() * TB + threadIdx.x, stride = (int64_t)gridDim.x * TB;
    cyc_t zq[FD_PRE];
    double pq[FD_PRE];
#pragma unroll
    for (int u = 0; u < FD_PRE; ++u) {
        const int64_t i = i0 + u * stride, ii = i < n ? i : n - 1;
        zq[u] = z[ii];
        pq[u] = p[ii];
    }
    const int iter = (int)sc[F_ITNO + prev];
    if (blockIdx.x == 0 && threadIdx.x == 0) sc[F_ITNO + cur] = (double)(iter + 1);
    if (iter > 0 && sc[F_CONV + prev] != 0.0) {
        if (blockIdx.x == 0 && threadIdx.x == 0) sc[F_CONV + cur] = 1.0;
        return;
    }
    double rz_new, zap, rr;
    reduce_partials3(part_rz, part_zap, part_rr, nparts, rz_new, zap, rr);
    const double rz_old = iter > 0 ? sc[F_RZ + prev] : 1.0;
    const double beta = (iter > 0 && rz_old != 0.0) ? -sc[F_ALPHA + prev] * zap / rz_old : 0.0;
    const double bb = iter == 0 ? rr : sc[F_BB];
    const bool bad = !(rz_new >= 0.0) || !(rr == rr);
    const bool converged = bb == 0.0 || rr <= sc[F_TOL2] * bb || bad;
    if (blockIdx.x == 0 && threadIdx.x == 0) {
        sc[F_RZ + cur] = rz_new;
        sc[F_RR] = rr;
        if (iter == 0) sc[F_BB] = rr;
        if (bad) sc[F_FLAG] = 1.0;
        sc[F_CONV + cur] = converged ? 1.0 : 0.0;
        if (converged) sc[F_ITERS] = (double)iter;
    }
    if (converged) return;
#pragma unroll
    for (int u = 0; u < FD_PRE; ++u) {
        const int64_t i = i0 + u * stride;
        if (i < n) p[i] = iter > 0 ? fma(beta, pq[u], (double)zq[u]) : (double)zq[u];
    }
    for (int64_t i = i0 + FD_PRE * stride; i < n; i += stride)
        p[i] = iter > 0 ? fma(beta, p[i], (double)z[i]) : (double)z[i];
}

template <int W>
__global__ __launch_bounds__(TB * RowLanes<W>::value) void k_ell_spmv(Ell A, const double *__restrict__ x,
                                                                      double *__restrict__ y) {
    constexpr int LPR = RowLanes<W>::value, NT = TB * LPR;
    const int sub = threadIdx.x & (LPR - 1);
    for (int64_t t = (int64_t)xcd_block() * NT + threadIdx.x; t / LPR < A.n; t += (int64_t)gridDim.x * NT) {
        const int64_t i = t / LPR;
        const double s = ell_row_w<W>(A, A.val, i, sub, [&](int32_t j) { return x[j]; });
        if (sub == 0) y[i] = s;
    }
}

template <int W>
__global__ __launch_bounds__(TB * RowLanes<W>::value) void f_spmv(Ell A, const double *__restrict__ p, double *__restrict__ Ap,
                                             double *__restrict__ part_pap, const double *__restrict__ sc,
                                             int iter) {
    if (sc[F_CONV + (iter & 1)] != 0.0) return;
    double acc = 0.0;
    constexpr int LPR = RowLanes<W>::value, NT = TB * LPR;
    const int sub = threadIdx.x & (LPR - 1);
    for (int64_t t = (int64_t)xcd_block() * NT + threadIdx.x; t / LPR < A.n; t += (int64_t)gridDim.x * NT) {
        const int64_t i = t / LPR;
        const double s = ell_row_w<W>(A, A.val, i, sub, [&](int32_t j) { return p[j]; });
        if (sub != 0) continue;
        Ap[i] = s;
        acc = fma(p[i], s, acc);
    }
    acc = block_sum<NT>(acc);
    if (threadIdx.x == 0) part_pap[blockIdx.x] = acc;
}

template <int W>
__global__ __launch_bounds__(TB * RowLanes<W>::value) void f_dir_spmv(Ell A, const cyc_t *__restrict__ z,
                                                 const double *__restrict__ p_old, double *__restrict__ p_new,
                                                 double *__restrict__ Ap, const double *__restrict__ part_rz,
                                                 const double *__restrict__ part_zap, const double *__restrict__ part_rr,
                                                 int nparts, double *__restrict__ part_pap, double *__restrict__ sc,
                                                 int parity) {
    static_assert(RowLanes<W>::value == 1, "the reduction of the partials assumes TB threads");
    const int cur = parity & 1, prev = cur ^ 1;
    const int64_t i0 = (int64_t)xcd_block() * TB + threadIdx.x, stride = (int64_t)gridDim.x * TB;
    int32_t c0[W > 0 ? W : 1];
    double v0[W > 0 ? W : 1];
    const int64_t ifirst = i0 < A.n ? i0 : A.n - 1;
    if constexpr (W > 0) ell_row_load<W>(A, A.val, ifirst, c0, v0);
    const cyc_t zfirst = z[ifirst];
    const double pfirst = p_old[ifirst];
    const int iter = (int)sc[F_ITNO + prev];
    if (blockIdx.x == 0 && threadIdx.x == 0) sc[F_ITNO + cur] = (double)(iter + 1);
    if (iter > 0 && sc[F_CONV + prev] != 0.0) {
        if (blockIdx.x == 0 && threadIdx.x == 0) sc[F_CONV + cur] = 1.0;
        return;
    }
    double rz_new, zap, rr;
    reduce_partials3(part_rz, part_zap, part_rr, nparts, rz_new, zap, rr);
    const double rz_old = iter > 0 ? sc[F_RZ + prev] : 1.0;
    const double beta = (iter > 0 && rz_old != 0.0) ? -sc[F_ALPHA + prev] * zap / rz_old : 0.0;
    const double bb = iter == 0 ? rr : sc[F_BB];
    const bool bad = !(rz_new >= 0.0) || !(rr == rr);
    const bool converged = bb == 0.0 || rr <= sc[F_TOL2] * bb || bad;
    if (blockIdx.x == 0 && threadIdx.x == 0) {
        sc[F_RZ + cur] = rz_new;
        sc[F_RR] = rr;
        if (iter == 0) sc[F_BB] = rr;
        if (bad) sc[F_FLAG] = 1.0;
        sc[F_CONV + cur] = converged ? 1.0 : 0.0;
        if (converged) sc[F_ITERS] = (double)iter;
    }
    if (converged) return;
    const bool first = iter == 0;
    auto pn = [&](int32_t j) { return first ? (double)z[j] : fma(beta, p_old[j], (double)z[j]); };
    double acc = 0.0;
    for (int64_t i = i0; i < A.n; i += stride) {
        double s, pi;
        if (W > 0 && i == i0) {
            s = ell_row_sum<W>(i, c0, v0, pn);
            pi = first ? (double)zfirst : fma(beta, pfirst, (double)zfirst);
        } else {
            s = ell_row_w<W>(A, A.val, i, 0, pn);
            pi = pn((int32_t)i);
        }
        p_new[i] = pi;
        Ap[i] = s;
        acc = fma(pi, s, acc);
    }
    acc = block_sum<TB>(acc);
    if (threadIdx.x == 0) part_pap[blockIdx.x] = acc;
}

__global__ __launch_bounds__(TB) void f_update(double *__restrict__ x, double *__restrict__ r,
                                               const double *__restrict__ p, const double *__restrict__ Ap,
                                               const double *__restrict__ part_pap, int nparts,
                                               const double *__restrict__ dinv, cyc_t *__restrict__ x0,
                                               double *__restrict__ part_rr, double *__restrict__ sc, int iter,
                                               int64_t n) {
    const int cur = iter & 1;
    constexpr int FU_PRE = 4;
    const int64_t i0 = (int64_t)xcd_block() * TB + threadIdx.x, stride = (int64_t)gridDim.x * TB;
    double xq[FU_PRE], rq[FU_PRE], pq[FU_PRE], aq[FU_PRE], dq[FU_PRE];
#pragma unroll
    for (int u = 0; u < FU_PRE; ++u) {
        const int64_t i = i0 + u * stride, ii = i < n ? i : n - 1;
        xq[u] = x[ii];
        rq[u] = r[ii];
        pq[u] = p[ii];
        aq[u] = Ap[ii];
        dq[u] = dinv[ii];
    }
    if (sc[F_CONV + cur] != 0.0) return;
    const double pap = reduce_partials(part_pap, nparts);
    const double rz = sc[F_RZ + cur];
    const bool bad = !(pap > 0.0) && rz != 0.0;
    const double alpha = (pap > 0.0) ? rz / pap : 0.0;
    if (blockIdx.x == 0 && threadIdx.x == 0) {
        sc[F_ALPHA + cur] = alpha;
        if (bad) sc[F_FLAG] = 1.0;
    }
    double srr = 0.0;
#pragma unroll
    for (int u = 0; u < FU_PRE; ++u) {
        const int64_t i = i0 + u * stride;
        if (i < n) {
            x[i] = fma(alpha, pq[u], xq[u]);
            const double ri = fma(-alpha, aq[u], rq[u]);
            r[i] = ri;
            x0[i] = (cyc_t)(OMEGA * dq[u] * ri);
            srr = fma(ri, ri, srr);
        }
    }
    for (int64_t i = i0 + FU_PRE * stride; i < n; i += stride) {
        x[i] = fma(alpha, p[i], x[i]);
        const double ri = fma(-alpha, Ap[i], r[i]);
        r[i] = ri;
        x0[i] = (cyc_t)(OMEGA * dinv[i] * ri);
        srr = fma(ri, ri, srr);
    }
    srr = block_sum(srr);
    if (threadIdx.x == 0) part_rr[blockIdx.x] = srr;
}

}
```

Before: 165.3 circuits/s.

## Trim AMG setup launches: sharded stats, fused MIS first round, fused CSR-to-ELL

Adds a bitmask knob, on by default with value 29 (stats, MIS, scalars and rows), that removes several small kernel launches from the smoothed-aggregation setup and solve start. Per-block stats now go into 64 atomic shards that the host folds, replacing the single-block reduce_bstat kernels. The first MIS round computes initial hashes inline, which drops mis_init. Row stats and the CSR-to-ELL conversion are fused into one kernel, and f_init now sets the solver scalars so f_set_scalars is no longer launched. The trade-off is atomic contention on the shards, a larger host copy of the stats buffer, and the correctness of the f_set_scalars replacement resting on f_init zeroing the scalars it previously set.

Result: faster. 167.0 circuits/s (median of 5 runs) (+1.0%).

```diff
diff --git a/nodal_amd/csrc/knobs.h b/nodal_amd/csrc/knobs.h
--- a/nodal_amd/csrc/knobs.h
+++ b/nodal_amd/csrc/knobs.h
@@ -120,6 +120,7 @@
 inline constexpr OnUnless0 SA_TAIL_DENSE{"NODAL_SA_TAIL_DENSE"};
 inline constexpr OffUnlessNon0 SA_TAIL_CHECK{"NODAL_SA_TAIL_CHECK"};
 inline constexpr Int SA_TAIL_NU{"NODAL_SA_TAIL_NU", 3};
+inline constexpr Int SA_LEAN{"NODAL_SA_LEAN", 29};
 inline constexpr Present TAIL_PROBE{"NODAL_TAIL_PROBE"};
 inline constexpr IntIfSet AMG_PASSES0{"NODAL_AMG_PASSES0"};
 inline constexpr IntIfSet AMG_PASSES1{"NODAL_AMG_PASSES1"};
diff --git a/nodal_amd/csrc/sagg.hip b/nodal_amd/csrc/sagg.hip
--- a/nodal_amd/csrc/sagg.hip
+++ b/nodal_amd/csrc/sagg.hip
@@ -40,6 +40,12 @@
     return (unsigned)(g > cap ? cap : g);
 }
 inline int64_t pad64(int64_t n) { return (n + 63) & ~(int64_t)63; }
+
+enum { LEAN_STATS = 1, LEAN_MIS = 4, LEAN_SCALARS = 8, LEAN_ROWS = 16 };
+inline bool lean(int item) {
+    static const int mask = knob::SA_LEAN.now();
+    return (mask & item) != 0;
+}
 inline size_t align256(size_t x) { return (x + 255) & ~(size_t)255; }
 
 __device__ __forceinline__ unsigned xcd_block() {
@@ -193,6 +199,41 @@
 
 
 constexpr int BSTAT_MAX = 65536;
+
+constexpr int STAT_SHARDS = 64;
+enum { SH_LEN = 0 , SH_SUM = 1 , SH_MAXR = 2 ,
+       SH_KINDS = 3 };
+constexpr size_t STATS_WORDS = (size_t)MAX_LEVELS * ST_COUNT + (size_t)MAX_LEVELS * SH_KINDS * STAT_SHARDS;
+constexpr size_t STATS_BYTES = STATS_WORDS * 8;
+inline unsigned long long *shards_of(unsigned long long *dstats, int level) {
+    return dstats + (size_t)MAX_LEVELS * ST_COUNT + (size_t)level * SH_KINDS * STAT_SHARDS;
+}
+__device__ __forceinline__ void shard_put(unsigned long long *__restrict__ shard, int kind_max, uint32_t mx, int kind_sum,
+                                          uint32_t sum) {
+    const unsigned s = blockIdx.x % STAT_SHARDS;
+    if (mx) atomicMax(&shard[kind_max * STAT_SHARDS + s], (unsigned long long)mx);
+    if (kind_sum >= 0 && sum) atomicAdd(&shard[kind_sum * STAT_SHARDS + s], (unsigned long long)sum);
+}
+inline size_t stats_copy_bytes(int levels) {
+    const int k = levels < MAX_LEVELS ? levels : MAX_LEVELS;
+    return ((size_t)MAX_LEVELS * ST_COUNT + (lean(LEAN_STATS) ? (size_t)k * SH_KINDS * STAT_SHARDS : 0)) * 8;
+}
+void fold_shards(unsigned long long *hs, int levels) {
+    if (!lean(LEAN_STATS)) return;
+    for (int l = 0; l < levels && l < MAX_LEVELS; ++l) {
+        const unsigned long long *sh = shards_of(hs, l);
+        unsigned long long len = 0, sum = 0, maxr = 0;
+        for (int s = 0; s < STAT_SHARDS; ++s) {
+            len = std::max(len, sh[SH_LEN * STAT_SHARDS + s]);
+            sum += sh[SH_SUM * STAT_SHARDS + s];
+            maxr = std::max(maxr, sh[SH_MAXR * STAT_SHARDS + s]);
+        }
+        unsigned long long *w = hs + (size_t)l * ST_COUNT;
+        w[ST_MAXLEN] = len;
+        w[l == 0 ? ST_GRADED : ST_NNZ] = sum;
+        w[ST_MAXR] = maxr;
+    }
+}
 __global__ __launch_bounds__(1024) void reduce_bstat(int nblocks, const uint32_t *__restrict__ bstat,
                                                      unsigned long long *__restrict__ stats, int slot_max,
                                                      int slot_sum) {
@@ -219,7 +260,7 @@
                                                 const int32_t *__restrict__ indices,
                                                 const double *__restrict__ data, double share, double spread,
                                                 bool general, unsigned long long *__restrict__ stats,
-                                                uint32_t *__restrict__ bstat) {
+                                                uint32_t *__restrict__ bstat, unsigned long long *__restrict__ shard) {
     int32_t mlen = 0;
     uint32_t graded = 0, bad = 0, far = 0;
     for (int64_t i = (int64_t)xcd_block() * TB + threadIdx.x; i < n; i += (int64_t)gridDim.x * TB) {
@@ -249,8 +290,12 @@
     if (far) atomicOr(&s_bad, 2u);
     __syncthreads();
     if (threadIdx.x == 0) {
-        bstat[blockIdx.x] = s_len;
-        bstat[BSTAT_MAX + blockIdx.x] = s_graded;
+        if (shard) {
+            shard_put(shard, SH_LEN, s_len, SH_SUM, s_graded);
+        } else {
+            bstat[blockIdx.x] = s_len;
+            bstat[BSTAT_MAX + blockIdx.x] = s_graded;
+        }
         if (s_bad & 1u) atomicOr(&stats[ST_BADDIAG], 1ull);
         if (s_bad & 2u) stats[ST_FARCOL] = 1ull;
     }
@@ -285,6 +330,68 @@
     }
 }
 
+__global__ __launch_bounds__(TB) void row_stats_to_ell(int64_t n, int64_t ld, const int32_t *__restrict__ indptr,
+                                                       const int32_t *__restrict__ indices, const double *__restrict__ data,
+                                                       double share, double spread, bool general,
+                                                       unsigned long long *__restrict__ stats, uint32_t *__restrict__ bstat,
+                                                       unsigned long long *__restrict__ shard, int32_t *__restrict__ col,
+                                                       double *__restrict__ val, float *__restrict__ valf,
+                                                       int32_t *__restrict__ len, double *__restrict__ dinv, int32_t wpad,
+                                                       int16_t *__restrict__ dcol) {
+    int32_t mlen = 0;
+    uint32_t graded = 0, bad = 0, far = 0;
+    for (int64_t i = (int64_t)xcd_block() * TB + threadIdx.x; i < n; i += (int64_t)gridDim.x * TB) {
+        const int32_t e0 = indptr[i], e1 = indptr[i + 1];
+        mlen = max(mlen, e1 - e0);
+        double d = 0.0, mx = 0.0, mn = 1e300;
+        bool stored = false;
+        for (int32_t e = e0; e < e1; ++e) {
+            const int32_t c = indices[e];
+            const double v = data[e];
+            col[(int64_t)(e - e0) * ld + i] = c;
+            if (dcol) dcol[(int64_t)(e - e0) * ld + i] = (int16_t)(c - (int32_t)i);
+            val[(int64_t)(e - e0) * ld + i] = v;
+            valf[(int64_t)(e - e0) * ld + i] = (float)v;
+            const int64_t dc = (int64_t)c - i;
+            if (dc > 32767 || dc < -32767) far = 1;
+            if (c == (int32_t)i) { d = v; stored = true; }
+            else if (v != 0.0) {
+                mx = fmax(mx, fabs(v));
+                mn = fmin(mn, fabs(v));
+                if (v > 0.0 && !general) bad = 1;
+            }
+        }
+        for (int32_t s = e1 - e0; s < wpad; ++s) {
+            col[(int64_t)s * ld + i] = (int32_t)i;
+            if (dcol) dcol[(int64_t)s * ld + i] = 0;
+            val[(int64_t)s * ld + i] = 0.0;
+            valf[(int64_t)s * ld + i] = 0.0f;
+        }
+        len[i] = e1 - e0;
+        dinv[i] = 1.0 / (stored ? d : 1.0);
+        if (!(d > 0.0)) bad = 1;
+        graded += (d > 0.0 && (mx > share * d || mx > spread * mn)) ? 1u : 0u;
+    }
+    __shared__ unsigned int s_len, s_graded, s_bad;
+    if (threadIdx.x == 0) s_len = s_graded = s_bad = 0;
+    __syncthreads();
+    atomicMax(&s_len, (unsigned)mlen);
+    if (graded) atomicAdd(&s_graded, graded);
+    if (bad) atomicOr(&s_bad, 1u);
+    if (far) atomicOr(&s_bad, 2u);
+    __syncthreads();
+    if (threadIdx.x == 0) {
+        if (shard) {
+            shard_put(shard, SH_LEN, s_len, SH_SUM, s_graded);
+        } else {
+            bstat[blockIdx.x] = s_len;
+            bstat[BSTAT_MAX + blockIdx.x] = s_graded;
+        }
+        if (s_bad & 1u) atomicOr(&stats[ST_BADDIAG], 1ull);
+        if (s_bad & 2u) stats[ST_FARCOL] = 1ull;
+    }
+}
+
 
 __device__ __forceinline__ uint32_t hash30(uint32_t x) {
     x ^= x >> 16;
@@ -324,13 +431,37 @@
         m[i] = nbr_max(A, v, i, A.len[i], v[i]);
 }
 
+template <int NB>
+__device__ __forceinline__ uint32_t nbr_max_first_batch(const Ell &A, int64_t i, int32_t l, int32_t s0, uint32_t best) {
+    int32_t c[NB];
+#pragma unroll
+    for (int u = 0; u < NB; ++u) c[u] = A.col[(int64_t)(s0 + u < l ? s0 + u : 0) * A.ld + i];
+#pragma unroll
+    for (int u = 0; u < NB; ++u) {
+        const uint32_t t = (1u << 30) | hash30((uint32_t)c[u]);
+        best = t > best ? t : best;
+    }
+    return best;
+}
+__global__ __launch_bounds__(TB) void mis_max_first(Ell A, uint32_t *__restrict__ m) {
+    for (int64_t i = (int64_t)xcd_block() * TB + threadIdx.x; i < A.n; i += (int64_t)gridDim.x * TB) {
+        const int32_t l = A.len[i];
+        uint32_t best = (1u << 30) | hash30((uint32_t)i);
+        if (l <= 5) best = nbr_max_first_batch<5>(A, i, l, 0, best);
+        else for (int32_t s0 = 0; s0 < l; s0 += 8) best = nbr_max_first_batch<8>(A, i, l, s0, best);
+        m[i] = best;
+    }
+}
+
+template <bool FIRST>
 __global__ __launch_bounds__(TB) void mis_update(Ell A, uint32_t *__restrict__ T, const uint32_t *__restrict__ m1) {
     for (int64_t i = (int64_t)xcd_block() * TB + threadIdx.x; i < A.n; i += (int64_t)gridDim.x * TB) {
-        const uint32_t own = T[i];
-        if ((own >> 30) != 1) continue;
+        const uint32_t own = FIRST ? ((1u << 30) | hash30((uint32_t)i)) : T[i];
+        if (!FIRST && (own >> 30) != 1) continue;
         const uint32_t best = nbr_max(A, m1, i, A.len[i], m1[i]);
         if (best == own) T[i] = own | (2u << 30);
         else if ((best >> 30) == 3) T[i] = 0;
+        else if (FIRST) T[i] = own;
     }
 }
 
@@ -541,7 +672,7 @@
                                                double *__restrict__ rval, float *__restrict__ rvalf,
                                                int32_t *__restrict__ rlen,
                                                unsigned long long *__restrict__ stats, uint32_t *__restrict__ bstat,
-                                               uint32_t rcap) {
+                                               uint32_t rcap, unsigned long long *__restrict__ shard) {
     uint32_t mlen = 0;
     const int sub = threadIdx.x & 7;
     const int64_t rows_per_pass = (int64_t)gridDim.x * (TB / 8);
@@ -580,8 +711,12 @@
     if ((threadIdx.x & 63) == 0) atomicMax(&s_max, mlen);
     __syncthreads();
     if (threadIdx.x == 0) {
-        bstat[blockIdx.x] = s_max;
-        bstat[BSTAT_MAX + blockIdx.x] = 0;
+        if (shard) {
+            shard_put(shard, SH_MAXR, s_max, -1, 0);
+        } else {
+            bstat[blockIdx.x] = s_max;
+            bstat[BSTAT_MAX + blockIdx.x] = 0;
+        }
     }
 }
 
@@ -890,7 +1025,7 @@
                                                float *__restrict__ cvalf,
                                                int32_t *__restrict__ clen, double *__restrict__ cdinv,
                                                unsigned long long *__restrict__ stats, uint32_t *__restrict__ bstat,
-                                               int G, int pcap, int maxseg) {
+                                               int G, int pcap, int maxseg, unsigned long long *__restrict__ shard) {
     extern __shared__ __attribute__((aligned(16))) char gsm[];
     int32_t *set = reinterpret_cast<int32_t *>(gsm);
     double *lV = reinterpret_cast<double *>(gsm + 1024);
@@ -1003,8 +1138,12 @@
         __syncthreads();
     }
     if (lane == 0) {
-        bstat[blockIdx.x] = my_max;
-        bstat[BSTAT_MAX + blockIdx.x] = my_nnz;
+        if (shard) {
+            shard_put(shard, SH_LEN, my_max, SH_SUM, my_nnz);
+        } else {
+            bstat[blockIdx.x] = my_max;
+            bstat[BSTAT_MAX + blockIdx.x] = my_nnz;
+        }
     }
     if (my_flags & 1u) atomicOr(&stats[ST_OVERFLOW], 1ull);
     if (my_flags & 4u) atomicOr(&stats[ST_BADDIAG], 1ull);
@@ -1162,11 +1301,13 @@
     static const int maxseg = knob::SA_GSEG.now();
     const unsigned gg = (unsigned)(nc < gcap ? nc : (gcap < BSTAT_MAX ? gcap : BSTAT_MAX));
     if (r_ready) NODAL_HIP_TRY(h, hipStreamWaitEvent(st, r_ready, 0));
+    const bool sharded = !NUMERIC && lean(LEAN_STATS);
     galerkin<NUMERIC><<<gg, 64, lds, st>>>(
         ld, apcol, apval, aplen, nc, L->rld, L->rcol.as<int32_t>(), L->rval.as<double>(), L->rlen.as<int32_t>(),
         C->ld, C->acol.as<int32_t>(), C->aval.as<double>(), C->avalf.as<float>(), C->alen.as<int32_t>(),
-        C->dinv.as<double>(), dstats + (size_t)(l + 1) * ST_COUNT, H->bstat.as<uint32_t>(), G, pcap, maxseg);
-    if (!NUMERIC)
+        C->dinv.as<double>(), dstats + (size_t)(l + 1) * ST_COUNT, H->bstat.as<uint32_t>(), G, pcap, maxseg,
+        sharded ? shards_of(dstats, l + 1) : nullptr);
+    if (!NUMERIC && !sharded)
         reduce_bstat<<<1, 1024, 0, st>>>((int)gg, H->bstat.as<uint32_t>(), dstats + (size_t)(l + 1) * ST_COUNT,
                                          ST_MAXLEN, ST_NNZ);
     NODAL_HIP_TRY(h, hipGetLastError());
@@ -1258,10 +1399,16 @@
     if (n <= MIS_SMALL_MAX && !trace_mis) {
         mis_small<<<1, 1024, 0, st>>>(A, T, M, flag, mis_rounds);
     } else {
-        mis_init<<<g, TB, 0, st>>>(n, T);
+        const bool first_forms = lean(LEAN_MIS);
+        if (!first_forms) mis_init<<<g, TB, 0, st>>>(n, T);
         for (int r = 0; r < mis_rounds; ++r) {
-            mis_max<<<g, TB, 0, st>>>(A, T, M);
-            mis_update<<<g, TB, 0, st>>>(A, T, M);
+            if (r == 0 && first_forms) {
+                mis_max_first<<<g, TB, 0, st>>>(A, M);
+                mis_update<true><<<g, TB, 0, st>>>(A, T, M);
+            } else {
+                mis_max<<<g, TB, 0, st>>>(A, T, M);
+                mis_update<false><<<g, TB, 0, st>>>(A, T, M);
+            }
             if (trace_mis) mis_count<<<g, TB, 0, st>>>(n, T, cnt + r + 1);
         }
         mis_flag_roots<<<grid_for(n + 1), TB, 0, st>>>(A, T, flag);
@@ -1269,7 +1416,7 @@
     NODAL_HIP_TRY(h, hipGetLastError());
     NODAL_TRY(scan_exclusive_u32(h, flag, id, n + 1, reinterpret_cast<uint32_t *>(dstats + (size_t)l * ST_COUNT + ST_NC),
                                  scan_tmp));
-    NODAL_HIP_TRY(h, hipMemcpyAsync(hs, dstats, (size_t)MAX_LEVELS * ST_COUNT * 8, hipMemcpyDeviceToHost, st));
+    NODAL_HIP_TRY(h, hipMemcpyAsync(hs, dstats, stats_copy_bytes(l + 1), hipMemcpyDeviceToHost, st));
     unsigned long long hcnt[MIS_ROUNDS + 1] = {0};
     if (trace_mis) NODAL_HIP_TRY(h, hipMemcpyAsync(hcnt, cnt, sizeof hcnt, hipMemcpyDeviceToHost, st));
     if (!H->ev_copy) NODAL_HIP_TRY(h, hipEventCreateWithFlags(&H->ev_copy, hipEventDisableTiming));
@@ -1283,6 +1430,7 @@
                              L->pval.as<double>(), L->pvalf.as<float>(), omega_p(l));
     NODAL_HIP_TRY(h, hipGetLastError());
     NODAL_WAIT_EVENT(h, H->ev_copy, st);
+    fold_shards(hs, l + 1);
     if (trace_mis) {
         fprintf(stderr, "[sagg] level %d: undecided after each MIS round:", l);
         for (int r = 1; r <= MIS_ROUNDS; ++r) fprintf(stderr, " %llu", hcnt[r]);
@@ -1397,10 +1545,13 @@
 
     {
         const unsigned gr = grid_for(nc * 8);
+        const bool sharded = lean(LEAN_STATS);
         r_to_ell<<<gr, TB, 0, st>>>(nc, L->rld, rstart, keys, ld, L->pval.as<double>(), L->rcol.as<int32_t>(),
                                    L->rval.as<double>(), L->rvalf.as<float>(), L->rlen.as<int32_t>(),
-                                   dstats + (size_t)l * ST_COUNT, H->bstat.as<uint32_t>(), (uint32_t)rcap);
-        reduce_bstat<<<1, 1024, 0, st>>>((int)gr, H->bstat.as<uint32_t>(), dstats + (size_t)l * ST_COUNT, ST_MAXR, -1);
+                                   dstats + (size_t)l * ST_COUNT, H->bstat.as<uint32_t>(), (uint32_t)rcap,
+                                   sharded ? shards_of(dstats, l) : nullptr);
+        if (!sharded)
+            reduce_bstat<<<1, 1024, 0, st>>>((int)gr, H->bstat.as<uint32_t>(), dstats + (size_t)l * ST_COUNT, ST_MAXR, -1);
     }
     if (forked) {
         NODAL_HIP_TRY(h, hipGetLastError());
@@ -1683,20 +1834,31 @@
     hipStream_t st = h->stream;
     unsigned long long *dstats = H->stats.as<unsigned long long>();
     unsigned long long *hs = reinterpret_cast<unsigned long long *>(H->host_stats);
-    NODAL_HIP_TRY(h, hipMemsetAsync(dstats, 0, (size_t)MAX_LEVELS * ST_COUNT * 8, st));
+    NODAL_HIP_TRY(h, hipMemsetAsync(dstats, 0, STATS_BYTES, st));
     SLevel *L0 = H->pool[0];
     const int64_t n0 = L0->n;
     {
         const unsigned gr = grid_for(n0);
         static const double spread = knob::SA_SPREAD.now();
         static const double share = knob::SA_SHARE.now();
-        row_stats<<<gr, TB, 0, st>>>(n0, indptr0, indices0, data0, share, spread, general, dstats, H->bstat.as<uint32_t>());
-        reduce_bstat<<<1, 1024, 0, st>>>((int)gr, H->bstat.as<uint32_t>(), dstats, ST_MAXLEN, ST_GRADED);
-    }
-    csr_to_ell<<<grid_for(n0), TB, 0, st>>>(n0, L0->ld, indptr0, indices0, data0, L0->acol.as<int32_t>(),
-                                           L0->aval.as<double>(), L0->avalf.as<float>(),
-                                           L0->alen.as<int32_t>(), L0->dinv.as<double>(), L0->wfix,
-                                           L0->d16 ? L0->adcol.as<int16_t>() : nullptr);
+        const bool sharded = lean(LEAN_STATS);
+        unsigned long long *shard = sharded ? shards_of(dstats, 0) : nullptr;
+        if (lean(LEAN_ROWS)) {
+            row_stats_to_ell<<<gr, TB, 0, st>>>(n0, L0->ld, indptr0, indices0, data0, share, spread, general, dstats,
+                                               H->bstat.as<uint32_t>(), shard, L0->acol.as<int32_t>(), L0->aval.as<double>(),
+                                               L0->avalf.as<float>(), L0->alen.as<int32_t>(), L0->dinv.as<double>(), L0->wfix,
+                                               L0->d16 ? L0->adcol.as<int16_t>() : nullptr);
+        } else {
+            row_stats<<<gr, TB, 0, st>>>(n0, indptr0, indices0, data0, share, spread, general, dstats, H->bstat.as<uint32_t>(),
+                                         shard);
+        }
+        if (!sharded) reduce_bstat<<<1, 1024, 0, st>>>((int)gr, H->bstat.as<uint32_t>(), dstats, ST_MAXLEN, ST_GRADED);
+    }
+    if (!lean(LEAN_ROWS))
+        csr_to_ell<<<grid_for(n0), TB, 0, st>>>(n0, L0->ld, indptr0, indices0, data0, L0->acol.as<int32_t>(),
+                                               L0->aval.as<double>(), L0->avalf.as<float>(),
+                                               L0->alen.as<int32_t>(), L0->dinv.as<double>(), L0->wfix,
+                                               L0->d16 ? L0->adcol.as<int16_t>() : nullptr);
     NODAL_HIP_TRY(h, hipGetLastError());
     for (int l = 0; l + 1 < H->nlev; ++l) {
         SLevel *L = H->pool[l], *C = H->pool[l + 1];
@@ -1728,8 +1890,9 @@
     if (H->tail >= 0) k_tail_pack<<<1, 1024, 0, st>>>(H->td, H->tail_image.as<char>());
     NODAL_HIP_TRY(h, hipGetLastError());
     NODAL_TRY(form_tail_op(h, H));
-    NODAL_HIP_TRY(h, hipMemcpyAsync(hs, dstats, (size_t)MAX_LEVELS * ST_COUNT * 8, hipMemcpyDeviceToHost, st));
+    NODAL_HIP_TRY(h, hipMemcpyAsync(hs, dstats, stats_copy_bytes(1), hipMemcpyDeviceToHost, st));
     NODAL_WAIT_STREAM(h, st);
+    fold_shards(hs, 1);
     const int64_t bar = n0 / 100 < 32 ? (n0 / 100 > 0 ? n0 / 100 : 1) : 32;
     if (hs[ST_BADDIAG] || (int64_t)hs[ST_GRADED] >= bar) return NODAL_OK;
     for (int k = 1; k < H->nlev; ++k)
@@ -1795,23 +1958,26 @@
     H->flags_levels = 0;
     H->last_iters = 0;
     H->drop_graph();
-    NODAL_HIP_TRY(h, H->stats.reserve((size_t)MAX_LEVELS * ST_COUNT * 8 + 64));
+    NODAL_HIP_TRY(h, H->stats.reserve(STATS_BYTES + 64));
     if (!H->host_stats)
-        NODAL_HIP_TRY(h, hipHostMalloc(reinterpret_cast<void **>(&H->host_stats), (size_t)MAX_LEVELS * ST_COUNT * 8 + 64));
+        NODAL_HIP_TRY(h, hipHostMalloc(reinterpret_cast<void **>(&H->host_stats), STATS_BYTES + 64));
     unsigned long long *dstats = H->stats.as<unsigned long long>();
     unsigned long long *hs = reinterpret_cast<unsigned long long *>(H->host_stats);
-    NODAL_HIP_TRY(h, hipMemsetAsync(dstats, 0, (size_t)MAX_LEVELS * ST_COUNT * 8, st));
+    NODAL_HIP_TRY(h, hipMemsetAsync(dstats, 0, STATS_BYTES, st));
     NODAL_HIP_TRY(h, H->bstat.reserve((size_t)2 * BSTAT_MAX * 4 + 64));
     {
         const unsigned gr = grid_for(n0);
         static const double spread = knob::SA_SPREAD.now();
         static const double share = knob::SA_SHARE.now();
-        row_stats<<<gr, TB, 0, st>>>(n0, indptr0, indices0, data0, share, spread, general, dstats, H->bstat.as<uint32_t>());
-        reduce_bstat<<<1, 1024, 0, st>>>((int)gr, H->bstat.as<uint32_t>(), dstats, ST_MAXLEN, ST_GRADED);
+        const bool sharded = lean(LEAN_STATS);
+        row_stats<<<gr, TB, 0, st>>>(n0, indptr0, indices0, data0, share, spread, general, dstats, H->bstat.as<uint32_t>(),
+                                     sharded ? shards_of(dstats, 0) : nullptr);
+        if (!sharded) reduce_bstat<<<1, 1024, 0, st>>>((int)gr, H->bstat.as<uint32_t>(), dstats, ST_MAXLEN, ST_GRADED);
     }
     NODAL_HIP_TRY(h, hipGetLastError());
-    NODAL_HIP_TRY(h, hipMemcpyAsync(hs, dstats, ST_COUNT * 8, hipMemcpyDeviceToHost, st));
+    NODAL_HIP_TRY(h, hipMemcpyAsync(hs, dstats, lean(LEAN_STATS) ? stats_copy_bytes(1) : (size_t)ST_COUNT * 8, hipMemcpyDeviceToHost, st));
     NODAL_WAIT_STREAM(h, st);
+    fold_shards(hs, 1);
     const int64_t bar = n0 / 100 < 32 ? (n0 / 100 > 0 ? n0 / 100 : 1) : 32;
     if (hs[ST_MAXLEN] > (unsigned long long)W0_MAX || hs[ST_MAXLEN] == 0 || hs[ST_BADDIAG] ||
         (int64_t)hs[ST_GRADED] >= bar) {
@@ -1871,7 +2037,7 @@
     SLevel *last = H->level(l);
     last->fold_want = last->fold = false;
     if (H->nlev < 2) return NODAL_OK;
-    NODAL_HIP_TRY(h, hipMemcpyAsync(hs, dstats, (size_t)MAX_LEVELS * ST_COUNT * 8, hipMemcpyDeviceToHost, st));
+    NODAL_HIP_TRY(h, hipMemcpyAsync(hs, dstats, stats_copy_bytes(H->nlev), hipMemcpyDeviceToHost, st));
     if (!H->ev_copy) NODAL_HIP_TRY(h, hipEventCreateWithFlags(&H->ev_copy, hipEventDisableTiming));
     NODAL_HIP_TRY(h, hipEventRecord(H->ev_copy, st));
     if (check_floating) {
@@ -1892,6 +2058,7 @@
         NODAL_HIP_TRY(h, hipGetLastError());
     }
     NODAL_WAIT_EVENT(h, H->ev_copy, st);
+    fold_shards(hs, H->nlev);
     for (int k = 0; k < H->nlev; ++k) {
         const unsigned long long *s = hs + (size_t)k * ST_COUNT;
         if (k > 0) {
@@ -1921,16 +2088,18 @@
     NODAL_TRY(build_tail(h, H, hs));
 
     if (!check_floating) {
-        NODAL_HIP_TRY(h, hipMemcpyAsync(hs, dstats, (size_t)MAX_LEVELS * ST_COUNT * 8, hipMemcpyDeviceToHost, st));
+        NODAL_HIP_TRY(h, hipMemcpyAsync(hs, dstats, stats_copy_bytes(H->nlev), hipMemcpyDeviceToHost, st));
         NODAL_WAIT_STREAM(h, st);
+        fold_shards(hs, H->nlev);
         if (hs[(size_t)l * ST_COUNT + ST_BADDIAG] & 2ull) return NODAL_OK;
     } else {
         uint32_t *fl = reinterpret_cast<uint32_t *>(dstats + (size_t)(MAX_LEVELS - 1) * ST_COUNT + ST_COUNT - 1);
         if (H->dense_coarsest) last_level_floating<<<1, 64, 0, st>>>(last->A(), last->gflag.as<uint8_t>(), fl);
         else any_unflagged<<<grid_for(last->n), TB, 0, st>>>(last->n, last->gflag.as<uint8_t>(), fl);
         NODAL_HIP_TRY(h, hipGetLastError());
-        NODAL_HIP_TRY(h, hipMemcpyAsync(hs, dstats, (size_t)MAX_LEVELS * ST_COUNT * 8, hipMemcpyDeviceToHost, st));
+        NODAL_HIP_TRY(h, hipMemcpyAsync(hs, dstats, stats_copy_bytes(H->nlev), hipMemcpyDeviceToHost, st));
         NODAL_WAIT_STREAM(h, st);
+        fold_shards(hs, H->nlev);
         if (hs[(size_t)l * ST_COUNT + ST_BADDIAG] & 2ull) {
             if (trace) fprintf(stderr, "[sagg] declined: coarsest matrix not positive definite\n");
             return NODAL_OK;
@@ -2218,9 +2387,10 @@
     const Ell A0 = H->pool[0]->A();
 
     const double tol = 1e-13;
-    f_set_scalars<<<1, 1, 0, st>>>(sb.sc, tol * tol);
+    const bool init_sets = lean(LEAN_SCALARS);
+    if (!init_sets) f_set_scalars<<<1, 1, 0, st>>>(sb.sc, tol * tol);
     const double *dinv0 = H->pool[0]->dinv.as<double>();
-    f_init<<<sb.g0, TB, 0, st>>>(b, x, sb.r, sb.Ap, dinv0, sb.x0, sb.part_rr, n);
+    f_init<<<sb.g0, TB, 0, st>>>(b, x, sb.r, sb.Ap, dinv0, sb.x0, sb.part_rr, n, init_sets ? sb.sc : nullptr, tol * tol);
     NODAL_HIP_TRY(h, hipGetLastError());
 
     const int64_t maxit = knob::FCG_MAXIT.now().value_or(2000);
diff --git a/nodal_amd/csrc/sagg_cycle.h b/nodal_amd/csrc/sagg_cycle.h
--- a/nodal_amd/csrc/sagg_cycle.h
+++ b/nodal_amd/csrc/sagg_cycle.h
@@ -775,7 +775,9 @@
 __global__ __launch_bounds__(TB) void f_init(const double *__restrict__ b, double *__restrict__ x,
                                              double *__restrict__ r, double *__restrict__ Ap,
                                              const double *__restrict__ dinv, cyc_t *__restrict__ x0,
-                                             double *__restrict__ part_rr, int64_t n) {
+                                             double *__restrict__ part_rr, int64_t n, double *__restrict__ sc,
+                                             double tol2) {
+    if (sc && blockIdx.x == 0 && threadIdx.x < F_COUNT) sc[threadIdx.x] = threadIdx.x == F_TOL2 ? tol2 : 0.0;
     double srr = 0.0;
     for (int64_t i = (int64_t)xcd_block() * TB + threadIdx.x; i < n; i += (int64_t)gridDim.x * TB) {
         const double ri = b[i];
```
